# preon7/2019global

Measured on AMD Instinct MI355X. Metric: Mray/s + ms/frame at 1920x1080, depth 8; %HBM roofline, higher is better.
Workload: dtype f64

## Files before the change

### 2019global_amd/__init__.py

```python
from __future__ import annotations

import ctypes
import os
import threading
from typing import Optional, Sequence

import numpy as np

from . import scenes as _scenes

__all__ = [
    "GIError", "lib", "Camera", "Material", "Octree", "ImpSphere", "ImpTriangle", "ExpQuad",
    "ExpSphere", "ExpCube", "ExpCone", "ExpRectangle", "ExpBox",
    "RayTracer", "DeviceScene", "MODE_R", "MODE_X", "STAT_RAYS", "STAT_NODES", "STAT_PRIMS",
    "STAT_PIXELS", "TILE", "MultiScene", "devices_from_env", "obj_entities", "RAY_DOUBLES",
    "AOV_OUTPUTS", "camera_rays", "camera_rays_device",
]

HERE = os.path.dirname(os.path.abspath(__file__))
LIB_PATH = os.environ.get("GI_LIB") or os.path.join(HERE, "libgi.so")

MODE_R, MODE_X = 0, 1
FLAG_STATS = 1
FLAG_R_DFS = 2
FLAG_TIME = 4
FLAG_X_NO_SHADOW = 8
FLAG_X_WF = 16
FLAG_X_MEGA = 32
FLAG_X_SEG = 64
KAT_X_TREE, KAT_X_HBM = 1, 2
X_FORMS = ("k_mode_x", "k_wf_bounce", "k_seg")
R_KERNELS = ("k_mode_r", "k_rf_walk", "k_mode_r_batch")
STAT_RAYS, STAT_NODES, STAT_PRIMS, STAT_PIXELS, STAT_X_PATH_MAX = 0, 1, 2, 3, 4
STAT_X_ITERS, STAT_X_TRAV, STAT_X_HANDLE, STAT_X_HLANES, STAT_X_HCLOSE, STAT_X_HSHADOW = 5, 6, 7, 8, 9, 10
STAT_X_CYC_TRAV, STAT_X_CYC_HIT, STAT_X_CYC_NEXT, STAT_X_CYC_ALL = 11, 12, 13, 14
STAT_X_RESOLVED = 15
STAT_X_IT_NODE, STAT_X_LN_NODE, STAT_X_IT_LEAF, STAT_X_LN_LEAF = 16, 17, 18, 19
STAT_X_IT_RS, STAT_X_LN_RS, STAT_X_IT_ST, STAT_X_LN_ST = 20, 21, 22, 23
STAT_R_PAIRS, STAT_R_OVF_TILES = 24, 25
STATS_N = 26
TILE = 8
ABI_VERSION = 13
RAY_DOUBLES = 8
AOV_OUTPUTS = ("t", "normal", "albedo", "prim", "entity", "uv")
_AOV_KINDS = {"t": (np.float64, ()), "normal": (np.float64, (3,)), "albedo": (np.float64, (3,)),
              "prim": (np.int32, ()), "entity": (np.int32, ()), "uv": (np.int32, (2,))}


class GIError(RuntimeError):
    pass


class EntityDesc(ctypes.Structure):
    _fields_ = [("kind", ctypes.c_int32), ("has_material", ctypes.c_int32), ("args", ctypes.c_double * 11),
                ("mat_color", ctypes.c_double * 3), ("mat_shader", ctypes.c_double * 3),
                ("mat_specular_power", ctypes.c_double), ("mat_reflectivity", ctypes.c_double)]


class SceneDesc(ctypes.Structure):
    _fields_ = [("octree_min", ctypes.c_double * 3), ("octree_max", ctypes.c_double * 3),
                ("n_entities", ctypes.c_int32), ("entities", ctypes.POINTER(EntityDesc))]


class CameraDesc(ctypes.Structure):
    _fields_ = [("pos", ctypes.c_double * 3), ("up", ctypes.c_double * 3), ("forward", ctypes.c_double * 3),
                ("focal", ctypes.c_double)]


class Opts(ctypes.Structure):
    _fields_ = [("mode", ctypes.c_int32), ("spp", ctypes.c_int32), ("depth", ctypes.c_int32),
                ("shard_count", ctypes.c_int32), ("shard_index", ctypes.c_int32), ("band_rows", ctypes.c_int32),
                ("flags", ctypes.c_uint32), ("reserved", ctypes.c_int32), ("seed", ctypes.c_uint64),
                ("stats", ctypes.c_void_p), ("sample_begin", ctypes.c_int32), ("sample_end", ctypes.c_int32)]


class SceneInfo(ctypes.Structure):
    _fields_ = [("n_entities", ctypes.c_int32), ("n_nodes", ctypes.c_int32), ("n_leaves", ctypes.c_int32),
                ("max_depth", ctypes.c_int32), ("n_reachable", ctypes.c_int32), ("n_dropped", ctypes.c_int32),
                ("x_nodes", ctypes.c_int32), ("x_prims", ctypes.c_int32), ("device_bytes", ctypes.c_int64),
                ("x_node_bytes", ctypes.c_int32), ("x_lds_resident", ctypes.c_int32)]


class Hit(ctypes.Structure):
    _fields_ = [("entity", ctypes.c_int32), ("u", ctypes.c_int32), ("v", ctypes.c_int32),
                ("point", ctypes.c_double * 3), ("normal", ctypes.c_double * 3)]


class AovFrame(ctypes.Structure):
    _fields_ = [("w", ctypes.c_int32), ("h", ctypes.c_int32), ("x0", ctypes.c_int32), ("y0", ctypes.c_int32),
                ("x1", ctypes.c_int32), ("y1", ctypes.c_int32)]


class Aov(ctypes.Structure):
    _fields_ = [("t", ctypes.c_void_p), ("normal", ctypes.c_void_p), ("albedo", ctypes.c_void_p),
                ("prim", ctypes.c_void_p), ("entity", ctypes.c_void_p), ("uv", ctypes.c_void_p)]


TILE_CB = ctypes.CFUNCTYPE(None, ctypes.c_void_p, ctypes.c_int, ctypes.c_int, ctypes.POINTER(ctypes.c_uint8),
                           ctypes.POINTER(ctypes.c_double))

EXPORTS = ["gi_abi_version", "gi_last_error", "gi_camera_init", "gi_scene_create", "gi_scene_destroy",
           "gi_scene_get_info", "gi_render", "gi_render_device", "gi_shard_tiles", "gi_unshard_device",
           "gi_trace_ray", "gi_kat_expbox", "gi_kat_x_query", "gi_kat_x_variant", "gi_scene_kernel_ms", "gi_scene_x_form", "gi_scene_r_kernel", "gi_octree_create", "gi_octree_destroy",
           "gi_octree_intersect", "gi_multi_create", "gi_multi_destroy", "gi_multi_info", "gi_multi_render", "gi_device_count",
           "gi_device_list", "gi_build_id", "gi_obj_parse", "gi_intersect", "gi_occluded", "gi_intersect_device",
           "gi_occluded_device", "gi_render_aov", "gi_render_aov_device", "gi_camera_rays", "gi_camera_rays_device"]

_lib = None
_lock = threading.Lock()


def lib():
    global _lib
    with _lock:
        if _lib is not None:
            return _lib
        if not os.path.exists(LIB_PATH):
            raise GIError(f"{LIB_PATH} is missing: run `python 2019global_amd/build.py` (no CPU fallback)")
        try:
            import torch
        except ImportError:
            pass
        L = ctypes.CDLL(LIB_PATH)
        vp, i32, dp = ctypes.c_void_p, ctypes.c_int, ctypes.POINTER(ctypes.c_double)
        L.gi_abi_version.restype = i32
        L.gi_last_error.restype = ctypes.c_char_p
        L.gi_camera_init.argtypes = [dp, dp, ctypes.c_double, ctypes.POINTER(CameraDesc)]
        L.gi_scene_create.argtypes = [ctypes.POINTER(SceneDesc), ctypes.POINTER(vp)]
        L.gi_scene_destroy.argtypes = [vp]
        L.gi_scene_destroy.restype = None
        L.gi_scene_get_info.argtypes = [vp, ctypes.POINTER(SceneInfo)]
        L.gi_render.argtypes = [vp, ctypes.POINTER(CameraDesc), dp, i32, i32, ctypes.POINTER(Opts), dp,
                                ctypes.POINTER(ctypes.c_uint8), ctypes.POINTER(ctypes.c_int), TILE_CB, vp]
        L.gi_render_device.argtypes = [vp, ctypes.POINTER(CameraDesc), dp, i32, i32, ctypes.POINTER(Opts), vp, vp, vp]
        L.gi_shard_tiles.argtypes = [i32, i32, i32]
        L.gi_shard_tiles.restype = ctypes.c_int64
        L.gi_unshard_device.argtypes = [i32, i32, i32, vp, vp, vp, vp, vp]
        L.gi_trace_ray.argtypes = [vp, dp, dp, dp, ctypes.POINTER(Hit), dp]
        L.gi_kat_expbox.argtypes = [i32, dp, ctypes.POINTER(ctypes.c_int32)]
        ip = ctypes.POINTER(ctypes.c_int32)
        L.gi_kat_x_query.argtypes = [vp, i32, dp, dp, i32, ip, dp, ip, ip, ip, dp, ip, dp]
        L.gi_kat_x_variant.argtypes = [vp, i32, ip]
        i64 = ctypes.c_int64
        L.gi_intersect.argtypes = [vp, i64, dp, dp, ip, ip, dp]
        L.gi_occluded.argtypes = [vp, i64, dp, ip]
        L.gi_intersect_device.argtypes = [vp, i64, vp, vp, vp, vp, vp, vp]
        L.gi_occluded_device.argtypes = [vp, i64, vp, vp, vp]
        L.gi_render_aov.argtypes = [vp, ctypes.POINTER(CameraDesc), ctypes.POINTER(AovFrame), ctypes.POINTER(Aov)]
        L.gi_render_aov_device.argtypes = [vp, ctypes.POINTER(CameraDesc), ctypes.POINTER(AovFrame), ctypes.POINTER(Aov), vp]
        L.gi_camera_rays.argtypes = [ctypes.POINTER(CameraDesc), ctypes.POINTER(AovFrame), dp]
        L.gi_camera_rays_device.argtypes = [ctypes.POINTER(CameraDesc), ctypes.POINTER(AovFrame), vp, vp]
        L.gi_scene_kernel_ms.argtypes = [vp, ctypes.POINTER(ctypes.c_float), ctypes.POINTER(ctypes.c_int64)]
        L.gi_scene_x_form.argtypes = [vp, ctypes.POINTER(Opts), ctypes.POINTER(ctypes.c_int32)]
        L.gi_scene_r_kernel.argtypes = [vp, ctypes.POINTER(Opts), ctypes.POINTER(ctypes.c_int32)]
        L.gi_octree_create.argtypes = [ctypes.POINTER(SceneDesc), ctypes.POINTER(vp)]
        L.gi_octree_destroy.argtypes = [vp]
        L.gi_octree_destroy.restype = None
        L.gi_octree_intersect.argtypes = [vp, dp, dp, ctypes.POINTER(ctypes.c_int32), ctypes.c_int64,
                                          ctypes.POINTER(ctypes.c_int64)]
        L.gi_multi_create.argtypes = [ctypes.POINTER(SceneDesc), i32, ctypes.POINTER(ctypes.c_int), ctypes.POINTER(vp)]
        L.gi_multi_destroy.argtypes = [vp]
        L.gi_multi_destroy.restype = None
        L.gi_multi_info.argtypes = [vp, ctypes.POINTER(ctypes.c_int), ctypes.POINTER(ctypes.c_int),
                                    ctypes.POINTER(ctypes.c_int)]
        L.gi_multi_render.argtypes = [vp, ctypes.POINTER(CameraDesc), dp, i32, i32, ctypes.POINTER(Opts), dp,
                                      ctypes.POINTER(ctypes.c_uint8), ctypes.POINTER(ctypes.c_int), TILE_CB, vp]
        L.gi_device_list.argtypes = [ctypes.POINTER(ctypes.c_int32), i32]
        L.gi_build_id.restype = ctypes.c_char_p
        L.gi_obj_parse.argtypes = [ctypes.c_char_p, ctypes.c_int64, ctypes.POINTER(EntityDesc),
                                   ctypes.POINTER(EntityDesc), ctypes.c_int64, ctypes.POINTER(ctypes.c_int64)]
        if L.gi_abi_version() != ABI_VERSION:
            raise GIError(f"libgi ABI {L.gi_abi_version()} != {ABI_VERSION}")
        _lib = L
        return L


def build_id() -> str:
    return lib().gi_build_id().decode()


def _check(rc: int, what: str) -> None:
    if rc != 0:
        raise GIError(f"{what} failed ({rc}): {lib().gi_last_error().decode()}")


def _check_rays(rays) -> int:
    if not isinstance(rays, np.ndarray) or rays.dtype != np.float64 or rays.ndim != 2 or rays.shape[1] != RAY_DOUBLES or \
            not rays.flags.c_contiguous:
        raise ValueError(f"rays: a C-contiguous float64 array of shape (n, {RAY_DOUBLES}) -- o[3], d[3], tmax, reserved")
    return int(rays.shape[0])


def _aov_frame(w, h, window) -> AovFrame:
    def whole(v):
        return isinstance(v, (int, np.integer)) and not isinstance(v, bool)
    if not (whole(w) and whole(h)) or w <= 0 or h <= 0 or w >= 2 ** 31 or h >= 2 ** 31:
        raise ValueError("frame: w and h are positive integers")
    if window is None:
        window = (0, 0, w, h)
    window = tuple(window)
    if len(window) != 4 or not all(whole(v) for v in window):
        raise ValueError("window: four integers (x0, y0, x1, y1)")
    x0, y0, x1, y1 = (int(v) for v in window)
    if not (0 <= x0 <= x1 <= w and 0 <= y0 <= y1 <= h):
        raise ValueError(f"window {window}: reversed or not inside the {w} x {h} frame")
    return AovFrame(int(w), int(h), x0, y0, x1, y1)


def _d3(v) -> ctypes.Array:
    return (ctypes.c_double * 3)(*[float(x) for x in v])


class Material:

    def __init__(self, color, shader=(0.1, 0.7, 1.0), specular_power: float = 5.0, reflectivity: float = 0.0):
        self.color = tuple(float(c) for c in color)
        self.shader_parameters = tuple(float(c) for c in shader)
        self.specular_power = float(specular_power)
        self.reflectivity = float(reflectivity)


class _Entity:
    kind = 0

    def __init__(self, args: Sequence[float], material: Optional[Material]):
        self._args = tuple(float(a) for a in args)
        self._material = material

    @property
    def material(self) -> Optional[Material]:
        return self._material

    @material.setter
    def material(self, m: Material) -> None:
        self._material = m

    def _desc(self, d: EntityDesc) -> None:
        d.kind = self.kind
        for i, a in enumerate(self._args):
            d.args[i] = a
        m = self._material
        d.has_material = 1 if m is not None else 0
        if m is not None:
            for i in range(3):
                d.mat_color[i] = m.color[i]
                d.mat_shader[i] = m.shader_parameters[i]
            d.mat_specular_power = m.specular_power
            d.mat_reflectivity = m.reflectivity


class ImpSphere(_Entity):
    kind = _scenes.IMP_SPHERE

    def __init__(self, pos, radius, color):
        super().__init__((*pos, radius, *color), None)


class ImpTriangle(_Entity):
    kind = _scenes.IMP_TRIANGLE

    def __init__(self, p1, p2, p3):
        super().__init__((*p1, *p2, *p3), None)


class ExpQuad(_Entity):
    kind = _scenes.EXP_QUAD

    def __init__(self, pos, width, length, alpha, color):
        super().__init__((*pos, width, length, alpha, *color), None)


class ExpSphere(_Entity):
    kind = _scenes.EXP_SPHERE

    def __init__(self, pos, radius, color):
        super().__init__((*pos, radius, *color), None)


class ExpCube(_Entity):
    kind = _scenes.EXP_CUBE

    def __init__(self, pos, width, length, height, color):
        super().__init__((*pos, width, length, height, *color), None)


class ExpCone(_Entity):
    kind = _scenes.EXP_CONE

    def __init__(self, pos, dir, height, radius, color):
        super().__init__((*pos, *dir, height, radius, *color), None)


class ExpRectangle(_Entity):
    kind = _scenes.EXP_RECTANGLE

    def __init__(self, p1, p2, p3):
        super().__init__((*p1, *p2, *p3), None)


class ExpBox(_Entity):
    kind = _scenes.EXP_BOX

    def __init__(self, mn, mx):
        super().__init__((*mn, *mx), None)


def obj_entities(text, material: Optional[Material] = None) -> list:
    L = lib()
    data = text.encode() if isinstance(text, str) else bytes(text)
    tmpl = None
    if material is not None:
        tmpl = EntityDesc()
        t = _Entity((), material)
        t._desc(tmpl)
    n = ctypes.c_int64()
    _check(L.gi_obj_parse(data, len(data), tmpl, None, 0, ctypes.byref(n)), "gi_obj_parse")
    arr = (EntityDesc * max(1, n.value))()
    _check(L.gi_obj_parse(data, len(data), tmpl, arr, n.value, ctypes.byref(n)), "gi_obj_parse")
    out = []
    for i in range(n.value):
        d = arr[i]
        e = ImpTriangle(tuple(d.args[0:3]), tuple(d.args[3:6]), tuple(d.args[6:9]))
        if material is not None:
            e.material = Material(material.color, material.shader_parameters, material.specular_power,
                                  material.reflectivity)
        out.append(e)
    return out


class Octree:

    def __init__(self, min=(-20, -20, -20), max=(20, 20, 20)):
        self.min = tuple(float(v) for v in min)
        self.max = tuple(float(v) for v in max)
        self.entities = []
        self.generation = 0
        self._host = None
        self._host_gen = -1

    def push_back(self, e: _Entity) -> None:
        self.entities.append(e)
        self.generation += 1

    def intersect(self, origin, direction) -> list:
        L = lib()
        if self._host is None or self._host_gen != self.generation:
            self._close_host()
            d, keep = self._scene_desc()
            h = ctypes.c_void_p()
            _check(L.gi_octree_create(ctypes.byref(d), ctypes.byref(h)), "gi_octree_create")
            del keep
            self._host, self._host_gen = h, self.generation
        dv = np.asarray(direction, np.float64)
        dv = dv * (1.0 / np.sqrt((dv[0] * dv[0] + dv[1] * dv[1]) + dv[2] * dv[2]))
        n = ctypes.c_int64()
        _check(L.gi_octree_intersect(self._host, _d3(origin), _d3(dv), None, 0, ctypes.byref(n)), "gi_octree_intersect")
        out = (ctypes.c_int32 * max(1, n.value))()
        _check(L.gi_octree_intersect(self._host, _d3(origin), _d3(dv), out, n.value, ctypes.byref(n)),
               "gi_octree_intersect")
        return [self.entities[i] for i in out[:n.value]]

    def _close_host(self):
        if self._host is not None and self._host.value:
            lib().gi_octree_destroy(self._host)
        self._host = None

    def __del__(self):
        try:
            self._close_host()
        except Exception:
            pass

    @classmethod
    def from_scene(cls, s: "_scenes.Scene") -> "Octree":
        o = cls(s.octree_min, s.octree_max)
        for e in s.entities:
            ent = _Entity(e.args, None if e.material is None else
                          Material(e.material.color, e.material.shader, e.material.specular_power,
                                   e.material.reflectivity))
            ent.kind = e.kind
            o.push_back(ent)
        return o

    def _scene_desc(self):
        n = len(self.entities)
        arr = (EntityDesc * max(n, 1))()
        for i, e in enumerate(self.entities):
            e._desc(arr[i])
        d = SceneDesc()
        d.octree_min = _d3(self.min)
        d.octree_max = _d3(self.max)
        d.n_entities = n
        d.entities = ctypes.cast(arr, ctypes.POINTER(EntityDesc))
        return d, arr


class Camera:

    def __init__(self, pos, lookAt=(0.0, 0.0, 0.0), focal: float = 0.04):
        self._c = CameraDesc()
        _check(lib().gi_camera_init(_d3(pos), _d3(lookAt), float(focal), ctypes.byref(self._c)), "gi_camera_init")

    @property
    def pos(self):
        return tuple(self._c.pos)

    @property
    def up(self):
        return tuple(self._c.up)

    @property
    def forward(self):
        return tuple(self._c.forward)

    @property
    def focalDist(self):
        return self._c.focal


class DeviceScene:

    def __init__(self, octree: Octree):
        L = lib()
        d, keep = octree._scene_desc()
        h = ctypes.c_void_p()
        _check(L.gi_scene_create(ctypes.byref(d), ctypes.byref(h)), "gi_scene_create")
        self._h = h
        del keep

    @classmethod
    def from_scene(cls, s: "_scenes.Scene") -> "DeviceScene":
        return cls(Octree.from_scene(s))

    def close(self) -> None:
        if getattr(self, "_h", None) and self._h.value:
            lib().gi_scene_destroy(self._h)
            self._h = ctypes.c_void_p()

    def __del__(self):
        try:
            self.close()
        except Exception:
            pass

    def info(self) -> dict:
        i = SceneInfo()
        _check(lib().gi_scene_get_info(self._h, ctypes.byref(i)), "gi_scene_get_info")
        return {f: getattr(i, f) for f, _ in SceneInfo._fields_}

    @staticmethod
    def opts(mode=MODE_R, spp=1, depth=1, seed=0, shard_count=1, shard_index=0, band_rows=0, stats_ptr=0,
             flags=0, samples=None) -> Opts:
        o = Opts()
        o.mode, o.spp, o.depth, o.seed = mode, spp, depth, seed
        o.shard_count, o.shard_index, o.band_rows = shard_count, shard_index, band_rows
        o.flags = (FLAG_STATS if stats_ptr else 0) | flags
        o.stats = stats_ptr or None
        if samples is not None:
            o.sample_begin, o.sample_end = samples
        return o

    def render(self, cam: Camera, light, w: int, h: int, mode=MODE_R, spp=1, depth=1, seed=0, band_rows=0,
               cancel: Optional[ctypes.c_int] = None, callback=None, out=None, flags=0, samples=None):
        if out is None:
            rgb, rgb8 = np.zeros((h, w, 3), np.float64), np.zeros((h, w, 3), np.uint8)
        else:
            rgb, rgb8 = out
        for a, dt in ((rgb, np.float64), (rgb8, np.uint8)):
            if a is not None and (a.dtype != dt or a.size != w * h * 3 or not a.flags.c_contiguous):
                raise ValueError("render: out arrays must be C-contiguous [h, w, 3] float64 / uint8")
        cb = TILE_CB(callback) if callback is not None else TILE_CB()
        o = self.opts(mode, spp, depth, seed, band_rows=band_rows, flags=flags, samples=samples)
        _check(lib().gi_render(self._h, ctypes.byref(cam._c), _d3(light), w, h, ctypes.byref(o),
                               rgb.ctypes.data_as(ctypes.POINTER(ctypes.c_double)) if rgb is not None else None,
                               rgb8.ctypes.data_as(ctypes.POINTER(ctypes.c_uint8)) if rgb8 is not None else None,
                               ctypes.byref(cancel) if cancel is not None else None, cb, None), "gi_render")
        return rgb, rgb8

    def render_device(self, cam: Camera, light, w: int, h: int, d_rgb: int, d_rgb8: int = 0, stream: int = 0,
                      mode=MODE_R, spp=1, depth=1, seed=0, shard_count=1, shard_index=0, stats_ptr=0,
                      flags=0, samples=None) -> None:
        o = self.opts(mode, spp, depth, seed, shard_count, shard_index, stats_ptr=stats_ptr, flags=flags,
                      samples=samples)
        _check(lib().gi_render_device(self._h, ctypes.byref(cam._c), _d3(light), w, h, ctypes.byref(o),
                                      d_rgb or None, d_rgb8 or None, stream or None), "gi_render_device")

    def x_form(self, mode=MODE_X, spp=1, depth=1, flags=0) -> str:
        o = self.opts(mode, spp, depth, 0, flags=flags)
        f = ctypes.c_int32()
        _check(lib().gi_scene_x_form(self._h, ctypes.byref(o), ctypes.byref(f)), "gi_scene_x_form")
        return X_FORMS[f.value]

    def r_kernel(self, flags=0) -> str:
        o = self.opts(MODE_R, 1, 1, 0, flags=flags)
        k = ctypes.c_int32()
        _check(lib().gi_scene_r_kernel(self._h, ctypes.byref(o), ctypes.byref(k)), "gi_scene_r_kernel")
        return R_KERNELS[k.value]

    def kernel_ms(self):
        ms, n = ctypes.c_float(), ctypes.c_int64()
        _check(lib().gi_scene_kernel_ms(self._h, ctypes.byref(ms), ctypes.byref(n)), "gi_scene_kernel_ms")
        return float(ms.value), int(n.value)

    def trace_ray(self, origin, direction, light):
        hit = Hit()
        rgb = (ctypes.c_double * 3)()
        _check(lib().gi_trace_ray(self._h, _d3(origin), _d3(direction), _d3(light), ctypes.byref(hit), rgb),
               "gi_trace_ray")
        return hit, tuple(rgb)

    INTERSECT_OUTPUTS = ("t", "prim", "entity", "normal")

    def intersect(self, rays: np.ndarray, want=INTERSECT_OUTPUTS) -> dict:
        n = _check_rays(rays)
        want = tuple(want)
        if not want or any(k not in self.INTERSECT_OUTPUTS for k in want) or len(set(want)) != len(want):
            raise ValueError(f"intersect: want is a non-empty selection of {self.INTERSECT_OUTPUTS}")
        m = max(n, 1)
        bufs = {"t": np.empty(m, np.float64), "prim": np.empty(m, np.int32), "entity": np.empty(m, np.int32),
                "normal": np.empty((m, 3), np.float64)}
        ip, dp = ctypes.POINTER(ctypes.c_int32), ctypes.POINTER(ctypes.c_double)
        ptr = {k: (bufs[k].ctypes.data_as(dp if bufs[k].dtype == np.float64 else ip) if k in want else None)
               for k in self.INTERSECT_OUTPUTS}
        _check(lib().gi_intersect(self._h, n, rays.ctypes.data_as(dp), ptr["t"], ptr["prim"], ptr["entity"], ptr["normal"]),
               "gi_intersect")
        return {k: bufs[k][:n] for k in want}

    def occluded(self, rays: np.ndarray) -> np.ndarray:
        n = _check_rays(rays)
        out = np.empty(max(n, 1), np.int32)
        _check(lib().gi_occluded(self._h, n, rays.ctypes.data_as(ctypes.POINTER(ctypes.c_double)),
                                 out.ctypes.data_as(ctypes.POINTER(ctypes.c_int32))), "gi_occluded")
        return out[:n]

    def intersect_device(self, n: int, d_rays: int, d_t: int = 0, d_prim: int = 0, d_entity: int = 0, d_normal: int = 0,
                         stream: int = 0) -> None:
        _check(lib().gi_intersect_device(self._h, int(n), d_rays or None, d_t or None, d_prim or None, d_entity or None,
                                         d_normal or None, stream or None), "gi_intersect_device")

    def occluded_device(self, n: int, d_rays: int, d_occluded: int, stream: int = 0) -> None:
        _check(lib().gi_occluded_device(self._h, int(n), d_rays or None, d_occluded or None, stream or None),
               "gi_occluded_device")

    def render_aov(self, cam: "Camera", w: int, h: int, window=None, want=AOV_OUTPUTS) -> dict:
        want = tuple(want)
        if not want or any(k not in AOV_OUTPUTS for k in want) or len(set(want)) != len(want):
            raise ValueError(f"render_aov: want is a non-empty selection of {AOV_OUTPUTS}")
        f = _aov_frame(w, h, window)
        rows, cols = f.y1 - f.y0, f.x1 - f.x0
        bufs = {k: np.empty((rows, cols) + _AOV_KINDS[k][1], _AOV_KINDS[k][0]) for k in want}
        a = Aov(**{k: bufs[k].ctypes.data if bufs[k].size else _scratch_ptr() for k in want})
        _check(lib().gi_render_aov(self._h, ctypes.byref(cam._c), ctypes.byref(f), ctypes.byref(a)), "gi_render_aov")
        return bufs

    def render_aov_device(self, cam: "Camera", w: int, h: int, window=None, d_t: int = 0, d_normal: int = 0,
                          d_albedo: int = 0, d_prim: int = 0, d_entity: int = 0, d_uv: int = 0, stream: int = 0) -> None:
        f = _aov_frame(w, h, window)
        a = Aov(d_t or None, d_normal or None, d_albedo or None, d_prim or None, d_entity or None, d_uv or None)
        _check(lib().gi_render_aov_device(self._h, ctypes.byref(cam._c), ctypes.byref(f), ctypes.byref(a), stream or None),
               "gi_render_aov_device")

    def kat_x_variant(self, flags: int = 0) -> dict:
        out = (ctypes.c_int32 * 6)()
        _check(lib().gi_kat_x_variant(self._h, int(flags), out), "gi_kat_x_variant")
        return dict(zip(("LDS", "W4", "SH", "TRI", "CN", "FLAT"), (bool(v) for v in out)))

    def kat_x_query(self, recs: np.ndarray, cam_pos, flags: int = 0) -> dict:
        recs = np.ascontiguousarray(recs, np.float64).reshape(-1, 12)
        n = recs.shape[0]
        out = dict(prim1=np.zeros(n, np.int32), t1=np.zeros(n), occl=np.zeros(n, np.int32), skip_s=np.zeros(n, np.int32),
                   prim2=np.zeros(n, np.int32), t2=np.zeros(n), skip2=np.zeros(n, np.int32))
        sc = ctypes.c_double(float("nan"))
        ip, dp = ctypes.POINTER(ctypes.c_int32), ctypes.POINTER(ctypes.c_double)
        _check(lib().gi_kat_x_query(self._h, n, recs.ctypes.data_as(dp), _d3(cam_pos), int(flags),
                                    out["prim1"].ctypes.data_as(ip), out["t1"].ctypes.data_as(dp),
                                    out["occl"].ctypes.data_as(ip), out["skip_s"].ctypes.data_as(ip),
                                    out["prim2"].ctypes.data_as(ip), out["t2"].ctypes.data_as(dp),
                                    out["skip2"].ctypes.data_as(ip), ctypes.byref(sc)), "gi_kat_x_query")
        out["skip_cos"] = sc.value if n else None
        return out


_scratch = None


def _scratch_ptr() -> int:
    global _scratch
    if _scratch is None:
        _scratch = np.zeros(8)
    return _scratch.ctypes.data


def camera_rays(cam: "Camera", w: int, h: int, window=None) -> np.ndarray:
    f = _aov_frame(w, h, window)
    rays = np.empty(((f.y1 - f.y0) * (f.x1 - f.x0), RAY_DOUBLES), np.float64)
    p = rays.ctypes.data_as(ctypes.POINTER(ctypes.c_double)) if rays.size else \
        ctypes.cast(_scratch_ptr(), ctypes.POINTER(ctypes.c_double))
    _check(lib().gi_camera_rays(ctypes.byref(cam._c), ctypes.byref(f), p), "gi_camera_rays")
    return rays


def camera_rays_device(cam: "Camera", w: int, h: int, d_rays: int, window=None, stream: int = 0) -> None:
    f = _aov_frame(w, h, window)
    _check(lib().gi_camera_rays_device(ctypes.byref(cam._c), ctypes.byref(f), d_rays or None, stream or None),
           "gi_camera_rays_device")


def devices_from_env(default=None):
    v = os.environ.get("GI_DEVICES")
    if not v:
        return default
    if v.strip() == "all":
        import torch
        return list(range(torch.cuda.device_count()))
    return [int(t) for t in v.split(",") if t.strip()]


class MultiScene:

    def __init__(self, octree: Octree, devices: Sequence[int]):
        L = lib()
        d, keep = octree._scene_desc()
        devs = (ctypes.c_int * len(devices))(*[int(x) for x in devices])
        h = ctypes.c_void_p()
        _check(L.gi_multi_create(ctypes.byref(d), len(devices), devs, ctypes.byref(h)), "gi_multi_create")
        self._h = h
        del keep

    @classmethod
    def from_scene(cls, s: "_scenes.Scene", devices: Sequence[int]) -> "MultiScene":
        return cls(Octree.from_scene(s), devices)

    def info(self) -> dict:
        a, b, c = ctypes.c_int(), ctypes.c_int(), ctypes.c_int()
        _check(lib().gi_multi_info(self._h, ctypes.byref(a), ctypes.byref(b), ctypes.byref(c)), "gi_multi_info")
        return {"shards": a.value, "devices": b.value, "rccl": bool(c.value)}

    def render(self, cam: Camera, light, w: int, h: int, mode=MODE_R, spp=1, depth=1, seed=0, band_rows=0,
               cancel: Optional[ctypes.c_int] = None, callback=None, out=None):
        if out is None:
            rgb, rgb8 = np.zeros((h, w, 3), np.float64), np.zeros((h, w, 3), np.uint8)
        else:
            rgb, rgb8 = out
        for a, dt in ((rgb, np.float64), (rgb8, np.uint8)):
            if a is not None and (a.dtype != dt or a.size != w * h * 3 or not a.flags.c_contiguous):
                raise ValueError("render: out arrays must be C-contiguous [h, w, 3] float64 / uint8")
        cb = TILE_CB(callback) if callback is not None else TILE_CB()
        o = DeviceScene.opts(mode, spp, depth, seed, band_rows=band_rows)
        _check(lib().gi_multi_render(self._h, ctypes.byref(cam._c), _d3(light), w, h, ctypes.byref(o),
                                     rgb.ctypes.data_as(ctypes.POINTER(ctypes.c_double)) if rgb is not None else None,
                                     rgb8.ctypes.data_as(ctypes.POINTER(ctypes.c_uint8)) if rgb8 is not None else None,
                                     ctypes.byref(cancel) if cancel is not None else None, cb, None), "gi_multi_render")
        return rgb, rgb8

    def close(self) -> None:
        if getattr(self, "_h", None) and self._h.value:
            lib().gi_multi_destroy(self._h)
            self._h = ctypes.c_void_p()

    def __del__(self):
        try:
            self.close()
        except Exception:
            pass


def kat_expbox(recs: np.ndarray) -> np.ndarray:
    recs = np.ascontiguousarray(recs, np.float64)
    out = np.zeros(recs.shape[0], np.int32)
    _check(lib().gi_kat_expbox(recs.shape[0], recs.ctypes.data_as(ctypes.POINTER(ctypes.c_double)),
                               out.ctypes.data_as(ctypes.POINTER(ctypes.c_int32))), "gi_kat_expbox")
    return out


def shard_tiles(w: int, h: int, shard_count: int) -> int:
    return int(lib().gi_shard_tiles(w, h, shard_count))


def unshard_device(w, h, shard_count, d_packed, d_packed8, d_rgb, d_rgb8, stream=0) -> None:
    _check(lib().gi_unshard_device(w, h, shard_count, d_packed or None, d_packed8 or None, d_rgb or None,
                                   d_rgb8 or None, stream or None), "gi_unshard_device")


class Image:

    def __init__(self, rgb8: np.ndarray, rgb: Optional[np.ndarray] = None):
        self.rgb8 = rgb8
        self.radiance = rgb

    def width(self) -> int:
        return self.rgb8.shape[1]

    def height(self) -> int:
        return self.rgb8.shape[0]

    def getPixel(self, x: int, y: int):
        p = self.rgb8[y, x]
        return (p[0] / 255.0, p[1] / 255.0, p[2] / 255.0)


class RayTracer:

    def __init__(self, camera: Camera, light):
        self._camera = camera
        self._light = tuple(float(v) for v in light)
        self._image = Image(np.zeros((0, 0, 3), np.uint8))
        self._scene: Optional[Octree] = None
        self._dev: Optional[DeviceScene] = None
        self._cancel = ctypes.c_int(1)
        self.band_rows = 64

    def setScene(self, scene: Octree) -> None:
        self._scene = scene
        self._dev = None
        self._dev_gen = -1

    def running(self) -> bool:
        return self._cancel.value == 0

    def stop(self) -> None:
        self._cancel.value = 1

    def start(self) -> None:
        self._cancel.value = 0

    def getImage(self) -> Image:
        return self._image

    def run(self, w: int, h: int) -> None:
        self._image = Image(np.zeros((h, w, 3), np.uint8), np.zeros((h, w, 3)))
        if self._scene is None:
            raise GIError("setScene() was not called")
        if self._dev is None or getattr(self, "_dev_gen", -1) != self._scene.generation:
            devs = devices_from_env()
            self._dev = MultiScene(self._scene, devs) if devs and len(devs) > 1 else DeviceScene(self._scene)
            self._dev_gen = self._scene.generation
        img = self._image

        def on_band(_user, y0, rows, p8, pf):
            n = w * rows * 3
            img.rgb8[y0:y0 + rows] = np.ctypeslib.as_array(p8, shape=(n,)).reshape(rows, w, 3)
            img.radiance[y0:y0 + rows] = np.ctypeslib.as_array(pf, shape=(n,)).reshape(rows, w, 3)

        rgb = np.zeros((h, w, 3))
        rgb8 = np.zeros((h, w, 3), np.uint8)
        o = DeviceScene.opts(MODE_R, band_rows=self.band_rows)
        cb = TILE_CB(on_band)
        fn = lib().gi_multi_render if isinstance(self._dev, MultiScene) else lib().gi_render
        rc = fn(self._dev._h, ctypes.byref(self._camera._c), _d3(self._light), w, h, ctypes.byref(o),
                             rgb.ctypes.data_as(ctypes.POINTER(ctypes.c_double)),
                             rgb8.ctypes.data_as(ctypes.POINTER(ctypes.c_uint8)), ctypes.byref(self._cancel), cb, None)
        if rc not in (0, -4):
            _check(rc, "gi_render")
```

### 2019global_amd/build.py

```python
from __future__ import annotations

import glob
import hashlib
import os
import shutil
import subprocess
import sys

HERE = os.path.dirname(os.path.abspath(__file__))
ROOT = os.path.dirname(HERE)
CSRC = os.path.join(HERE, "csrc")
INCLUDE = os.path.join(ROOT, "include")
OUT = os.path.join(HERE, "libgi.so")
ROCM = os.environ.get("ROCM_PATH", "/opt/rocm")
ARCH = "gfx950"

HOST_SRCS = ["gi_build.cpp", "gi_bvh.cpp", "gi_capi.cpp", "gi_multi.cpp", "gi_obj.cpp"]
DEV_SRCS = ["gi_kernels.hip", "gi_wf.hip"]
HEADERS = ["gi_math.h", "gi_scene.h", "gi_internal.h", "gi_dev.h"]

COMMON = ["-std=c++17", "-fPIC", "-ffp-contract=off", "-fno-fast-math", f"-I{INCLUDE}", f"-I{CSRC}"]


def source_hash() -> str:
    h = hashlib.sha256()
    for name in sorted(HOST_SRCS + DEV_SRCS + HEADERS):
        h.update(name.encode() + b"\0" + open(os.path.join(CSRC, name), "rb").read() + b"\0")
    h.update(b"gi.h\0" + open(os.path.join(INCLUDE, "gi.h"), "rb").read())
    return h.hexdigest()[:16]


def _run(cmd, verbose):
    if verbose:
        print(" ".join(cmd), flush=True)
    subprocess.run(cmd, check=True)


def _stale(out, deps):
    if not os.path.exists(out):
        return True
    t = os.path.getmtime(out)
    return any(os.path.getmtime(d) > t for d in deps)


def build(verbose: bool = False, force: bool = False, variant: str = "", hip_defines=()) -> str:
    hipcc = shutil.which("hipcc") or os.path.join(ROCM, "bin", "hipcc")
    objdir = os.path.join(HERE, "_obj")
    out = OUT
    if variant:
        out = os.path.join(HERE, "_variants", f"libgi_{variant}.so")
        os.makedirs(os.path.dirname(out), exist_ok=True)
    os.makedirs(objdir, exist_ok=True)
    hdrs = [os.path.join(CSRC, h) for h in HEADERS] + [os.path.join(INCLUDE, "gi.h")]
    bid = source_hash()
    bid_file = os.path.join(objdir, "build_id")
    old_bid = open(bid_file).read().strip() if os.path.exists(bid_file) else ""
    objs = []
    for s in HOST_SRCS:
        src, obj = os.path.join(CSRC, s), os.path.join(objdir, s + ".o")
        defs = [f'-DGI_BUILD_ID="{bid}"'] if s == "gi_capi.cpp" else []
        if force or _stale(obj, [src] + hdrs) or (defs and old_bid != bid):
            _run(["g++", "-O2", *COMMON, *defs, "-D__HIP_PLATFORM_AMD__", f"-I{ROCM}/include", "-c", src, "-o", obj],
                 verbose)
        objs.append(obj)
    with open(bid_file, "w") as f:
        f.write(bid + "\n")
    jobs = []
    for s in DEV_SRCS:
        src = os.path.join(CSRC, s)
        obj = os.path.join(objdir, s + (f".{variant}" if variant else "") + ".o")
        if force or _stale(obj, [src] + hdrs):
            extra = os.environ.get("GI_VARIANT_FLAGS", "").split() if variant else []
            cmd = [hipcc, f"--offload-arch={ARCH}", "-O3", "-Wshadow", *COMMON, *[f"-D{d}" for d in hip_defines],
                   *extra, "-munsafe-fp-atomics", "-c", src, "-o", obj]
            if verbose:
                print(" ".join(cmd), flush=True)
            jobs.append((cmd, subprocess.Popen(cmd)))
        objs.append(obj)
    failed = [(cmd, p.returncode) for cmd, p in [(c, p) for c, p in jobs if p.wait() != 0]]
    for cmd, _ in failed:
        if os.path.exists(cmd[-1]):
            os.remove(cmd[-1])
    if failed:
        for cmd, rc in failed:
            print(f"build failed ({rc}): {' '.join(cmd)}", file=sys.stderr)
        raise subprocess.CalledProcessError(failed[0][1], failed[0][0])
    if force or _stale(out, objs):
        _run([hipcc, f"--offload-arch={ARCH}", "-shared", "-o", out, *objs, f"-L{ROCM}/lib", "-lamdhip64", "-ldl"], verbose)
    for leftover in glob.glob(out + ".[0-9]*.hipv4-*") + glob.glob(out + ".[0-9]*.host-*"):
        os.remove(leftover)
    return out


if __name__ == "__main__":
    args = sys.argv[1:]
    var, defs = "", []
    if "--variant" in args:
        i = args.index("--variant")
        var, defs = args[i + 1], [a for a in args[i + 2:] if not a.startswith("--")]
    build(verbose=True, force="--force" in args, variant=var, hip_defines=defs)
```

### 2019global_amd/csrc/gi_capi.cpp

```cpp
#include <hip/hip_runtime_api.h>

#include <algorithm>
#include <cmath>
#include <cstring>
#include <memory>
#include <mutex>
#include <new>
#include <string>
#include <vector>

#include "gi.h"
#include "gi_internal.h"
#include "gi_scene.h"

namespace gi {
bool build_host_scene(const gi_scene_desc& desc, HostScene& hs, std::string& err);
long long shard_tiles(int w, int h, int shard_count);
hipError_t x_launch_config(const DevScene& sc, int device, XLaunchCfg& cfg);
int x_form_choice(const DevScene& sc, const XLaunchCfg& xc, const gi_opts& o);
long long x_wf_chunk();
int x_env_rf_per_slot();
int r_kernel_choice(const DevScene& sc, const gi_opts& o);
unsigned rf_own_pairs();
unsigned rf_page_pairs();
// ... 399 lines not shown
        return fail(GI_ERR_ARG, "progressive pass out of order: a pass continues the previous pass's frame "
                                "(same camera, light, size, spp, depth, seed, shard) from its sample_end");
    }
    s->prog_key = key;
    s->prog_next = -1;
    return GI_OK;
}
void prog_done(gi_scene* s, const gi_opts& o) {
    s->prog_next = (o.sample_end > 0 && o.sample_end < o.spp) ? o.sample_end : -1;
}

int band_rows_of(const gi_opts* o, int h) {
    int band = o->band_rows > 0 ? o->band_rows : h;
    band = ((band + GI_TILE - 1) / GI_TILE) * GI_TILE;
    return std::min(band, ((h + GI_TILE - 1) / GI_TILE) * GI_TILE);
}

int scene_create_on(const gi_scene_desc* desc, int device, gi_scene** out) {
    *out = nullptr;
    int rc = bind_device(device);
    if (rc || (rc = check_device(device))) return rc;
    std::unique_ptr<gi_scene, void (*)(gi_scene*)> s(new gi_scene(), [](gi_scene* p) { destroy_scene(p); });
    s->device = device;
    std::string err;
    if (!build_host_scene(*desc, s->host, err)) return fail(GI_ERR_SCENE, err);
    DevScene& d = s->dev;
    memset(&d, 0, sizeof d);
    const HostScene& h = s->host;
    hipError_t e;
    gi_scene* sp = s.get();
    if ((e = upload(sp, h.rnodes, &d.rnodes)) != hipSuccess || (e = upload(sp, h.leaf_ents, &d.leaf_ents)) != hipSuccess ||
        (e = upload(sp, h.ents, &d.ents)) != hipSuccess || (e = upload(sp, h.tris, &d.tris)) != hipSuccess ||
        (e = upload(sp, h.xwnodes, &d.xwnodes)) != hipSuccess || (e = upload(sp, h.xhot, &d.xhot)) != hipSuccess ||
        (e = upload(sp, h.xbox, &d.xbox)) != hipSuccess ||
        (e = upload(sp, h.xprims, &d.xprims)) != hipSuccess || (e = upload(sp, h.xflat, &d.xflat)) != hipSuccess ||
        (e = upload(sp, std::vector<unsigned>(16, 0u), const_cast<const unsigned**>(&d.work))) != hipSuccess ||
        (e = upload(sp, h.app_off, &d.app_off)) != hipSuccess || (e = upload(sp, h.app_rec, &d.app_rec)) != hipSuccess ||
        (e = upload(sp, h.rpath_rec, &d.rpath_rec)) != hipSuccess || (e = upload(sp, h.rc_nodes, &d.rc_nodes)) != hipSuccess ||
        (e = upload(sp, h.rc_ent, &d.rc_ent)) != hipSuccess || (e = upload(sp, h.rc_maxkey, &d.rc_maxkey)) != hipSuccess ||
        (e = upload(sp, h.r_always, &d.r_always)) != hipSuccess ||
        (e = upload(sp, h.r_leaf_of_rank, &d.r_leaf_of_rank)) != hipSuccess)
        return hip_fail(e, "scene upload");
    d.n_rnodes = (int32_t)h.rnodes.size();
    d.n_ents = (int32_t)h.ents.size();
    d.n_xwnodes = (int32_t)h.xwnodes.size();
    d.n_xprims = (int32_t)h.xprims.size();
    d.x_max_depth = h.x_max_depth;
    d.x_handle8 = h.x_handle8;
    d.x_flags = h.x_flags;
    d.x_skip_a = h.x_skip_a;
    d.x_skip_b = h.x_skip_b;
    d.n_xhot = (int32_t)h.xhot.size();
    d.n_r_always = (int32_t)h.r_always.size();
    d.rc_ext = (float)h.rc_ext;
    {
        const size_t bytes = h.xwnodes.size() * sizeof(XWNode) + h.xhot.size() * sizeof(XHot) +
                             h.xprims.size() * sizeof(XPrim) + h.ents.size() * sizeof(REnt);
        d.x_lds_bytes = bytes <= 40 * 1024 ? (int32_t)bytes : 0;
        d.n_xflat = (int32_t)h.xflat.size();
        d.x_flat = (d.x_lds_bytes > 0 && h.x_flat_ok) ? 1 : 0;
        const size_t per_wg = bytes + 256 * 10 * sizeof(double) + 4 * 68 * sizeof(unsigned);
        d.x_waves4 = (d.x_lds_bytes > 0 && 4 * per_wg <= 160 * 1024) ? 1 : 0;
        d.x_tri_only = 1;
        for (const REnt& r : h.ents)
            if (r.kind == K_IMP_SPHERE || r.kind == K_EXP_SPHERE || r.kind == K_EXP_CONE || r.kind == K_EXP_RECTANGLE) {
                d.x_waves4 = 0;
                d.x_tri_only = 0;
            }
        for (const XPrim& xp : h.xprims)
            if (xp.kind != 0) d.x_tri_only = 0;
        d.r_tri_only = 1;
        for (const REnt& r : h.ents)
            if (r.kind != K_IMP_TRIANGLE) d.r_tri_only = 0;
    }
    const bool want_cn = h.xwnodes.size() * sizeof(XWNode) > (size_t)2 << 20;
    if (d.x_lds_bytes == 0 && want_cn && encode_xcnodes(h.xwnodes, s->host.xcnodes) &&
        (e = upload(sp, h.xcnodes, &d.xcnodes)) != hipSuccess)
        return hip_fail(e, "scene upload (quantised nodes)");
    for (int k = 0; k < 3; ++k) { d.root_lo[k] = INFINITY; d.root_hi[k] = -INFINITY; }
    if (!h.xwnodes.empty())
        for (int c = 0; c < 8; ++c)
            if (h.xwnodes[0].child[c] != XEMPTY)
                for (int k = 0; k < 3; ++k) {
                    d.root_lo[k] = std::min(d.root_lo[k], h.xwnodes[0].lo[k][c]);
                    d.root_hi[k] = std::max(d.root_hi[k], h.xwnodes[0].hi[k][c]);
                }
    d.x_far_r = INFINITY;
    for (int k = 0; k < 3; ++k)
        if (d.root_lo[k] <= d.root_hi[k]) {
            const float m = 16.0f * std::max(std::fabs(d.root_lo[k]), std::fabs(d.root_hi[k]));
            d.x_far_r = std::isinf(d.x_far_r) ? m : std::max(d.x_far_r, m);
        }
    if ((e = x_launch_config(d, device, s->xcfg)) != hipSuccess) return hip_fail(e, "occupancy query");
    *out = s.release();
    return GI_OK;
}

void scene_destroy(gi_scene* s) noexcept { destroy_scene(s); }
int scene_device(const gi_scene* s) { return s->device; }
std::mutex& scene_mutex(gi_scene* s) { return s->mu; }

int scene_render_band(gi_scene* s, const CamDev& cd, const double light[3], int w, int h, int y0, const gi_opts& o,
                      double* d_rgb, uint8_t* d_rgb8, hipStream_t stream, bool timer) {
    int rc = bind_device(s->device);
    if (rc || (rc = ensure_xscratch(s, w, h, &o)) || (timer && (rc = ensure_timer(s, &o)))) return rc;
    return issue_render(s, cd, v3(light[0], light[1], light[2]), w, h, y0, o, d_rgb, d_rgb8, stream, timer);
}

int unshard(int w, int h, int n, const double* packed, const uint8_t* packed8, double* rgb, uint8_t* rgb8,
            hipStream_t stream) {
    const hipError_t e = launch_unshard(w, h, n, packed, packed8, rgb, rgb8, stream);
    return e == hipSuccess ? GI_OK : hip_fail(e, "unshard launch");
}

}

extern "C" {

int gi_abi_version(void) { return GI_ABI_VERSION; }
const char* gi_last_error(void) { return g_err.c_str(); }

int gi_device_list(int32_t* out, int cap) {
    int ndev = 0, n = 0;
    if (hipGetDeviceCount(&ndev) != hipSuccess) return 0;
    for (int d = 0; d < ndev; ++d) {
        hipDeviceProp_t prop;
        if (hipGetDeviceProperties(&prop, d) == hipSuccess && std::strncmp(prop.gcnArchName, "gfx950", 6) == 0) {
            if (out && n < cap) out[n] = d;
            ++n;
        }
    }
    return n;
}

int gi_device_count(void) { return gi_device_list(nullptr, 0); }

#ifndef GI_BUILD_ID
#define GI_BUILD_ID "unknown"
#endif
const char* gi_build_id(void) { return GI_BUILD_ID; }

int gi_camera_init(const double pos[3], const double look_at[3], double focal, gi_camera* out) {
    if (!pos || !look_at || !out) return fail(GI_ERR_ARG, "null argument");
    const V3 p = v3(pos[0], pos[1], pos[2]);
    const V3 f = normalize(v3(look_at[0], look_at[1], look_at[2]) - p);
    st3(out->pos, p);
    out->up[0] = 0; out->up[1] = 0; out->up[2] = 1.0;
    st3(out->forward, f);
    out->focal = focal;
    return GI_OK;
}

int gi_scene_create(const gi_scene_desc* desc, gi_scene** out) {
    return guard([&]() -> int {
        if (!desc || !out || desc->n_entities < 0 || (desc->n_entities > 0 && !desc->entities))
            return fail(GI_ERR_ARG, "bad scene descriptor");
        *out = nullptr;
        int ndev = 0;
        hipError_t e = hipGetDeviceCount(&ndev);
        if (e != hipSuccess || ndev <= 0) return fail(GI_ERR_DEVICE, "no HIP device (libgi renders only on gfx950)");
        int dev = 0;
        if ((e = hipGetDevice(&dev)) != hipSuccess) return hip_fail(e, "hipGetDevice");
        return scene_create_on(desc, dev, out);
    });
}

void gi_scene_destroy(gi_scene* s) { destroy_scene(s); }

int gi_scene_get_info(const gi_scene* s, gi_scene_info* info) {
    if (!s || !info) return fail(GI_ERR_ARG, "null argument");
    info->n_entities = (int32_t)s->host.ents.size();
    info->n_nodes = (int32_t)s->host.rnodes.size();
    info->n_leaves = s->host.n_leaves;
    info->max_depth = s->host.max_depth;
    info->n_reachable = s->host.n_reachable;
    info->n_dropped = s->host.n_dropped;
    info->x_nodes = (int32_t)(s->host.xnodes.empty() ? s->host.xwnodes.size() : s->host.xnodes.size());
    info->x_prims = (int32_t)s->host.xprims.size();
    info->device_bytes = s->bytes;
    info->x_node_bytes = s->dev.xcnodes ? (int32_t)sizeof(XCNode) : (int32_t)sizeof(XWNode);
    info->x_lds_resident = s->dev.x_lds_bytes > 0 ? 1 : 0;
    return GI_OK;
}

int64_t gi_shard_tiles(int w, int h, int shard_count) {
    if (w <= 0 || h <= 0 || shard_count < 1) return -1;
    return shard_tiles(w, h, shard_count);
}

int gi_render_device(gi_scene* s, const gi_camera* cam, const double light[3], int w, int h, const gi_opts* o,
                     double* d_rgb, uint8_t* d_rgb8, void* stream) {
    return guard([&]() -> int {
        DeviceRestore keep;
        if (!s) return fail(GI_ERR_ARG, "null scene");
        int rc = check_opts(w, h, o);
        if (rc) return rc;
        if (!cam || !light) return fail(GI_ERR_ARG, "null camera or light");
        std::lock_guard<std::mutex> lk(s->mu);
        if ((rc = prog_check(s, *cam, light, w, h, *o))) return rc;
        rc = scene_render_band(s, make_cam(*cam, w), light, w, h, 0, *o, d_rgb, d_rgb8, static_cast<hipStream_t>(stream),
                               true);
        if (rc == GI_OK) prog_done(s, *o);
        return rc;
    });
}

int gi_render(gi_scene* s, const gi_camera* cam, const double light[3], int w, int h, const gi_opts* o, double* rgb,
              uint8_t* rgb8, const volatile int* cancel, gi_tile_cb cb, void* user) {
    return guard([&]() -> int {
        DeviceRestore keep;
        if (!s) return fail(GI_ERR_ARG, "null scene");
        int rc = check_opts(w, h, o);
        if (rc) return rc;
        if (!cam || !light) return fail(GI_ERR_ARG, "null camera or light");
        if (o->shard_count != 1) return fail(GI_ERR_ARG, "gi_render renders whole frames; use gi_render_device or gi_multi to shard");
        std::lock_guard<std::mutex> lk(s->mu);
        if ((rc = bind_device(s->device))) return rc;
        const int band = band_rows_of(o, h);
        const size_t band_px = (size_t)w * (size_t)band;
        const int n_bands = (h + band - 1) / band;
        if (o->sample_end > 0 && n_bands > 1)
            return fail(GI_ERR_ARG, "progressive passes render whole frames: band_rows 0 or >= h");
        if ((rc = prog_check(s, *cam, light, w, h, *o))) return rc;
        if ((rc = ensure_hostpath(s, band_px, std::min(n_bands, HostPath::kSlots)))) return rc;
        HostPath& hp = s->hp;
        const CamDev cd = make_cam(*cam, w);
        const bool want_rgb = rgb || cb, want_rgb8 = rgb8 || cb;
        const bool direct = n_bands == 1;
        double* const dst_rgb = direct && rgb ? rgb : hp.h_rgb[0];
        uint8_t* const dst_rgb8 = direct && rgb8 ? rgb8 : hp.h_rgb8[0];
        auto issue = [&](int i) -> int {
            const int k = i % HostPath::kSlots, y0 = i * band, rows = std::min(band, h - y0);
            const size_t n = (size_t)w * rows * 3;
            hipError_t e = hipSuccess;
            if (i >= HostPath::kSlots && (e = hipStreamWaitEvent(hp.render, hp.copied[k], 0)) != hipSuccess)
                return hip_fail(e, "render");
            const int r = scene_render_band(s, cd, light, w, rows, y0, *o, hp.d_rgb[k], hp.d_rgb8[k], hp.render, false);
            if (r) return r;
            e = hipEventRecord(hp.rendered[k], hp.render);
            if (e == hipSuccess) e = hipStreamWaitEvent(hp.copy, hp.rendered[k], 0);
            double* const to = i == 0 ? dst_rgb : hp.h_rgb[k];
            uint8_t* const to8 = i == 0 ? dst_rgb8 : hp.h_rgb8[k];
            if (e == hipSuccess && want_rgb) e = hipMemcpyAsync(to, hp.d_rgb[k], n * sizeof(double), hipMemcpyDeviceToHost, hp.copy);
            if (e == hipSuccess && want_rgb8) e = hipMemcpyAsync(to8, hp.d_rgb8[k], n, hipMemcpyDeviceToHost, hp.copy);
            if (e == hipSuccess) e = hipEventRecord(hp.copied[k], hp.copy);
            return e == hipSuccess ? GI_OK : hip_fail(e, "render");
        };
        hipError_t e = hipSuccess;
        if (cancel && *cancel) rc = fail(GI_ERR_CANCELLED, "cancelled");
        else rc = issue(0);
        for (int i = 0; rc == GI_OK && i < n_bands; i++) {
            if (i + 1 < n_bands) {
                if (cancel && *cancel) { rc = fail(GI_ERR_CANCELLED, "cancelled"); break; }
                if ((rc = issue(i + 1)) != GI_OK) break;
            }
            const int k = i % HostPath::kSlots, y0 = i * band, rows = std::min(band, h - y0);
            const size_t n = (size_t)w * rows * 3;
            if ((e = hipEventSynchronize(hp.copied[k])) != hipSuccess) { rc = hip_fail(e, "render"); break; }
            const double* hr = i == 0 ? dst_rgb : hp.h_rgb[k];
            const uint8_t* hr8 = i == 0 ? dst_rgb8 : hp.h_rgb8[k];
            if (rgb && hr != rgb) { std::memcpy(rgb + (size_t)y0 * w * 3, hr, n * sizeof(double)); hr = rgb + (size_t)y0 * w * 3; }
            if (rgb8 && hr8 != rgb8) { std::memcpy(rgb8 + (size_t)y0 * w * 3, hr8, n); hr8 = rgb8 + (size_t)y0 * w * 3; }
            if (cb) cb(user, y0, rows, hr8, hr);
        }
        const hipError_t e1 = hipStreamSynchronize(hp.render), e2 = hipStreamSynchronize(hp.copy);
        if (rc == GI_OK && (e1 != hipSuccess || e2 != hipSuccess)) rc = hip_fail(e1 != hipSuccess ? e1 : e2, "render");
        if (rc == GI_OK) prog_done(s, *o);
        return rc;
    });
}

int gi_scene_kernel_ms(gi_scene* s, float* avg_ms, int64_t* n) {
    return guard([&]() -> int {
        DeviceRestore keep;
        if (!s || !avg_ms) return fail(GI_ERR_ARG, "null argument");
        std::lock_guard<std::mutex> lk(s->mu);
        KTimer& kt = s->kt;
        if (kt.recorded == 0) return fail(GI_ERR_ARG, "no render issued with GI_FLAG_TIME since the last read");
        int rc = bind_device(s->device);
        if (rc) return rc;
        const long long first = kt.recorded > KTimer::kRing ? kt.recorded - KTimer::kRing : 0;
        for (long long r = std::max(first, kt.folded); r < kt.recorded; r++) {
            const hipError_t e = fold_timer(kt, (int)(r % KTimer::kRing));
            if (e != hipSuccess) return hip_fail(e, "gi_scene_kernel_ms");
        }
        *avg_ms = (float)(kt.sum_ms / (double)kt.folded);
        if (n) *n = kt.folded;
        kt.recorded = 0;
        kt.folded = 0;
        kt.sum_ms = 0.0;
        return GI_OK;
    });
}

int gi_scene_x_form(gi_scene* s, const gi_opts* o, int32_t* form) {
    return guard([&]() -> int {
        if (!s || !o || !form) return fail(GI_ERR_ARG, "null argument");
        std::lock_guard<std::mutex> lk(s->mu);
        *form = x_form_choice(s->dev, s->xcfg, *o);
        return GI_OK;
    });
}

int gi_scene_r_kernel(gi_scene* s, const gi_opts* o, int32_t* kernel) {
    return guard([&]() -> int {
        if (!s || !o || !kernel) return fail(GI_ERR_ARG, "null argument");
        std::lock_guard<std::mutex> lk(s->mu);
        *kernel = r_kernel_choice(s->dev, *o);
        if (*kernel == 1 && s->xs.rf_failed > 0 && s->xs.rf_slots == 0) *kernel = 2;
        return GI_OK;
    });
}

int gi_unshard_device(int w, int h, int shard_count, const double* d_packed, const uint8_t* d_packed8, double* d_rgb,
                      uint8_t* d_rgb8, void* stream) {
    return guard([&]() -> int {
        if (w <= 0 || h <= 0 || shard_count < 1) return fail(GI_ERR_ARG, "bad unshard arguments");
        if ((d_rgb && !d_packed) || (d_rgb8 && !d_packed8)) return fail(GI_ERR_ARG, "missing packed input");
        return unshard(w, h, shard_count, d_packed, d_packed8, d_rgb, d_rgb8, static_cast<hipStream_t>(stream));
    });
}

int gi_trace_ray(gi_scene* s, const double origin[3], const double dir[3], const double light[3], gi_hit* hit,
                 double rgb[3]) {
    return guard([&]() -> int {
        DeviceRestore keep;
        if (!s || !origin || !dir || !light || !hit || !rgb) return fail(GI_ERR_ARG, "null argument");
        std::lock_guard<std::mutex> lk(s->mu);
        int rc = bind_device(s->device);
        if (rc) return rc;
        int32_t* d_i = nullptr;
        double* d_d = nullptr;
        hipError_t e;
        if ((e = hipMalloc((void**)&d_i, 4 * sizeof(int32_t))) != hipSuccess) return hip_fail(e, "hipMalloc");
        if ((e = hipMalloc((void**)&d_d, 9 * sizeof(double))) != hipSuccess) { (void)hipFree(d_i); return hip_fail(e, "hipMalloc"); }
        const V3 o = v3(origin[0], origin[1], origin[2]);
        const V3 d = normalize(v3(dir[0], dir[1], dir[2]));
        e = launch_trace_ray(s->dev, o, d, v3(light[0], light[1], light[2]), d_i, d_d, nullptr);
        int32_t hi[3] = {-1, 0, 0};
        double hd[9] = {0};
        if (e == hipSuccess) e = hipMemcpy(hi, d_i, 3 * sizeof(int32_t), hipMemcpyDeviceToHost);
        if (e == hipSuccess) e = hipMemcpy(hd, d_d, 9 * sizeof(double), hipMemcpyDeviceToHost);
        (void)hipFree(d_i);
        (void)hipFree(d_d);
        if (e != hipSuccess) return hip_fail(e, "trace_ray");
        hit->entity = hi[0];
        hit->u = hi[1];
        hit->v = hi[2];
        for (int k = 0; k < 3; ++k) { hit->point[k] = hd[k]; hit->normal[k] = hd[3 + k]; rgb[k] = hd[6 + k]; }
        return GI_OK;
    });
}

namespace {
int check_ray_args(const gi_scene* s, int64_t n, const double* rays) {
    if (!s) return fail(GI_ERR_ARG, "null scene");
    if (n < 0) return fail(GI_ERR_ARG, "negative ray count");
    if (n > 0 && !rays) return fail(GI_ERR_ARG, "null rays");
    return GI_OK;
}
int ray_query_device(gi_scene* s, bool any, const CastIO& io, hipStream_t stream) {
    if (reinterpret_cast<uintptr_t>(io.rays) & 15) return fail(GI_ERR_ARG, "device ray records must be 16-byte aligned");
    int rc = bind_device(s->device);
    if (rc) return rc;
    const hipError_t e = launch_ray_query(s->dev, s->xcfg, any, io, stream);
    return e == hipSuccess ? GI_OK : hip_fail(e, any ? "gi_occluded launch" : "gi_intersect launch");
}
struct DevBuf {
    void* p = nullptr;
    ~DevBuf() { (void)hipFree(p); }
    hipError_t alloc(size_t bytes) { return hipMalloc(&p, bytes); }
};
}

int gi_intersect_device(gi_scene* s, int64_t n, const double* d_rays, double* d_t, int32_t* d_prim, int32_t* d_entity,
                        double* d_normal, void* stream) {
    return guard([&]() -> int {
        DeviceRestore keep;
        int rc = check_ray_args(s, n, d_rays);
        if (rc) return rc;
        if (!d_t && !d_prim && !d_entity && !d_normal) return fail(GI_ERR_ARG, "gi_intersect: every output is null");
        if (n == 0) return GI_OK;
        return ray_query_device(s, false, CastIO{d_rays, (long long)n, d_t, d_prim, d_entity, d_normal, nullptr},
                                static_cast<hipStream_t>(stream));
    });
}

int gi_occluded_device(gi_scene* s, int64_t n, const double* d_rays, int32_t* d_occluded, void* stream) {
    return guard([&]() -> int {
        DeviceRestore keep;
        int rc = check_ray_args(s, n, d_rays);
        if (rc) return rc;
        if (!d_occluded) return fail(GI_ERR_ARG, "gi_occluded: null output");
        if (n == 0) return GI_OK;
        return ray_query_device(s, true, CastIO{d_rays, (long long)n, nullptr, nullptr, nullptr, nullptr, d_occluded},
                                static_cast<hipStream_t>(stream));
    });
}

int gi_intersect(gi_scene* s, int64_t n, const double* rays, double* t, int32_t* prim, int32_t* entity, double* normal) {
    return guard([&]() -> int {
        DeviceRestore keep;
        int rc = check_ray_args(s, n, rays);
        if (rc) return rc;
        if (!t && !prim && !entity && !normal) return fail(GI_ERR_ARG, "gi_intersect: every output is null");
        if (n == 0) return GI_OK;
        if ((rc = bind_device(s->device))) return rc;
        const size_t m = (size_t)n;
        DevBuf dr, dt, dp, de, dn;
        hipError_t e = dr.alloc(m * GI_RAY_DOUBLES * sizeof(double));
        if (e == hipSuccess && t) e = dt.alloc(m * sizeof(double));
        if (e == hipSuccess && prim) e = dp.alloc(m * sizeof(int32_t));
        if (e == hipSuccess && entity) e = de.alloc(m * sizeof(int32_t));
        if (e == hipSuccess && normal) e = dn.alloc(m * 3 * sizeof(double));
        if (e != hipSuccess) return hip_fail(e, "hipMalloc (ray query staging)");
        if ((e = hipMemcpy(dr.p, rays, m * GI_RAY_DOUBLES * sizeof(double), hipMemcpyHostToDevice)) != hipSuccess)
            return hip_fail(e, "gi_intersect");
        rc = ray_query_device(s, false, CastIO{static_cast<const double*>(dr.p), (long long)n, static_cast<double*>(dt.p),
                                               static_cast<int32_t*>(dp.p), static_cast<int32_t*>(de.p),
                                               static_cast<double*>(dn.p), nullptr}, nullptr);
        if (rc) return rc;
        if (t) e = hipMemcpy(t, dt.p, m * sizeof(double), hipMemcpyDeviceToHost);
        if (e == hipSuccess && prim) e = hipMemcpy(prim, dp.p, m * sizeof(int32_t), hipMemcpyDeviceToHost);
        if (e == hipSuccess && entity) e = hipMemcpy(entity, de.p, m * sizeof(int32_t), hipMemcpyDeviceToHost);
        if (e == hipSuccess && normal) e = hipMemcpy(normal, dn.p, m * 3 * sizeof(double), hipMemcpyDeviceToHost);
        return e == hipSuccess ? GI_OK : hip_fail(e, "gi_intersect");
    });
}

int gi_occluded(gi_scene* s, int64_t n, const double* rays, int32_t* occluded) {
    return guard([&]() -> int {
        DeviceRestore keep;
        int rc = check_ray_args(s, n, rays);
        if (rc) return rc;
        if (!occluded) return fail(GI_ERR_ARG, "gi_occluded: null output");
        if (n == 0) return GI_OK;
        if ((rc = bind_device(s->device))) return rc;
        const size_t m = (size_t)n;
        DevBuf dr, dc;
        hipError_t e = dr.alloc(m * GI_RAY_DOUBLES * sizeof(double));
        if (e == hipSuccess) e = dc.alloc(m * sizeof(int32_t));
        if (e != hipSuccess) return hip_fail(e, "hipMalloc (ray query staging)");
        if ((e = hipMemcpy(dr.p, rays, m * GI_RAY_DOUBLES * sizeof(double), hipMemcpyHostToDevice)) != hipSuccess)
            return hip_fail(e, "gi_occluded");
        rc = ray_query_device(s, true, CastIO{static_cast<const double*>(dr.p), (long long)n, nullptr, nullptr, nullptr, nullptr,
                                              static_cast<int32_t*>(dc.p)}, nullptr);
        if (rc) return rc;
        e = hipMemcpy(occluded, dc.p, m * sizeof(int32_t), hipMemcpyDeviceToHost);
        return e == hipSuccess ? GI_OK : hip_fail(e, "gi_occluded");
    });
}

namespace {
int check_aov_frame(const gi_camera* cam, const gi_aov_frame* f, bool* empty) {
    if (!cam || !f) return fail(GI_ERR_ARG, "null camera or frame");
    if (f->w <= 0 || f->h <= 0 || (int64_t)f->w * f->h > (int64_t)1 << 34) return fail(GI_ERR_ARG, "bad frame size");
    if (f->x0 < 0 || f->y0 < 0 || f->x1 > f->w || f->y1 > f->h || f->x0 > f->x1 || f->y0 > f->y1)
        return fail(GI_ERR_ARG, "the window [x0, x1) x [y0, y1) is reversed or not inside the frame");
    bool fin = std::isfinite(cam->focal);
    for (int k = 0; k < 3; ++k) fin = fin && std::isfinite(cam->pos[k]) && std::isfinite(cam->up[k]) && std::isfinite(cam->forward[k]);
    if (!fin) return fail(GI_ERR_ARG, "non-finite camera field");
    *empty = f->x0 == f->x1 || f->y0 == f->y1;
    return GI_OK;
}
bool aov_all_null(const gi_aov& a) { return !a.t && !a.normal && !a.albedo && !a.prim && !a.entity && !a.uv; }
AovIO aov_io(const gi_aov_frame& f, const gi_aov& a) {
    return AovIO{f.x0, f.y0, f.x1 - f.x0, f.y1 - f.y0, a.t, a.normal, a.albedo, a.prim, a.entity, a.uv};
}
}

int gi_render_aov_device(gi_scene* s, const gi_camera* cam, const gi_aov_frame* frame, const gi_aov* d_out, void* stream) {
    return guard([&]() -> int {
        DeviceRestore keep;
        if (!s) return fail(GI_ERR_ARG, "null scene");
        if (!d_out) return fail(GI_ERR_ARG, "null output struct");
        bool empty = false;
        int rc = check_aov_frame(cam, frame, &empty);
        if (rc) return rc;
        if (aov_all_null(*d_out)) return fail(GI_ERR_ARG, "gi_render_aov: every output is null");
        if (empty) return GI_OK;
        if ((rc = bind_device(s->device))) return rc;
        const hipError_t e = launch_aov(s->dev, s->xcfg, make_cam(*cam, frame->w), aov_io(*frame, *d_out), static_cast<hipStream_t>(stream));
        return e == hipSuccess ? GI_OK : hip_fail(e, "gi_render_aov launch");
    });
}

int gi_render_aov(gi_scene* s, const gi_camera* cam, const gi_aov_frame* frame, const gi_aov* out) {
    return guard([&]() -> int {
        DeviceRestore keep;
        if (!s) return fail(GI_ERR_ARG, "null scene");
        if (!out) return fail(GI_ERR_ARG, "null output struct");
        bool empty = false;
        int rc = check_aov_frame(cam, frame, &empty);
        if (rc) return rc;
        if (aov_all_null(*out)) return fail(GI_ERR_ARG, "gi_render_aov: every output is null");
        if (empty) return GI_OK;
        if ((rc = bind_device(s->device))) return rc;
        const size_t m = (size_t)(frame->x1 - frame->x0) * (size_t)(frame->y1 - frame->y0);
        DevBuf dt, dn, da, dp, de, du;
        hipError_t e = hipSuccess;
        if (out->t) e = dt.alloc(m * sizeof(double));
        if (e == hipSuccess && out->normal) e = dn.alloc(m * 3 * sizeof(double));
        if (e == hipSuccess && out->albedo) e = da.alloc(m * 3 * sizeof(double));
        if (e == hipSuccess && out->prim) e = dp.alloc(m * sizeof(int32_t));
        if (e == hipSuccess && out->entity) e = de.alloc(m * sizeof(int32_t));
        if (e == hipSuccess && out->uv) e = du.alloc(m * 2 * sizeof(int32_t));
        if (e != hipSuccess) return hip_fail(e, "hipMalloc (feature buffer staging)");
        const gi_aov d{static_cast<double*>(dt.p), static_cast<double*>(dn.p), static_cast<double*>(da.p),
                       static_cast<int32_t*>(dp.p), static_cast<int32_t*>(de.p), static_cast<int32_t*>(du.p)};
        e = launch_aov(s->dev, s->xcfg, make_cam(*cam, frame->w), aov_io(*frame, d), nullptr);
        if (e != hipSuccess) return hip_fail(e, "gi_render_aov launch");
        if (out->t) e = hipMemcpy(out->t, dt.p, m * sizeof(double), hipMemcpyDeviceToHost);
        if (e == hipSuccess && out->normal) e = hipMemcpy(out->normal, dn.p, m * 3 * sizeof(double), hipMemcpyDeviceToHost);
        if (e == hipSuccess && out->albedo) e = hipMemcpy(out->albedo, da.p, m * 3 * sizeof(double), hipMemcpyDeviceToHost);
        if (e == hipSuccess && out->prim) e = hipMemcpy(out->prim, dp.p, m * sizeof(int32_t), hipMemcpyDeviceToHost);
        if (e == hipSuccess && out->entity) e = hipMemcpy(out->entity, de.p, m * sizeof(int32_t), hipMemcpyDeviceToHost);
        if (e == hipSuccess && out->uv) e = hipMemcpy(out->uv, du.p, m * 2 * sizeof(int32_t), hipMemcpyDeviceToHost);
        return e == hipSuccess ? GI_OK : hip_fail(e, "gi_render_aov");
    });
}

int gi_camera_rays_device(const gi_camera* cam, const gi_aov_frame* frame, double* d_rays, void* stream) {
    return guard([&]() -> int {
        bool empty = false;
        int rc = check_aov_frame(cam, frame, &empty);
        if (rc) return rc;
        if (!d_rays) return fail(GI_ERR_ARG, "null rays");
        if (reinterpret_cast<uintptr_t>(d_rays) & 15) return fail(GI_ERR_ARG, "device ray records must be 16-byte aligned");
        if (empty) return GI_OK;
        const hipError_t e = launch_cam_rays(make_cam(*cam, frame->w), frame->x0, frame->y0, frame->x1 - frame->x0,
                                             frame->y1 - frame->y0, d_rays, static_cast<hipStream_t>(stream));
        return e == hipSuccess ? GI_OK : hip_fail(e, "gi_camera_rays launch");
    });
}

int gi_camera_rays(const gi_camera* cam, const gi_aov_frame* frame, double* rays) {
    return guard([&]() -> int {
        bool empty = false;
        int rc = check_aov_frame(cam, frame, &empty);
        if (rc) return rc;
        if (!rays) return fail(GI_ERR_ARG, "null rays");
        if (empty) return GI_OK;
        const size_t bytes = (size_t)(frame->x1 - frame->x0) * (size_t)(frame->y1 - frame->y0) * GI_RAY_DOUBLES * sizeof(double);
        DevBuf dr;
        hipError_t e = dr.alloc(bytes);
        if (e != hipSuccess) return hip_fail(e, "hipMalloc (camera ray staging)");
        e = launch_cam_rays(make_cam(*cam, frame->w), frame->x0, frame->y0, frame->x1 - frame->x0, frame->y1 - frame->y0,
                            static_cast<double*>(dr.p), nullptr);
        if (e == hipSuccess) e = hipMemcpy(rays, dr.p, bytes, hipMemcpyDeviceToHost);
        return e == hipSuccess ? GI_OK : hip_fail(e, "gi_camera_rays");
    });
}

int gi_kat_expbox(int n, const double* recs, int32_t* out) {
    return guard([&]() -> int {
        if (n < 0 || (n > 0 && (!recs || !out))) return fail(GI_ERR_ARG, "bad arguments");
        if (n == 0) return GI_OK;
        int ndev = 0;
        if (hipGetDeviceCount(&ndev) != hipSuccess || ndev <= 0) return fail(GI_ERR_DEVICE, "no HIP device");
        double* d_r = nullptr;
        int32_t* d_o = nullptr;
        hipError_t e;
        if ((e = hipMalloc((void**)&d_r, (size_t)n * 12 * sizeof(double))) != hipSuccess) return hip_fail(e, "hipMalloc");
        if ((e = hipMalloc((void**)&d_o, (size_t)n * sizeof(int32_t))) != hipSuccess) { (void)hipFree(d_r); return hip_fail(e, "hipMalloc"); }
        e = hipMemcpy(d_r, recs, (size_t)n * 12 * sizeof(double), hipMemcpyHostToDevice);
        if (e == hipSuccess) e = launch_box_kat(n, d_r, d_o, nullptr);
        if (e == hipSuccess) e = hipMemcpy(out, d_o, (size_t)n * sizeof(int32_t), hipMemcpyDeviceToHost);
        (void)hipFree(d_r);
        (void)hipFree(d_o);
        return e == hipSuccess ? GI_OK : hip_fail(e, "gi_kat_expbox");
    });
}

int gi_kat_x_query(gi_scene* s, int n, const double* recs, const double cam_pos[3], int flags, int32_t* prim1, double* t1,
                   int32_t* occl, int32_t* skip_s, int32_t* prim2, double* t2, int32_t* skip2, double* skip_cos) {
    return guard([&]() -> int {
        DeviceRestore keep;
        if (!s || !cam_pos || n < 0 || (flags & ~3) != 0) return fail(GI_ERR_ARG, "bad arguments");
        if (n > 0 && (!recs || !prim1 || !t1 || !occl || !skip_s || !prim2 || !t2 || !skip2)) return fail(GI_ERR_ARG, "null argument");
        if (n == 0) return GI_OK;
        std::lock_guard<std::mutex> lk(s->mu);
        int rc = bind_device(s->device);
        if (rc) return rc;
        double *d_r = nullptr, *d_d = nullptr;
        int32_t* d_i = nullptr;
        std::vector<int32_t> hi((size_t)n * 5);
        std::vector<double> hd((size_t)n * 2 + 1);
        hipError_t e;
        if ((e = hipMalloc((void**)&d_r, (size_t)n * 12 * sizeof(double))) == hipSuccess &&
            (e = hipMalloc((void**)&d_i, hi.size() * sizeof(int32_t))) == hipSuccess)
            e = hipMalloc((void**)&d_d, hd.size() * sizeof(double));
        if (e == hipSuccess) e = hipMemcpy(d_r, recs, (size_t)n * 12 * sizeof(double), hipMemcpyHostToDevice);
        if (e == hipSuccess)
            e = launch_x_query(s->dev, s->xcfg, v3(cam_pos[0], cam_pos[1], cam_pos[2]), flags, n, d_r, d_i, d_d, nullptr);
        if (e == hipSuccess) e = hipMemcpy(hi.data(), d_i, hi.size() * sizeof(int32_t), hipMemcpyDeviceToHost);
        if (e == hipSuccess) e = hipMemcpy(hd.data(), d_d, hd.size() * sizeof(double), hipMemcpyDeviceToHost);
        (void)hipFree(d_r);
        (void)hipFree(d_i);
        (void)hipFree(d_d);
        if (e != hipSuccess) return hip_fail(e, "gi_kat_x_query");
        for (size_t i = 0; i < (size_t)n; ++i) {
            prim1[i] = hi[5 * i];
            occl[i] = hi[5 * i + 1];
            skip_s[i] = hi[5 * i + 2];
            prim2[i] = hi[5 * i + 3];
            skip2[i] = hi[5 * i + 4];
// ... 48 lines not shown
```

### 2019global_amd/csrc/gi_kernels.hip

```cpp
#include <hip/hip_runtime.h>

#include <algorithm>
#include <cfloat>
#include <cmath>
#include <cstdlib>
#include <mutex>

#include "gi.h"
#include "gi_dev.h"
#include "gi_scene.h"

namespace gi {

namespace {

template <bool TRI = false>
__device__ bool ent_hit(const DevScene& sc, const REnt& e, V3 o, V3 d, V3& P, V3& N, uint32_t& nprim) {
    if (TRI) {
        ++nprim;
        return tri_hit(sc.tris[e.tri_first], o, d, P, N);
    }
    if (e.kind == K_IMP_SPHERE) {
        ++nprim;
        return sphere_hit(ld3(e.pos), e.radius, o, d, P, N);
// ... 1486 lines not shown
                                    const unsigned li = spread ? e * n_groups + ng : ng * 64u + e;
                                    blk_list[e] = li < n_list ? wk.list[li] : 0xFFFFFFFFu;
                                }
                            }
                            __builtin_amdgcn_wave_barrier();
                            used_new = n_need - avail;
                            if (lane == leader) { blk_meta[1] = ng; blk_meta[2] = nc; }
                            if (!have) {
                                j = rank - avail;
                                ps = blk_list[j];
                                c = nc;
                                g = ng;
                                have = true;
                            }
                        } else if (!have && phase == PH_NEED) {
                            phase = PH_DEAD;
                        }
                        if (nb >= n_blocks && lane == leader) blk_meta[3] = 1u;
                    }
                    if (lane == leader) blk_meta[0] = used_new;
                    __builtin_amdgcn_wave_barrier();
                    if (phase == PH_NEED && have) {
                        const unsigned i = pm ? g : spread ? j * n_groups + g : g * 64u + j;
                        const unsigned cu = pm ? c + j : c;
                        if (ps != 0xFFFFFFFFu) {
                            slot_pixel(m, (long long)(ps >> 6), (int)(ps & 63), idx, x, y);
                            y += m.y0;
                            if (spp > 1) idx = (long long)i;
                            key = mx_key(seed, (uint64_t)y * (uint64_t)m.w + (uint64_t)x);
                            smp = wk.s0 + (int)cu * k;
                            phase = PH_START;
                            if (cu == 0) ++npx;
                        }
                    }
                }
                if (phase == PH_NEED) continue;
                if (phase == PH_DEAD) break;
                if (phase == PH_START) {
                    double jx = 0.0, jy = 0.0;
                    if (spp > 1) {
                        jx = mx_u01k(key, smp, 0xFFFF, 0);
                        jy = mx_u01k(key, smp, 0xFFFF, 1);
                    }
                    const V3 d0 = primary_dir(cam, (double)x + jx, (double)y + jy);
                    if (burst < GI_X_START_BURST) {
                        const F3 iv0 = f3(__builtin_amdgcn_rcpf((float)d0.x), __builtin_amdgcn_rcpf((float)d0.y),
                                          __builtin_amdgcn_rcpf((float)d0.z));
                        if (!root_hit(sc, f3((float)cam.pos.x, (float)cam.pos.y, (float)cam.pos.z), iv0)) {
                            ++nrays;
                            ++nres;
                            if (spp > 1) {
                                double* q = wk.part + 3 * ((size_t)idx * (size_t)spp + (size_t)smp);
                                q[0] = 0.0; q[1] = 0.0; q[2] = 0.0;
                            } else {
                                if (rgb) { rgb[3 * idx] = 0.0; rgb[3 * idx + 1] = 0.0; rgb[3 * idx + 2] = 0.0; }
                                if (rgb8) { rgb8[3 * idx] = 0; rgb8[3 * idx + 1] = 0; rgb8[3 * idx + 2] = 0; }
                            }
                            ++burst;
                            ++smp;
                            phase = (smp < wk.s1 && ((smp - wk.s0) & (k - 1)) != 0) ? PH_START : PH_DONEPX;
                            continue;
                        }
                    }
                    if (STATS) {
                        cnt.path_t0 = (uint64_t)wall_clock64();
                        cnt.path_it = 0;
                        cnt.path_st = 0;
                    }
                    o = cam.pos;
                    d = normalize(d0);
                    Lv = v3(0, 0, 0);
                    T = v3(1, 1, 1);
                    b = 0;
                    tmax = INFINITY;
                    tbest = INFINITY;
                    tbest_f = INFINITY;
                }
                if (no_shadow && phase == PH_SHADOW) {
                    best = -1;
                    raying = false;
                    break;
                }
                of = f3((float)o.x, (float)o.y, (float)o.z);
                ivf = inv_dir(d);
                dmask = (d.x < 0 ? 1 : 0) | (d.y < 0 ? 2 : 0) | (d.z < 0 ? 4 : 0);
                const uint32_t rm = children_mask<false>(W, of, ivf, tbest_f, dmask);
                if (phase == PH_START) phase = PH_CLOSEST;
                best = -1;
                node = 0;
                level = 0;
                mlo = mhi = 0;
                lvl_set<SH>(mlo, mhi, 0, rm);
                raying = rm != 0;
                if (raying) prefetch();
                break;
            }
        }
        if (HELP) any_gave = __ballot(gave) != 0;
        if (STATS) {
            const uint64_t t3 = clock64();
            cnt.cyc_trav += t1 - t0;
            cnt.cyc_hit += t2 - t1;
            cnt.cyc_next += t3 - t2;
        }
    }
    if (STATS) cnt.cyc_all += clock64() - t_begin;
    if (STATS) {
        uint64_t ns = nsteps;
        for (int off = 32; off > 0; off >>= 1) ns += __shfl_xor(ns, off);
        cnt.trav += ns;
    }
    cnt.rays += nrays;
    cnt.nodes += nnode;
    cnt.prims += nprim;
    cnt.px += npx;
    cnt.res += nres;
}

template <bool STATS, bool HELP, bool CN, bool SH, bool TR>
__global__ __launch_bounds__(256, GI_X_MIN_WAVES) void k_mode_x(DevScene sc, CamDev cam, V3 light, TileMap m, int spp, int depth,
                                                 uint64_t seed, double* rgb, uint8_t* rgb8,
                                                 unsigned long long* stats, XWork wk, int handle8, int xflags) {
    XCounters c;
    __shared__ unsigned s_blk[kWavesPerBlock][68];
    unsigned* blk = s_blk[threadIdx.x >> 6];
    extern __shared__ int lds_nst[];
    XHelp hp;
    hp.ray = reinterpret_cast<double*>(lds_nst + 16 * 256);
    hp.own = reinterpret_cast<int*>(hp.ray + 7 * 256);
    hp.res = hp.own + 256;
    if constexpr (CN)
        mode_x_wave<STATS, HELP, SH, TR>(sc, sc.xcnodes, sc.xhot, sc.xprims, sc.ents, lds_nst + threadIdx.x, hp, cam, light, m,
                                         spp, depth, seed, rgb, rgb8, blk, wk, handle8, xflags, c);
    else
        mode_x_wave<STATS, HELP, SH, TR>(sc, sc.xwnodes, sc.xhot, sc.xprims, sc.ents, lds_nst + threadIdx.x, hp, cam, light, m,
                                         spp, depth, seed, rgb, rgb8, blk, wk, handle8, xflags, c);
    if (STATS) {
        if ((threadIdx.x & 63) == 0) {
            atomicAdd(stats + GI_STAT_X_ITERS, (unsigned long long)c.iters);
            atomicAdd(stats + GI_STAT_X_TRAV, (unsigned long long)c.trav);
            atomicAdd(stats + GI_STAT_X_HANDLE, (unsigned long long)c.handle);
            atomicAdd(stats + GI_STAT_X_HLANES, (unsigned long long)c.hlanes);
            atomicAdd(stats + GI_STAT_X_HCLOSE, (unsigned long long)c.hclose);
            atomicAdd(stats + GI_STAT_X_HSHADOW, (unsigned long long)c.hshadow);
            atomicAdd(stats + GI_STAT_X_CYC_TRAV, (unsigned long long)c.cyc_trav);
            atomicAdd(stats + GI_STAT_X_CYC_HIT, (unsigned long long)c.cyc_hit);
            atomicAdd(stats + GI_STAT_X_CYC_NEXT, (unsigned long long)c.cyc_next);
            atomicAdd(stats + GI_STAT_X_CYC_ALL, (unsigned long long)c.cyc_all);
            atomicAdd(stats + GI_STAT_X_IT_NODE, (unsigned long long)c.it_node);
            atomicAdd(stats + GI_STAT_X_LN_NODE, (unsigned long long)c.ln_node);
            atomicAdd(stats + GI_STAT_X_IT_LEAF, (unsigned long long)c.it_leaf);
            atomicAdd(stats + GI_STAT_X_LN_LEAF, (unsigned long long)c.ln_leaf);
            atomicAdd(stats + GI_STAT_X_IT_RS, (unsigned long long)c.it_rs);
            atomicAdd(stats + GI_STAT_X_LN_RS, (unsigned long long)c.ln_rs);
            atomicAdd(stats + GI_STAT_X_IT_ST, (unsigned long long)c.it_st);
            atomicAdd(stats + GI_STAT_X_LN_ST, (unsigned long long)c.ln_st);
        }
        wave_add_stats(stats, c.rays, c.nodes, c.prims, c.px);
        uint64_t cr = c.res, pm = c.path_max;
        for (int off = 32; off > 0; off >>= 1) {
            cr += __shfl_xor(cr, off);
            pm = max(pm, (uint64_t)__shfl_xor(pm, off));
        }
        if ((threadIdx.x & 63) == 0) {
            atomicAdd(stats + GI_STAT_X_RESOLVED, (unsigned long long)cr);
            atomicMax(stats + GI_STAT_X_PATH_MAX, (unsigned long long)pm);
        }
    }
}

constexpr int kClassifyBlock = 1024;
template <bool STATS>
__global__ __launch_bounds__(kClassifyBlock) void k_x_classify(DevScene sc, CamDev cam, TileMap m, int spp, double* rgb,
                                                     uint8_t* rgb8, unsigned* list, unsigned* n_list,
                                                     unsigned long long* stats, unsigned* zero2) {
    if (zero2 && blockIdx.x == 0 && threadIdx.x < 2) zero2[threadIdx.x] = 0u;
    const long long s = (long long)blockIdx.x * blockDim.x + threadIdx.x;
    const long long lt = s >> 6;
    const int lane = threadIdx.x & 63;
    long long idx = -1;
    int x = 0, y = 0;
    bool scene = false, zero = false, bg = false;
    if (lt < m.n_local) {
        if (slot_pixel(m, lt, lane, idx, x, y)) {
            bg = pixel_misses_box(cam, x, y + m.y0, sc.root_lo, sc.root_hi);
            scene = !bg;
            zero = bg;
        } else {
            zero = idx >= 0 && m.shard_count > 1;
        }
    }
    if (zero) {
        if (rgb) { rgb[3 * idx] = 0; rgb[3 * idx + 1] = 0; rgb[3 * idx + 2] = 0; }
        if (rgb8) { rgb8[3 * idx] = 0; rgb8[3 * idx + 1] = 0; rgb8[3 * idx + 2] = 0; }
    }
    const unsigned long long ms = __ballot(scene && list != nullptr);
    __shared__ unsigned s_cnt[kClassifyBlock / 64 + 1];
    const int wv = threadIdx.x >> 6;
    if (lane == 0) s_cnt[wv] = (unsigned)__popcll(ms);
    __syncthreads();
    if (threadIdx.x == 0) {
        unsigned acc = 0;
        for (int k = 0; k < kClassifyBlock / 64; ++k) {
            const unsigned c = s_cnt[k];
            s_cnt[k] = acc;
            acc += c;
        }
        s_cnt[kClassifyBlock / 64] = acc ? atomicAdd(n_list, acc) : 0u;
    }
    __syncthreads();
    if (scene && list) list[s_cnt[kClassifyBlock / 64] + s_cnt[wv] + (unsigned)__popcll(ms & ((1ull << lane) - 1))] = (unsigned)s;
    if (STATS && (s & ~63ll) < m.n_local * 64) {
        wave_add_stats(stats, bg ? (uint64_t)spp : 0, 0, 0, bg ? 1 : 0);
        uint64_t r = bg ? (uint64_t)spp : 0;
        for (int off = 32; off > 0; off >>= 1) r += __shfl_xor(r, off);
        if (lane == 0 && r) atomicAdd(stats + GI_STAT_X_RESOLVED, (unsigned long long)r);
    }
}

__global__ __launch_bounds__(256) void k_x_reduce(TileMap m, XWork wk, int spp, double* rgb, uint8_t* rgb8) {
    const unsigned i = blockIdx.x * blockDim.x + threadIdx.x;
    if (i >= *wk.n_list) return;
    const unsigned ps = wk.list[i];
    long long idx = -1;
    int x = 0, y = 0;
    slot_pixel(m, (long long)(ps >> 6), (int)(ps & 63), idx, x, y);
    double a = 0, b = 0, c = 0;
    const double* p = wk.part + 3 * (size_t)i * (size_t)spp;
    int s = 0;
    if ((spp & 1) == 0) {
        const double2* q = reinterpret_cast<const double2*>(p);
        for (; s + 1 < wk.s1; s += 2) {
            const double2 v0 = q[3 * (s >> 1)], v1 = q[3 * (s >> 1) + 1], v2 = q[3 * (s >> 1) + 2];
            a = a + v0.x;
            b = b + v0.y;
            c = c + v1.x;
            a = a + v1.y;
            b = b + v2.x;
            c = c + v2.y;
        }
    }
    for (; s < wk.s1; ++s) {
        a = a + p[3 * s];
        b = b + p[3 * s + 1];
        c = c + p[3 * s + 2];
    }
    const double n = (double)wk.s1;
    const double c0 = smin(a / n, 1.0), c1 = smin(b / n, 1.0), c2 = smin(c / n, 1.0);
    if (rgb) { rgb[3 * idx] = c0; rgb[3 * idx + 1] = c1; rgb[3 * idx + 2] = c2; }
    if (rgb8) quantize(c0, c1, c2, rgb8 + 3 * idx);
}

__global__ __launch_bounds__(256) void k_unshard(TileMap m, const double* packed, const uint8_t* packed8, double* rgb,
                                                  uint8_t* rgb8) {
    const long long i = (long long)blockIdx.x * blockDim.x + threadIdx.x;
    const long long t = i / (kTile * kTile);
    if (t >= m.n_tiles) return;
    const int lane = (int)(i % (kTile * kTile));
    const int ty = (int)(t / m.tiles_x), tx = (int)(t % m.tiles_x);
    const int x = tx * kTile + (lane & 7), y = ty * kTile + (lane >> 3);
    if (x >= m.w || y >= m.h) return;
    const long long r = t % m.shard_count, lt = t / m.shard_count;
    const long long src = (r * m.n_local + lt) * (kTile * kTile) + lane;
    const long long dst = (long long)y * m.w + x;
    if (rgb) { rgb[3 * dst] = packed[3 * src]; rgb[3 * dst + 1] = packed[3 * src + 1]; rgb[3 * dst + 2] = packed[3 * src + 2]; }
    if (rgb8) { rgb8[3 * dst] = packed8[3 * src]; rgb8[3 * dst + 1] = packed8[3 * src + 1]; rgb8[3 * dst + 2] = packed8[3 * src + 2]; }
}

__global__ __launch_bounds__(256) void k_box_kat(int n, const double* recs, int32_t* out) {
    const int i = blockIdx.x * blockDim.x + threadIdx.x;
    if (i >= n) return;
    const double* q = recs + 12 * (size_t)i;
    out[i] = box_hit(v3(q[0], q[1], q[2]), v3(q[3], q[4], q[5]), v3(q[6], q[7], q[8]),
                     normalize(v3(q[9], q[10], q[11]))) ? 1 : 0;
}

__global__ __launch_bounds__(64) void k_trace_ray(DevScene sc, V3 o, V3 d, V3 light, int32_t* out_i, double* out_d) {
    if (threadIdx.x != 0 || blockIdx.x != 0) return;
    RResult r;
    uint32_t nn = 0, np = 0;
    const double reach = fmax(fabs(o.x), fmax(fabs(o.y), fabs(o.z))) + (double)sc.rc_ext;
    trace_mode_r_cand(sc, o, d, (float)(1e-5 * reach + 1e-30), r, nn, np);
    out_i[0] = r.ent;
    out_i[1] = out_i[2] = 0;
    for (int k = 0; k < 9; ++k) out_d[k] = 0;
    if (r.ent >= 0) {
        const REnt e = sc.ents[r.ent];
        int32_t u, v;
        tex_coord(sc, e, r.P, u, v);
        const V3 col = shade_ref(e, d, light, r.P, r.N, u, v);
        out_i[1] = u; out_i[2] = v;
        out_d[0] = r.P.x; out_d[1] = r.P.y; out_d[2] = r.P.z;
        out_d[3] = r.N.x; out_d[4] = r.N.y; out_d[5] = r.N.z;
        out_d[6] = col.x; out_d[7] = col.y; out_d[8] = col.z;
    }
}


}

long long shard_tiles(int w, int h, int shard_count) { return make_map(w, h, shard_count, 0).n_local; }

struct XEnv {
    int run_log2 = 0, help = 1, wf = -1, flat = 1;
    int r_flat = -1;
    int rf_per_slot = 16;
    int rf_group = 0;
};
const XEnv& x_env() {
    static XEnv env;
    static std::once_flag once;
    std::call_once(once, [] {
        if (const char* v = std::getenv("GI_X_HELP")) env.help = std::atoi(v) != 0;
        if (const char* v = std::getenv("GI_X_FLAT")) env.flat = std::atoi(v) != 0;
        if (const char* v = std::getenv("GI_R_FLAT")) env.r_flat = std::atoi(v);
        if (const char* v = std::getenv("GI_RF_PER_SLOT")) env.rf_per_slot = std::max(0, std::min(1024, std::atoi(v)));
        if (const char* v = std::getenv("GI_X_WF")) env.wf = std::atoi(v);
        if (const char* v = std::getenv("GI_RF_GROUP")) env.rf_group = (std::atoi(v) == 1 || std::atoi(v) == 4) ? std::atoi(v) : 0;
        const char* v = std::getenv("GI_X_MAX_RUN");
        const int r = v ? std::max(1, std::min(128, std::atoi(v))) : GI_X_MAX_RUN;
        int lg = 0;
        while ((2 << lg) <= r) ++lg;
        env.run_log2 = lg;
    });
    return env;
}

hipError_t launch_wf(const DevScene& sc, XVariant var, size_t lds_bytes, int resident, int form, const CamDev& cam, V3 light,
                     int w, int h, int y0, const gi_opts& o, double* rgb, uint8_t* rgb8, const XScratch& xs,
                     const unsigned* n_list_dev, unsigned long long* stats, int xflags, hipStream_t stream,
                     hipEvent_t ev_begin, hipEvent_t ev_end);
hipError_t wf_occupancy(const DevScene& sc, XVariant var, bool flat, size_t lds_bytes, int form, int* per_cu);
size_t wf_slot_bytes();
size_t wf_scene_lds_bytes(const DevScene& sc);

#ifndef GI_WF_MAX_DEPTH
#define GI_WF_MAX_DEPTH 64
#endif
int x_form_choice(const DevScene& sc, const XLaunchCfg& xc, const gi_opts& o) {
    if (o.mode != GI_MODE_X || (o.flags & GI_FLAG_X_MEGA)) return 0;
    if (o.flags & GI_FLAG_X_SEG) return 2;
    if (o.flags & GI_FLAG_X_WF) return o.depth <= GI_WF_MAX_DEPTH ? 1 : 0;
    const XEnv& env = x_env();
    if (env.wf >= 0) return env.wf == 1 ? (o.depth <= GI_WF_MAX_DEPTH ? 1 : 0) : env.wf == 2 ? 2 : 0;
    return (xc.var.lds || (size_t)sc.n_xwnodes * sizeof(XWNode) <= ((size_t)1 << 20)) ? 2 : 0;
}
long long x_wf_chunk() { return 8ll << 20; }
int x_env_rf_per_slot() { return x_env().rf_per_slot; }
unsigned rf_own_pairs() { return GI_RF_S0; }
unsigned rf_page_pairs() { return GI_RF_PAGE; }
unsigned rf_max_pages() { return GI_RF_KMAX; }
unsigned rf_seg_pairs() { return GI_RF_SEG; }
int r_kernel_choice(const DevScene& sc, const gi_opts& o) {
    if (o.mode != GI_MODE_R || (o.flags & GI_FLAG_R_DFS) || sc.n_rnodes <= 1) return 0;
    const XEnv& env = x_env();
    const bool large = env.r_flat >= 0 ? env.r_flat != 0 : sc.n_ents > 4096;
    if (!large) return 0;
    return (env.r_flat == 2 || (unsigned)sc.n_ents > kRfEntMask) ? 2 : 1;
}

template <typename F>
void x_dispatch(const DevScene& sc, bool help, bool stats, F&& f) {
    with_bools([&](auto S, auto HP, auto C, auto H, auto T) { f(&k_mode_x<S.value, HP.value, C.value, H.value, T.value>); },
               stats, help, sc.xcnodes != nullptr, sc.x_max_depth <= 7, sc.x_tri_only != 0);
}

hipError_t x_launch_config(const DevScene& sc, int device, XLaunchCfg& cfg) {
    const bool lds = sc.x_lds_bytes > 0;
    cfg.lds_bytes = 16 * 256 * sizeof(int) + 256 * (7 * sizeof(double) + 2 * sizeof(int));
    cfg.var.lds = lds;
    cfg.var.w4 = lds && sc.x_waves4;
    int cus = 0, per_cu = 0;
    hipError_t e = hipDeviceGetAttribute(&cus, hipDeviceAttributeMultiprocessorCount, device);
    if (e != hipSuccess) return e;
    x_dispatch(sc, false, false, [&](auto kernel) {
        e = hipOccupancyMaxActiveBlocksPerMultiprocessor(&per_cu, reinterpret_cast<const void*>(kernel), 64 * kWavesPerBlock,
                                                         cfg.lds_bytes);
    });
    if (e != hipSuccess) return e;
    cfg.resident = std::max(1, cus) * std::max(1, per_cu);
    cfg.wf_lds_bytes = (lds ? wf_scene_lds_bytes(sc) : 16 * 256 * sizeof(int)) + wf_slot_bytes();
    const bool flat = sc.x_flat && x_env().flat;
    e = wf_occupancy(sc, cfg.var, flat, cfg.wf_lds_bytes, 1, &per_cu);
    if (e != hipSuccess) return e;
    cfg.wf_resident = std::max(1, cus) * std::max(1, per_cu);
    e = wf_occupancy(sc, cfg.var, flat, cfg.wf_lds_bytes, 2, &per_cu);
    if (e != hipSuccess) return e;
    cfg.seg_resident = std::max(1, cus) * std::max(1, per_cu);
    e = wf_occupancy(sc, cfg.var, flat, cfg.wf_lds_bytes, 3, &per_cu);
    if (e != hipSuccess) return e;
    cfg.cast_resident = std::max(1, cus) * std::max(1, per_cu);
    e = wf_occupancy(sc, cfg.var, flat, cfg.wf_lds_bytes, 4, &per_cu);
    if (e != hipSuccess) return e;
    cfg.occl_resident = std::max(1, cus) * std::max(1, per_cu);
    e = wf_occupancy(sc, cfg.var, flat, cfg.wf_lds_bytes, 5, &per_cu);
    if (e != hipSuccess) return e;
    cfg.aov_resident = std::max(1, cus) * std::max(1, per_cu);
    return hipSuccess;
}

hipError_t launch_render(const DevScene& sc, const XLaunchCfg& xc, const CamDev& cam, V3 light, int w, int h, int y0,
                         const gi_opts& o, double* rgb, uint8_t* rgb8, const XScratch& xs, KTimer* kt,
                         hipStream_t stream) {
    const bool timed = (o.flags & GI_FLAG_TIME) && kt && kt->ev0[0];
    const int slot = timed ? (int)(kt->recorded % KTimer::kRing) : 0;
    hipEvent_t ev_begin = timed ? static_cast<hipEvent_t>(kt->ev0[slot]) : nullptr;
    hipEvent_t ev_end = timed ? static_cast<hipEvent_t>(kt->ev1[slot]) : nullptr;
    auto mark = [&](hipEvent_t ev) { if (timed) (void)hipEventRecord(ev, stream); };
    const TileMap m = make_map(w, h, o.shard_count, o.shard_index, y0);
    if (m.n_local == 0) return hipSuccess;
    const dim3 grid((unsigned)((m.n_local + kWavesPerBlock - 1) / kWavesPerBlock)), block(64 * kWavesPerBlock);
    unsigned long long* st = reinterpret_cast<unsigned long long*>(o.stats);
    const bool stats = (o.flags & GI_FLAG_STATS) && st;
    if (o.mode == GI_MODE_R) {
        const double reach = std::max(std::fabs(cam.pos.x), std::max(std::fabs(cam.pos.y), std::fabs(cam.pos.z))) + (double)sc.rc_ext;
        const float tau = (float)(1e-5 * reach + 1e-30);
        const int dfs = ((o.flags & GI_FLAG_R_DFS) || sc.n_rnodes <= 1) ? 1 : 0;
        const int rk = r_kernel_choice(sc, o);
        const bool tri = sc.r_tri_only != 0;
        mark(ev_begin);
        if (rk == 1 && xs.rf_pairs && xs.rf_slots >= m.n_local * (kTile * kTile)) {
            const RFlat f{xs.rf_pairs, xs.rf_pairs + (size_t)(xs.rf_slots / 64) * GI_RF_S0, xs.rf_pt, xs.rf_best, xs.rf_cnt,
                          xs.rf_ovf, xs.rf_rcnt, xs.rf_soff, xs.rf_shc, xs.rf_sreg, xs.rf_hoff, xs.rf_dir, xs.rf_pages};
            const dim3 pgrid((unsigned)((m.n_local * (kTile * kTile) + 255) / 256)), fgrid(4096);
            hipError_t e1 = hipMemsetAsync(xs.rf_cnt, 0, 2 * sizeof(unsigned), stream);
            if (e1 != hipSuccess) return e1;
            const dim3 bgrid((unsigned)std::min<long long>(2 * m.n_local, 2048));
            const dim3 hgrid(16384);
            const int rgroup = x_env().rf_group;
            with_bools([&](auto S, auto T) {
                hipLaunchKernelGGL(k_rf_walk<S.value>, pgrid, block, 0, stream, sc, cam, m, tau, f, st);
                hipLaunchKernelGGL(k_rf_scan, dim3(1), dim3(1024), 0, stream, f.rcnt, f.soff, nullptr, m.n_local, GI_RF_SEG);
                hipLaunchKernelGGL((k_rf_hit<S.value, T.value>), hgrid, dim3(64), 0, stream, sc, cam, m, f, st);
                hipLaunchKernelGGL(k_rf_scan, dim3(1), dim3(1024), 0, stream, f.shc, f.hoff, f.soff + m.n_local, 0ll, 1u);
                hipLaunchKernelGGL(k_rf_reach<S.value>, dim3(4 * fgrid.x), dim3(64), 0, stream, sc, cam, m, f, st, rgroup);
                hipLaunchKernelGGL((k_rf_shade<S.value, T.value>), pgrid, block, 0, stream, sc, cam, light, m, rgb, rgb8, f, st);
                hipLaunchKernelGGL((k_mode_r_batch<S.value, T.value>), bgrid, block, 0, stream, sc, cam, light, m, rgb, rgb8, st, tau,
                                   (const unsigned*)xs.rf_ovf, (const unsigned*)(xs.rf_cnt + 1));
            }, stats, tri);
        } else if (rk) {
            const dim3 sgrid((unsigned)((m.n_local * (kTile * kTile) + 31) / 32));
            with_bools([&](auto S, auto T) {
                hipLaunchKernelGGL((k_mode_r_batch<S.value, T.value>), sgrid, block, 0, stream, sc, cam, light, m, rgb, rgb8, st, tau, nullptr, nullptr);
            }, stats, tri);
        } else {
            with_bools([&](auto S) { hipLaunchKernelGGL(k_mode_r<S.value>, grid, block, 0, stream, sc, cam, light, m, rgb, rgb8, st, tau, dfs); },
                       stats);
        }
        mark(ev_end);
    } else {
        const XEnv& env = x_env();
        const long long n_slots = m.n_local * (kTile * kTile);
        const bool help = env.help && n_slots * (long long)o.spp <= 32ll * 256ll * (long long)xc.resident;
        const long long want = (n_slots * (long long)o.spp / 64 + kWavesPerBlock - 1) / kWavesPerBlock;
        const dim3 pgrid((unsigned)std::max<long long>(1, std::min<long long>(want, xc.resident)));
        if (!xs.list || (unsigned long long)xs.cap < (unsigned long long)n_slots || (o.spp > 1 && (!xs.part || xs.spp < o.spp)))
            return hipErrorInvalidValue;
        const int s0 = o.sample_end > 0 ? o.sample_begin : 0, s1 = o.sample_end > 0 ? o.sample_end : o.spp;
        const bool cont = s0 > 0;
        hipError_t e = hipMemsetAsync(sc.work, 0, (cont ? 1 : 16) * sizeof(unsigned), stream);
        if (e == hipSuccess && cont) e = hipMemsetAsync(sc.work + 2, 0, 14 * sizeof(unsigned), stream);
        if (e != hipSuccess) return e;
        XWork wk;
        wk.list = xs.list;
        wk.n_list = sc.work + 1;
        wk.part = xs.part;
        wk.blocks = sc.work;
        wk.s0 = s0;
        wk.s1 = s1;
        const dim3 sgrid((unsigned)((n_slots + 255) / 256));
        const dim3 cgrid((unsigned)((n_slots + kClassifyBlock - 1) / kClassifyBlock));
        const int form = x_form_choice(sc, xc, o);
        unsigned* zero2 = form == 2 ? xs.wcnt : nullptr;
        unsigned* cl = cont ? nullptr : xs.list;
        with_bools([&](auto S) {
            hipLaunchKernelGGL(k_x_classify<S.value>, cgrid, dim3(kClassifyBlock), 0, stream, sc, cam, m, s1 - s0, rgb, rgb8, cl, sc.work + 1, st, zero2);
        }, stats);
        const int h8 = sc.x_handle8;
        const int xf = sc.x_flags | (env.run_log2 << XF_RUN_SHIFT) | ((o.flags & GI_FLAG_X_NO_SHADOW) ? XF_NO_SHADOW : 0) |
                       (env.help ? XF_HANDOFF : 0) | (help ? XF_SPREAD : 0) | XF_PIXEL_MAJOR | (env.flat ? 0 : XF_NO_FLAT);
        if (form) {
            if (!xs.wcnt || (form == 1 && (!xs.wq[0] || !xs.wq[1] || xs.wcap <= 0))) return hipErrorInvalidValue;
            e = launch_wf(sc, xc.var, xc.wf_lds_bytes, form == 2 ? xc.seg_resident : xc.wf_resident, form, cam, light, w, h, y0,
                          o, rgb, rgb8, xs, sc.work + 1, stats ? st : nullptr, xf, stream, ev_begin, ev_end);
            if (e != hipSuccess) return e;
            if (o.spp > 1) hipLaunchKernelGGL(k_x_reduce, sgrid, dim3(256), 0, stream, m, wk, o.spp, rgb, rgb8);
            if (timed) kt->recorded++;
            return hipGetLastError();
        }
        mark(ev_begin);
        x_dispatch(sc, help, stats, [&](auto kernel) {
            hipLaunchKernelGGL(kernel, pgrid, block, xc.lds_bytes, stream, sc, cam, light, m, o.spp, o.depth, o.seed, rgb, rgb8, st, wk,
                               h8, xf);
        });
        mark(ev_end);
        if (o.spp > 1) hipLaunchKernelGGL(k_x_reduce, sgrid, dim3(256), 0, stream, m, wk, o.spp, rgb, rgb8);
    }
    if (timed) kt->recorded++;
    return hipGetLastError();
}

hipError_t launch_unshard(int w, int h, int shard_count, const double* packed, const uint8_t* packed8, double* rgb,
                          uint8_t* rgb8, hipStream_t stream) {
    const TileMap m = make_map(w, h, shard_count, 0);
    const long long n = m.n_tiles * kTile * kTile;
    hipLaunchKernelGGL(k_unshard, dim3((unsigned)((n + 255) / 256)), dim3(256), 0, stream, m, packed, packed8, rgb, rgb8);
    return hipGetLastError();
}

hipError_t launch_box_kat(int n, const double* recs, int32_t* out, hipStream_t stream) {
    if (n > 0) hipLaunchKernelGGL(k_box_kat, dim3((unsigned)((n + 255) / 256)), dim3(256), 0, stream, n, recs, out);
    return hipGetLastError();
}

hipError_t launch_x_query_kat(const DevScene& sc, XVariant var, bool flat, size_t lds_bytes, V3 cam_pos, int n,
                              const double* recs, int32_t* oi, double* od, hipStream_t stream);
void wf_variant(const DevScene& sc, XVariant var, bool flat, int32_t out[6]);
namespace {
struct XQueryCfg {
    XVariant var;
    size_t lds_bytes;
    bool flat;
};
XQueryCfg x_query_cfg(const XLaunchCfg& xc, int flags) {
    const bool hbm = (flags & 2) != 0 && xc.var.lds;
    return XQueryCfg{hbm ? XVariant{} : xc.var, hbm ? 16 * 256 * sizeof(int) + wf_slot_bytes() : xc.wf_lds_bytes,
                     x_env().flat && (flags & 1) == 0};
}
}
hipError_t launch_x_query(const DevScene& sc, const XLaunchCfg& xc, V3 cam_pos, int flags, int n, const double* recs,
                          int32_t* oi, double* od, hipStream_t stream) {
    const XQueryCfg c = x_query_cfg(xc, flags);
    return launch_x_query_kat(sc, c.var, c.flat, c.lds_bytes, cam_pos, n, recs, oi, od, stream);
}
void x_query_variant(const DevScene& sc, const XLaunchCfg& xc, int flags, int32_t out[6]) {
    const XQueryCfg c = x_query_cfg(xc, flags);
    wf_variant(sc, c.var, c.flat, out);
}

hipError_t launch_cast(const DevScene& sc, XVariant var, bool flat, size_t lds_bytes, int resident, bool any, const CastIO& io,
                       hipStream_t stream);
hipError_t launch_ray_query(const DevScene& sc, const XLaunchCfg& xc, bool any, const CastIO& io, hipStream_t stream) {
    const XQueryCfg c = x_query_cfg(xc, 0);
    return launch_cast(sc, c.var, c.flat, c.lds_bytes, any ? xc.occl_resident : xc.cast_resident, any, io, stream);
}

hipError_t launch_aov_kernel(const DevScene& sc, XVariant var, bool flat, size_t lds_bytes, int resident, const CamDev& cam,
                             const AovIO& io, hipStream_t stream);
hipError_t launch_aov(const DevScene& sc, const XLaunchCfg& xc, const CamDev& cam, const AovIO& io, hipStream_t stream) {
    const XQueryCfg c = x_query_cfg(xc, 0);
    return launch_aov_kernel(sc, c.var, c.flat, c.lds_bytes, xc.aov_resident, cam, io, stream);
}

hipError_t launch_trace_ray(const DevScene& sc, V3 o, V3 d, V3 light, int32_t* out_i, double* out_d, hipStream_t stream) {
    hipLaunchKernelGGL(k_trace_ray, dim3(1), dim3(64), 0, stream, sc, o, d, light, out_i, out_d);
    return hipGetLastError();
}

}
```

### 2019global_amd/csrc/gi_scene.h

```cpp
#pragma once
#include <stdint.h>
#include <type_traits>
#include <vector>

#include "gi_math.h"

namespace gi {

enum EntKind : int32_t { K_IMP_SPHERE = 1, K_IMP_TRIANGLE = 2, K_EXP_QUAD = 3, K_EXP_SPHERE = 4, K_EXP_CUBE = 5,
                         K_EXP_CONE = 6, K_EXP_RECTANGLE = 7, K_EXP_BOX = 8 };

struct RNode {
    double mn[3], mx[3];
    int32_t child0;
    int32_t parent;
    int32_t ent_off;
    int32_t ent_cnt;
};
static_assert(sizeof(RNode) == 64, "RNode layout");

struct RPathRec {
    double mn[3], mx[3];
    int32_t node;
    int32_t ent_cnt;
    int32_t pad[2];
};
static_assert(sizeof(RPathRec) == 64, "RPathRec layout");
struct RApp {
    int64_t rank;
    int32_t p0, p1;
};
static_assert(sizeof(RApp) == 16, "RApp layout");

struct REnt {
    int32_t kind, tri_first, tri_count, pad0;
    double pos[3];
    float radius, width, length, alpha;
    double qv0[3], qv1[3], qv2[3];
    double color[3], shader[3];
    double spec_pow;
    float height, pad1;
    double sin_theta;
    double refl;
};
static_assert(sizeof(REnt) == 208, "REnt layout");

struct XPrim {
    double a[3];
    double b[3];
    double c[3];
    double n[3];
    int32_t kind;
    int32_t ent;
    int32_t pad[2];
};
static_assert(sizeof(XPrim) == 112, "XPrim layout");

struct XNode {
    double mn[3], mx[3];
    int32_t child_base;
    int32_t child_mask;
    int32_t prim_off;
    int32_t prim_cnt;
};
static_assert(sizeof(XNode) == 64, "XNode layout");

constexpr int32_t XEMPTY = (int32_t)0x80000000;
struct XWNode {
    float lo[3][8];
    float hi[3][8];
    int32_t child[8];
    int32_t parent;
    uint16_t cnt[8];
    int32_t exists;
    int32_t pad[2];
};
static_assert(sizeof(XWNode) == 256, "XWNode layout");
struct XCNode {
    float org[3];
    int8_t ex[3];
    uint8_t exists;
    uint8_t qlo[3][8];
    uint8_t qhi[3][8];
    int32_t child[8];
    uint8_t cnt[8];
    int32_t parent;
    int32_t pad[5];
};
static_assert(sizeof(XCNode) == 128, "XCNode layout");
bool encode_xcnodes(const std::vector<XWNode>& w, std::vector<XCNode>& out);

struct XHot {
    double a[3], b[3], c[3];
    int32_t prim;
    int32_t kind;
};
static_assert(sizeof(XHot) == 80, "XHot layout");
struct XBox {
    float lo[3], hi[3];
    int32_t pad[2];
};
static_assert(sizeof(XBox) == 32, "XBox layout");
struct XLeaf {
    int32_t off, cnt;
};
#ifndef GI_XFLAT_MAX
#define GI_XFLAT_MAX 32
#endif
static_assert(GI_XFLAT_MAX >= 1 && GI_XFLAT_MAX <= 32, "the candidate mask is one 32-bit word");
struct XFlatLeaf {
    float lo[3], hi[3];
    int32_t off;
    uint16_t cnt;
    uint8_t group;
    uint8_t pad;
};
static_assert(sizeof(XFlatLeaf) == 32, "XFlatLeaf layout");

struct HostScene {
    std::vector<RNode> rnodes;
    std::vector<int32_t> leaf_ents;
    std::vector<REnt> ents;
    std::vector<TriRec> tris;
    int32_t max_depth = 0, n_leaves = 0, n_reachable = 0, n_dropped = 0;
    std::vector<XNode> xnodes;
    std::vector<XWNode> xwnodes;
    std::vector<XCNode> xcnodes;
    std::vector<XLeaf> xleaves;
    std::vector<int32_t> xprim_idx;
    std::vector<XHot> xhot;
    std::vector<XBox> xbox;
    std::vector<XPrim> xprims;
    int32_t x_max_depth = 0;
    std::vector<int32_t> app_off;
    std::vector<int32_t> app_leaf;
    std::vector<int64_t> app_rank;
    std::vector<int32_t> rpath_off;
    std::vector<int32_t> rpath;
    std::vector<RPathRec> rpath_rec;
    std::vector<RApp> app_rec;
    std::vector<XWNode> rc_nodes;
    std::vector<int32_t> rc_ent;
    std::vector<int64_t> rc_maxkey;
    std::vector<int32_t> r_always;
    std::vector<int32_t> r_leaf_of_rank;
    double rc_ext = 0;
    int32_t x_handle8 = 6;
    int32_t x_flags = 0;
    double x_est_nodes = 0, x_est_prims = 0;
    bool x_spatial = false;
    double x_skip_a = 0.0, x_skip_b = 2.0;
    std::vector<XFlatLeaf> xflat;
    bool x_flat_ok = false;
};
void build_xflat(HostScene& hs);

inline void finalize_xwnodes(std::vector<XWNode>& w) {
    for (XWNode& n : w) {
        n.exists = 0;
        for (int c = 0; c < 8; ++c)
            if (n.child[c] != XEMPTY) n.exists |= 1 << c;
    }
}

void build_xbvh(const std::vector<XPrim>& prims, const std::vector<double>& bounds, int leaf_max, HostScene& hs,
                bool geometric = false);
void build_rcand(HostScene& hs);

struct DevScene {
    const RNode* rnodes;
    const int32_t* leaf_ents;
    const REnt* ents;
    const TriRec* tris;
    const XWNode* xwnodes;
    const XCNode* xcnodes;
    const XHot* xhot;
    const XBox* xbox;
    const XPrim* xprims;
    unsigned* work;
    int32_t n_rnodes, n_ents, n_xwnodes, n_xprims;
    int32_t x_max_depth;
    int32_t x_handle8;
    int32_t x_flags;
    int32_t n_xhot;
    int32_t x_lds_bytes;
    int32_t x_waves4;
    int32_t x_tri_only;
    int32_t r_tri_only;
    float root_lo[3], root_hi[3];
    double x_skip_a, x_skip_b;
    const int32_t* app_off;
    const RApp* app_rec;
    const RPathRec* rpath_rec;
    const XWNode* rc_nodes;
    const int32_t* rc_ent;
    const int64_t* rc_maxkey;
    const int32_t* r_always;
    const int32_t* r_leaf_of_rank;
    int32_t n_r_always;
    float rc_ext;
    const XFlatLeaf* xflat;
    int32_t n_xflat;
    int32_t x_flat;
    float x_far_r;
};

struct KTimer {
    static constexpr int kRing = 64;
    void* ev0[kRing] = {};
    void* ev1[kRing] = {};
    long long recorded = 0;
    double sum_ms = 0.0;
    long long folded = 0;
};

struct XScratch {
    unsigned* list = nullptr;
    double* part = nullptr;
    long long cap = 0;
    int spp = 0;
    double* wq[2] = {nullptr, nullptr};
    unsigned* wid[2] = {nullptr, nullptr};
    unsigned* wcnt = nullptr;
    long long wcap = 0;
    unsigned* rf_pairs = nullptr;
    unsigned* rf_pt = nullptr;
    unsigned long long* rf_best = nullptr;
    double* rf_dir = nullptr;
    unsigned* rf_cnt = nullptr;
    unsigned* rf_ovf = nullptr;
    unsigned* rf_rcnt = nullptr;
    unsigned* rf_soff = nullptr;
    unsigned* rf_shc = nullptr;
    unsigned* rf_sreg = nullptr;
    unsigned* rf_hoff = nullptr;
    unsigned rf_pages = 0;
    long long rf_slots = 0;
    size_t rf_bytes = 0;
    long long rf_failed = 0;
};

enum XFlag : int {
    XF_INLINE_SHADOW = 1 << 0,
    XF_NO_SHADOW = 1 << 2,
    XF_HANDOFF = 1 << 3,
    XF_SPREAD = 1 << 4,
    XF_PIXEL_MAJOR = 1 << 5,
    XF_NO_FLAT = 1 << 6,
    XF_RUN_SHIFT = 8, XF_RUN_MASK = 7,
};

struct XVariant {
    bool lds = false;
    bool w4 = false;
};
template <bool STATS, bool LDS, bool W4, bool SH, bool TRI, bool CN, bool FLAT>
struct XTag {
    static constexpr bool stats = STATS, lds = LDS, w4 = W4, sh = SH, tri = TRI, cn = CN, flat = FLAT;
};
template <bool... Bs, typename F>
void with_bools(F&& f) {
    f(std::integral_constant<bool, Bs>{}...);
}
template <bool... Bs, typename F, typename... R>
void with_bools(F&& f, bool b, R... r) {
    if (b) with_bools<Bs..., true>(f, r...);
    else with_bools<Bs..., false>(f, r...);
}

struct XLaunchCfg {
    XVariant var;
    size_t lds_bytes = 0;
    int resident = 1;
    size_t wf_lds_bytes = 0;
    int wf_resident = 1;
    int seg_resident = 1;
    int cast_resident = 1;
    int occl_resident = 1;
    int aov_resident = 1;
};

struct CastIO {
    const double* rays;
    long long n;
    double* t;
    int32_t* prim;
    int32_t* ent;
    double* nrm;
    int32_t* occl;
};

struct AovIO {
    int x0, y0, cols, rows;
    double* t;
    double* nrm;
    double* alb;
    int32_t* prim;
    int32_t* ent;
    int32_t* uv;
};

}
```

### 2019global_amd/csrc/gi_wf.hip

```cpp
#include <hip/hip_runtime.h>

#include <algorithm>
#include <cstdlib>
#include <mutex>
#include <type_traits>

#include "gi.h"
#include "gi_dev.h"
#include "gi_scene.h"

namespace gi {
namespace {

constexpr long long kWfTile = 8;

#ifndef GI_WF_MIN_WAVES_LDS
#define GI_WF_MIN_WAVES_LDS 4
#endif
#ifndef GI_WF_MIN_WAVES
#define GI_WF_MIN_WAVES 3
#endif
#ifndef GI_WF_TAKE
#define GI_WF_TAKE 16
#endif
constexpr size_t kWfSlotBytes = 9 * 256 * sizeof(double);

struct PathId {
    uint64_t key;
    unsigned smp;
    int b;
};
__device__ __forceinline__ void slot_put_u64(double* pl, int f, uint64_t v) { reinterpret_cast<uint64_t*>(pl)[f * 256] = v; }
__device__ __forceinline__ uint64_t slot_get_u64(const double* pl, int f) { return reinterpret_cast<const uint64_t*>(pl)[f * 256]; }

struct WFQ {
    double* r;
    uint2* id;
    long long cap;
};

template <bool ANY, bool PAIR, bool AXIS, bool SH, bool TRI, bool NST, typename NodeP, typename HotP>
__device__ __forceinline__ int wf_trace(float far_r, NodeP W, HotP H, V3 o, V3 d, double tmax, bool act, int* nst, double& t_out,
                                        uint32_t& nnode, uint32_t& nprim, uint32_t& nsteps, int skip = 254) {
    constexpr bool kSkip = std::is_same<NodeP, const XWNode*>::value;
    const F3 of = ray_org32(o, d, far_r);
    const F3 ivf = inv_dir(d);
    const int dmask = (d.x < 0 ? 1 : 0) | (d.y < 0 ? 2 : 0) | (d.z < 0 ? 4 : 0);
    double tb = tmax;
    float tbf = up32(tmax);
    int best = -1;
    uint64_t mlo = 0, mhi = 0;
    int node = 0, level = 0;
    bool raying = false;
    if (act) {
        uint32_t rm;
        if constexpr (kSkip) rm = children_mask<AXIS, true>(W, of, ivf, tbf, dmask, skip);
        else rm = children_mask<AXIS>(W, of, ivf, tbf, dmask);
        lvl_set<SH>(mlo, mhi, 0, rm);
        raying = rm != 0;
    }
    while (raying) {
        ++nsteps;
        const auto* nd = W + node;
        const uint32_t msk = lvl_get<SH>(mlo, mhi, level);
        const int kc = __builtin_ctz(msk);
        lvl_set<SH>(mlo, mhi, level, msk & (msk - 1));
        const int c = kc ^ dmask;
        bool keep = true;
        if (!ANY && !NST && best >= 0) {
            keep = child_hit(nd, c, of, ivf, tbf);
        }
        const int ch = nd->child[c];
        if (keep) {
            if (ch < 0) {
                const int cnt = nd->cnt[c];
                const auto* hp = H + ~ch;
                if constexpr (PAIR) {
                    for (int j = 0; j < cnt; j += 2) {
                        const bool two = j + 1 < cnt;
                        const XHotR r0 = load_hot(hp + j), r1 = load_hot(hp + (two ? j + 1 : j));
                        const double ta = x_prim_t<TRI>(r0.h, o, d, MX_TMIN);
                        const double tq = two ? x_prim_t<TRI>(r1.h, o, d, MX_TMIN) : INFINITY;
                        nprim += two ? 2 : 1;
                        if (ANY) {
                            if ((ta < tmax) | (tq < tmax)) {
                                best = ta < tmax ? r0.h.prim : r1.h.prim;
                                break;
                            }
                        } else {
                            const bool ua = (ta < tb) | ((ta == tb) & (r0.h.prim < best));
                            tb = ua ? ta : tb;
                            best = ua ? r0.h.prim : best;
                            const bool uq = (tq < tb) | ((tq == tb) & (r1.h.prim < best));
                            tb = uq ? tq : tb;
                            best = uq ? r1.h.prim : best;
                            tbf = up32(tb);
                        }
                    }
                } else {
                    XHotR cur = load_hot(hp);
                    for (int j = 0; j < cnt; ++j) {
                        const XHotR rec = cur;
                        if (j + 1 < cnt) cur = load_hot(hp + j + 1);
                        ++nprim;
                        const double t = x_prim_t<TRI>(rec.h, o, d, MX_TMIN);
                        if (ANY) {
                            if (t < tmax) { best = rec.h.prim; break; }
                        } else {
                            const bool u = (t < tb) | ((t == tb) & (rec.h.prim < best));
                            tb = u ? t : tb;
                            best = u ? rec.h.prim : best;
                            tbf = u ? up32(t) : tbf;
                        }
                    }
                }
            } else {
                ++nnode;
                uint32_t cm;
                if constexpr (kSkip) cm = children_mask<AXIS, true>(W + ch, of, ivf, tbf, dmask, skip);
                else cm = children_mask<AXIS>(W + ch, of, ivf, tbf, dmask);
                if (cm) {
                    node = ch;
                    ++level;
                    lvl_set<SH>(mlo, mhi, level, cm);
                    if (NST) nst[level * 256] = ch;
                }
            }
        }
        if (ANY && best >= 0) break;
        uint32_t rest = lvl_get<SH>(mlo, mhi, level);
        if (rest == 0 && level > 0) {
            if constexpr (NST) {
                const uint64_t lm = level >= 8 ? mlo : mlo & ((1ull << (8 * level)) - 1);
                const uint64_t hm = level <= 8 ? 0ull : mhi & ((1ull << (8 * (level - 8))) - 1);
                level = hm ? 8 + (63 - __clzll((long long)hm)) / 8 : lm ? (63 - __clzll((long long)lm)) / 8 : 0;
                rest = lvl_get<SH>(mlo, mhi, level);
                node = level == 0 ? 0 : nst[level * 256];
            } else {
                do {
                    --level;
                    node = level == 0 ? 0 : W[node].parent;
                    rest = lvl_get<SH>(mlo, mhi, level);
                } while (rest == 0 && level > 0);
            }
        }
        raying = rest != 0;
    }
    t_out = tb;
    return best;
}

constexpr size_t kFlatPkBytes = GI_XFLAT_MAX * sizeof(uint32_t);
typedef uint32_t u32x8 __attribute__((ext_vector_type(8)));
__device__ __forceinline__ u32x8 flat_rec_uniform(const XFlatLeaf* tab, int k) {
    return *(const __attribute__((address_space(4))) u32x8*)(uintptr_t)(tab + k);
}
__device__ __forceinline__ uint32_t flat_pack(uint32_t off, int k, uint32_t w7) { return off | ((uint32_t)k << 16) | ((w7 & 0xFFu) << 24); }
__device__ __forceinline__ uint32_t flat_shift_in(uint32_t m, unsigned long long hm) {
    uint32_t r;
    asm("v_addc_co_u32 %0, vcc, %1, %1, %2" : "=v"(r) : "v"(m), "s"(hm) : "vcc");
    return r;
}
__device__ __forceinline__ int flat_key(float tn, int k) {
    int r;
    asm("v_bfi_b32 %0, 31, %1, %2" : "=v"(r) : "s"(k), "v"(tn));
    return r;
}
__device__ __forceinline__ int flat_med3(int a, int b, int c) { return max(min(a, b), min(max(a, b), c)); }
__device__ __forceinline__ float flat_key_floor(int e) { return __int_as_float(e & ~31); }
__device__ __forceinline__ uint32_t flat_pk_of(const uint32_t* pkw, int k) { return pkw[k]; }
__device__ __forceinline__ bool flat_hit(const XFlatLeaf* r, F3 no, F3 ivf, int sm, float tmax, uint32_t& pk, int k) {
    const int4* q = reinterpret_cast<const int4*>(r);
    const int4 a = q[0], b = q[1];
    const float lx = __int_as_float(a.x), ly = __int_as_float(a.y), lz = __int_as_float(a.z);
    const float hx = __int_as_float(a.w), hy = __int_as_float(b.x), hz = __int_as_float(b.y);
    const float nx = (sm & 1) ? hx : lx, fx = (sm & 1) ? lx : hx;
    const float ny = (sm & 2) ? hy : ly, fy = (sm & 2) ? ly : hy;
    const float nz = (sm & 4) ? hz : lz, fz = (sm & 4) ? lz : hz;
    const float tn = fmaxf(fmaxf(__builtin_fmaf(nx, ivf.x, no.x), __builtin_fmaf(ny, ivf.y, no.y)),
                           fmaxf(__builtin_fmaf(nz, ivf.z, no.z), 0.0f));
    const float tf = fminf(fminf(__builtin_fmaf(fx, ivf.x, no.x), __builtin_fmaf(fy, ivf.y, no.y)),
                           fminf(__builtin_fmaf(fz, ivf.z, no.z), tmax));
    pk = flat_pack((uint32_t)b.z, k, (uint32_t)b.w);
    return tn <= tf;
}
template <bool ANY, bool TRI>
__device__ __forceinline__ int wf_flat(float far_r, const XFlatLeaf* tab, const uint32_t* pkw, int n, const XHot* H, V3 o, V3 d, double tmax, bool act,
                                       double& t_out, uint32_t& nnode, uint32_t& nprim, uint32_t& nsteps, int skip) {
    const F3 of = ray_org32(o, d, far_r);
    const F3 ivf = inv_dir(d);
    const F3 no = neg_oiv(of, ivf);
    const int sm = iv_signs(ivf);
    const bool sx = (sm & 1) != 0, sy = (sm & 2) != 0, sz = (sm & 4) != 0;
    double tb = tmax;
    float tbf = up32(tmax);
    int best = -1;
    const float tfa = __builtin_canonicalizef(act ? tbf : -1.0f);
    constexpr int kNone = 0x7F800000;
    uint32_t m = 0, pk = 0;
    int e1 = kNone, e2 = kNone;
    auto step = [&](const u32x8 w, int k) {
        const float lx = __uint_as_float(w[0]), ly = __uint_as_float(w[1]), lz = __uint_as_float(w[2]);
        const float hx = __uint_as_float(w[3]), hy = __uint_as_float(w[4]), hz = __uint_as_float(w[5]);
        const float ax = __builtin_fmaf(lx, ivf.x, no.x), bx = __builtin_fmaf(hx, ivf.x, no.x);
        const float ay = __builtin_fmaf(ly, ivf.y, no.y), by = __builtin_fmaf(hy, ivf.y, no.y);
        const float az = __builtin_fmaf(lz, ivf.z, no.z), bz = __builtin_fmaf(hz, ivf.z, no.z);
        const float tn = fmaxf(fmaxf(sx ? bx : ax, sy ? by : ay), fmaxf(sz ? bz : az, 0.0f));
        const float tf = fminf(fminf(sx ? ax : bx, sy ? ay : by), fminf(sz ? az : bz, tfa));
        const bool in = tn <= tf, other = (int)((w[7] >> 16) & 0xFFu) != skip;
        m = flat_shift_in(m, __builtin_amdgcn_ballot_w64(in) & __builtin_amdgcn_ballot_w64(other));
        if (!ANY) {
            const int key = flat_key(tn, k);
            const int eh = (in & other) ? key : kNone;
            e2 = flat_med3(e1, e2, eh);
            e1 = min(e1, eh);
        }
    };
    int k0 = 0;
    for (; k0 + 4 <= n; k0 += 4) {
        const u32x8 w0 = flat_rec_uniform(tab, k0), w1 = flat_rec_uniform(tab, k0 + 1);
        const u32x8 w2 = flat_rec_uniform(tab, k0 + 2), w3 = flat_rec_uniform(tab, k0 + 3);
        step(w0, k0);
        step(w1, k0 + 1);
        step(w2, k0 + 2);
        step(w3, k0 + 3);
    }
#pragma unroll 1
    for (int k = k0; k < n; ++k) step(flat_rec_uniform(tab, k), k);
    if (act) nnode += (uint32_t)((n * (int)sizeof(XFlatLeaf) + 255) / 256);
    bool go = m != 0;
    if (go) {
        const int bit = (ANY || e1 == kNone) ? __builtin_ctz(m) : n - 1 - (e1 & 31);
        m &= ~(1u << bit);
        pk = flat_pk_of(pkw, n - 1 - bit);
    }
    while (go) {
        ++nsteps;
        const int cnt = (int)(pk >> 24);
        const XHot* hp = H + (pk & 0xFFFFu);
        for (int j = 0; j < cnt; j += 2) {
            const bool two = j + 1 < cnt;
            const XHotR r0 = load_hot(hp + j), r1 = load_hot(hp + (two ? j + 1 : j));
            const double ta = x_prim_t<TRI>(r0.h, o, d, MX_TMIN);
            const double tq = two ? x_prim_t<TRI>(r1.h, o, d, MX_TMIN) : INFINITY;
            nprim += two ? 2 : 1;
            if (ANY) {
                if ((ta < tmax) | (tq < tmax)) {
                    best = ta < tmax ? r0.h.prim : r1.h.prim;
                    break;
                }
            } else {
                const bool ua = (ta < tb) | ((ta == tb) & (r0.h.prim < best));
                tb = ua ? ta : tb;
                best = ua ? r0.h.prim : best;
                const bool uq = (tq < tb) | ((tq == tb) & (r1.h.prim < best));
                tb = uq ? tq : tb;
                best = uq ? r1.h.prim : best;
                tbf = up32(tb);
            }
        }
        go = false;
        if (ANY) {
            if (best < 0 && m != 0) {
                const int bit = __builtin_ctz(m);
                m &= m - 1;
                pk = flat_pk_of(pkw, n - 1 - bit);
                go = true;
            }
        } else {
            if (flat_key_floor(e2) > tbf) m = 0;
            while (m != 0) {
                const int bit = 31 - __builtin_clz(m);
                m &= ~(1u << bit);
                const int k = n - 1 - bit;
                if (flat_hit(tab + k, no, ivf, sm, tbf, pk, k)) {
                    go = true;
                    break;
                }
            }
        }
    }
    t_out = tb;
    return best;
}

struct WFArgs {
    const unsigned* list;
    const unsigned* n_list;
    double* part;
    unsigned* take;
    const unsigned* n_in;
    unsigned* n_out;
    unsigned long long u0, u1;
    unsigned s0, ns;
};

struct WFView {
    const XWNode* LW = nullptr;
    const XHot* LH = nullptr;
    const XPrim* XP = nullptr;
    const REnt* EN = nullptr;
    const XFlatLeaf* FT = nullptr;
    const uint32_t* FP = nullptr;
    int* nst = nullptr;
    double* pl = nullptr;
};
template <bool LDS, bool FLAT = false>
__device__ __forceinline__ WFView wf_stage(const DevScene& sc, int4* lds) {
    WFView v;
    v.XP = sc.xprims;
    v.EN = sc.ents;
    v.FT = sc.xflat;
    if constexpr (LDS) {
        const int nw = sc.n_xwnodes * (int)(sizeof(XWNode) / sizeof(int4));
        const int nh = sc.n_xhot * (int)(sizeof(XHot) / sizeof(int4));
        const int np = sc.n_xprims * (int)(sizeof(XPrim) / sizeof(int4));
        const int ne = sc.n_ents * (int)(sizeof(REnt) / sizeof(int4));
        const int4* gw = reinterpret_cast<const int4*>(sc.xwnodes);
        const int4* gh = reinterpret_cast<const int4*>(sc.xhot);
        const int4* gp = reinterpret_cast<const int4*>(sc.xprims);
        const int4* ge = reinterpret_cast<const int4*>(sc.ents);
        for (int i = threadIdx.x; i < nw; i += blockDim.x) lds[i] = gw[i];
        for (int i = threadIdx.x; i < nh; i += blockDim.x) lds[nw + i] = gh[i];
        for (int i = threadIdx.x; i < np; i += blockDim.x) lds[nw + nh + i] = gp[i];
        for (int i = threadIdx.x; i < ne; i += blockDim.x) lds[nw + nh + np + i] = ge[i];
        constexpr int nk = FLAT ? (int)(kFlatPkBytes / sizeof(int4)) : 0;
        if constexpr (FLAT) {
            uint32_t* pkw = reinterpret_cast<uint32_t*>(lds + nw + nh + np + ne);
            for (int i = threadIdx.x; i < sc.n_xflat; i += blockDim.x) pkw[i] = flat_pack((uint32_t)sc.xflat[i].off, i, (uint32_t)sc.xflat[i].cnt);
            v.FP = pkw;
        }
        __syncthreads();
        v.LW = reinterpret_cast<const XWNode*>(lds);
        v.LH = reinterpret_cast<const XHot*>(lds + nw);
        v.XP = reinterpret_cast<const XPrim*>(lds + nw + nh);
        v.EN = reinterpret_cast<const REnt*>(lds + nw + nh + np);
        v.pl = reinterpret_cast<double*>(lds + nw + nh + np + ne + nk) + threadIdx.x;
    } else {
        v.nst = reinterpret_cast<int*>(lds) + threadIdx.x;
        v.pl = reinterpret_cast<double*>(reinterpret_cast<int*>(lds) + 16 * 256) + threadIdx.x;
    }
    return v;
}

__device__ __forceinline__ V3 wf_primary(const CamDev& cam, const TileMap& m, unsigned ps, int spp, uint64_t seed,
                                         unsigned li, unsigned smp, long long& idx, uint64_t& key) {
    int x = 0, y = 0;
    slot_pixel(m, (long long)(ps >> 6), (int)(ps & 63), idx, x, y);
    y += m.y0;
    if (spp > 1) idx = (long long)li;
    key = mx_key(seed, (uint64_t)y * (uint64_t)m.w + (uint64_t)x);
    double jx = 0.0, jy = 0.0;
    if (spp > 1) {
        jx = mx_u01k(key, smp, 0xFFFF, 0);
        jy = mx_u01k(key, smp, 0xFFFF, 1);
    }
    return primary_dir(cam, (double)x + jx, (double)y + jy);
}
__device__ __forceinline__ bool wf_primary_misses(const DevScene& sc, const CamDev& cam, V3 d0) {
    const F3 iv0 = f3(__builtin_amdgcn_rcpf((float)d0.x), __builtin_amdgcn_rcpf((float)d0.y), __builtin_amdgcn_rcpf((float)d0.z));
    return !root_hit(sc, ray_org32(cam.pos, d0, ray_far_r(sc, cam.pos)), iv0);
}
__device__ __forceinline__ void wf_store(double* part, double* rgb, uint8_t* rgb8, int spp, long long idx, unsigned smp, V3 L) {
    if (spp > 1) {
        double* q = part + 3 * ((size_t)idx * (size_t)spp + (size_t)smp);
        q[0] = L.x; q[1] = L.y; q[2] = L.z;
    } else {
        const double c0 = smin((0.0 + L.x) / 1.0, 1.0), c1 = smin((0.0 + L.y) / 1.0, 1.0), c2 = smin((0.0 + L.z) / 1.0, 1.0);
        if (rgb) { rgb[3 * idx] = c0; rgb[3 * idx + 1] = c1; rgb[3 * idx + 2] = c2; }
        if (rgb8) quantize(c0, c1, c2, rgb8 + 3 * idx);
    }
}

struct WFSegStats {
    uint64_t it_c = 0, ln_c = 0, it_s = 0, ln_s = 0, segs = 0, live = 0, iters = 0;
    uint64_t cyc_c = 0, cyc_s = 0, cyc_sh = 0, cyc_ref = 0, cyc_all = 0;
};
__device__ __forceinline__ void wf_wave_steps(uint32_t n, uint64_t& it, uint64_t& ln) {
    uint32_t mx = n, sm = n;
    for (int off = 32; off > 0; off >>= 1) {
        mx = max(mx, (uint32_t)__shfl_xor(mx, off));
        sm += __shfl_xor(sm, off);
    }
    if ((threadIdx.x & 63) == 0) { it += mx; ln += sm; }
}
template <bool ANY, bool LDS, bool SH, bool TRI, bool CN, bool FLAT>
__device__ __forceinline__ int x_query(const DevScene& sc, const WFView& v, float far_r, const V3& o, const V3& d, double tmax,
                                       bool act, double& t_out, uint32_t& nnode, uint32_t& nprim, uint32_t& st_steps, int skip) {
    if constexpr (FLAT) return wf_flat<ANY, TRI>(far_r, v.FT, v.FP, sc.n_xflat, v.LH, o, d, tmax, act, t_out, nnode, nprim, st_steps, skip);
    else if constexpr (LDS) return wf_trace<ANY, true, false, SH, TRI, false>(far_r, v.LW, v.LH, o, d, tmax, act, v.nst, t_out, nnode, nprim, st_steps, skip);
    else if constexpr (CN) return wf_trace<ANY, false, false, SH, TRI, true>(far_r, sc.xcnodes, sc.xhot, o, d, tmax, act, v.nst, t_out, nnode, nprim, st_steps);
    else return wf_trace<ANY, false, false, SH, TRI, true>(far_r, sc.xwnodes, sc.xhot, o, d, tmax, act, v.nst, t_out, nnode, nprim, st_steps, skip);
}
__device__ __forceinline__ int x_own_plane(int pg, const V3& pn, const V3& dir, double skip_cos) {
    return (pg < 254 && fabs(dot(dir, pn)) >= skip_cos) ? pg : 254;
}
struct XHitFrame { V3 P, Ld, pn; double ldist; int pg; };
__device__ __forceinline__ XHitFrame x_hit_frame(const WFView& v, const V3& light, const V3& o, const V3& d, bool hit, int best, double t) {
    XHitFrame h{o, v3(0, 0, 1), v3(0, 0, 1), 0.0, 254};
    if (hit) {
        h.P = o + t * d;
        const V3 lv = light - h.P;
        h.ldist = gsqrt(dot(lv, lv));
        h.Ld = normalize(lv);
        const XPrim& px = v.XP[best];
        h.pg = px.pad[0] < 254 ? px.pad[0] : 254;
        h.pn = ld3(px.n);
    }
    return h;
}

template <bool STATS, bool LDS, bool SH, bool TRI, bool CN, bool FLAT, typename KeyF>
__device__ __forceinline__ bool x_segment(const DevScene& sc, const WFView& v, const V3& light, int depth, bool no_shadow, bool act,
                                          const KeyF& id_of, V3& o, V3& d, V3& L, V3& T,
                                          uint32_t& nnode, uint32_t& nprim, uint32_t& nrays, WFSegStats& ws,
                                          double skip_cos = 2.0, int* splane = nullptr, float far_r = INFINITY) {
    uint32_t st_steps = 0;
    uint64_t c0 = STATS ? clock64() : 0;
    bool occl = false;
    double tbest = INFINITY;
    const int skip_c = splane ? *splane : 254;
    const int best = x_query<false, LDS, SH, TRI, CN, FLAT>(sc, v, far_r, o, d, INFINITY, act, tbest, nnode, nprim, st_steps, skip_c);
    if (act) ++nrays;
    if (STATS) {
        wf_wave_steps(st_steps, ws.it_c, ws.ln_c);
        st_steps = 0;
        const uint64_t c1 = clock64();
        ws.cyc_c += c1 - c0;
        c0 = c1;
    }
    const bool hit = act && best >= 0;
    const XHitFrame h = x_hit_frame(v, light, o, d, hit, best, tbest);
    const V3 &P = h.P, &Ld = h.Ld;
    if (!no_shadow) {
        double tdummy;
        const int skip_s = x_own_plane(h.pg, h.pn, Ld, skip_cos);
        occl = x_query<true, LDS, SH, TRI, CN, FLAT>(sc, v, INFINITY, P, Ld, h.ldist, hit, tdummy, nnode, nprim, st_steps, skip_s) >= 0;
        if (STATS) wf_wave_steps(st_steps, ws.it_s, ws.ln_s);
    }
    if (STATS) {
        const uint64_t c1 = clock64();
        ws.cyc_s += c1 - c0;
        c0 = c1;
    }
    {
        L = v3(v.pl[0], v.pl[256], v.pl[512]);
        T = v3(v.pl[768], v.pl[1024], v.pl[1280]);
    }
    bool cont = false;
    if (hit) {
        ++nrays;
        const XPrim& p = v.XP[best];
        V3 N = (TRI || p.kind == 0) ? ld3(p.n) : normalize(P - ld3(p.a));
        N = dot(d, N) < 0 ? N : -N;
        const REnt& e = v.EN[p.ent];
        int32_t tu, tv;
        x_texcoord<TRI>(sc, e, P, tu, tv);
        const V3 tc = texel(ld3(e.color), tu, tv);
        const V3 la = tc * e.shader[0];
        V3 loc = la;
        if (!occl) {
            const V3 ldf = (smax(0.0, dot(N, Ld)) * (tc * 0.5)) * e.shader[1];
            const V3 bis = normalize(normalize(-d) + Ld);
            const double spw = mx_pow(smax(0.0, dot(N, bis)), e.spec_pow);
            const V3 ls = v3(spw, spw, spw) * e.shader[2];
            loc = (la + ldf) + ls;
        }
        L = L + vmul(T, v3(smin(loc.x, 1.0), smin(loc.y, 1.0), smin(loc.z, 1.0)));
        const PathId id = id_of();
        const uint64_t key = id.key;
        const unsigned smp = id.smp;
        const int b = id.b;
        if (b != depth - 1) {
            if (e.refl > 0.0 && mx_u01k(key, smp, b, 4) < e.refl) {
                d = normalize(d - N * (2.0 * dot(d, N)));
                cont = true;
            } else {
                T = vmul(T, tc * 0.5);
                if (!((T.x == 0.0) & (T.y == 0.0) & (T.z == 0.0))) {
                    double sx, sy, r2;
                    mx_disk(mx_u01k(key, smp, b, 2), mx_u01k(key, smp, b, 3), sx, sy, r2);
                    const double sz = gsqrt(1.0 - r2);
                    const double sg = N.z >= 0.0 ? 1.0 : -1.0;
                    const double aa = -1.0 / (sg + N.z);
                    const double bb = N.x * N.y * aa;
                    const V3 bt1 = v3(1.0 + sg * N.x * N.x * aa, sg * bb, -sg * N.x);
                    const V3 bt2 = v3(bb, sg + N.y * N.y * aa, -N.y);
                    d = normalize((bt1 * sx + bt2 * sy) + N * sz);
                    cont = true;
                }
            }
            o = P;
        }
        if (cont) {
            v.pl[0] = L.x; v.pl[256] = L.y; v.pl[512] = L.z;
            v.pl[768] = T.x; v.pl[1024] = T.y; v.pl[1280] = T.z;
            if (splane) *splane = x_own_plane(h.pg, h.pn, d, skip_cos);
        }
    }
    if (STATS) ws.cyc_sh += clock64() - c0;
    return cont;
}

template <bool STATS, bool LDS, bool W4, bool SH, bool TRI, bool CN, bool FLAT>
__global__ __launch_bounds__(256, (LDS && W4) ? GI_WF_MIN_WAVES_LDS : GI_WF_MIN_WAVES) void k_wf_bounce(
    DevScene sc, CamDev cam, V3 light, TileMap m, int spp, int depth, uint64_t seed, int b, double* rgb, uint8_t* rgb8,
    unsigned long long* stats, WFArgs a, WFQ qin, WFQ qout, int xflags) {
    unsigned n_in;
    if (b == 0) {
        const unsigned long long tot = (unsigned long long)*a.n_list * (unsigned long long)a.ns;
        n_in = (unsigned)(min(tot, a.u1) > a.u0 ? min(tot, a.u1) - a.u0 : 0ull);
    } else {
        n_in = *a.n_in;
    }
    if (*(volatile unsigned*)a.take >= n_in) return;
    extern __shared__ int4 lds_dyn[];
    const WFView v = wf_stage<LDS, FLAT>(sc, lds_dyn);
    const bool no_shadow = (xflags & XF_NO_SHADOW) != 0;
    const int lane = threadIdx.x & 63;
    uint32_t nnode = 0, nprim = 0, nrays = 0, nres = 0, npx = 0;
    const long long qc = qin.cap, oc = qout.cap;
    const unsigned take = (unsigned)max(1u, min((unsigned)GI_WF_TAKE, n_in / (64u * 8u * (gridDim.x * (blockDim.x >> 6)))));
    unsigned base = 0, left = 0;
    for (;;) {
        if (left == 0) {
            if (lane == 0) base = atomicAdd(a.take, 64u * take);
            base = __shfl(base, 0);
            left = take;
        }
        if (base >= n_in) break;
        const unsigned j = base + (unsigned)lane;
        base += 64u;
        --left;
        bool act = j < n_in;
        unsigned li = 0, smp = 0;
        V3 o = cam.pos, d = v3(1, 0, 0), L = v3(0, 0, 0), T = v3(1, 1, 1);
        long long idx = -1;
        uint64_t key = 0;
        if (act) {
            if (b == 0) {
                const unsigned long long u = a.u0 + j;
                if (u < (1ull << 32)) {
                    li = (unsigned)u / a.ns;
                    smp = a.s0 + ((unsigned)u - li * a.ns);
                } else {
                    li = (unsigned)(u / (unsigned long long)a.ns);
                    smp = a.s0 + (unsigned)(u - (unsigned long long)li * (unsigned long long)a.ns);
                }
            } else {
                const uint2 id = qin.id[j];
                li = id.x;
                smp = id.y;
                const double* r = qin.r + j;
                o = v3(r[0], r[qc], r[2 * qc]);
                d = v3(r[3 * qc], r[4 * qc], r[5 * qc]);
                L = v3(r[6 * qc], r[7 * qc], r[8 * qc]);
                T = v3(r[9 * qc], r[10 * qc], r[11 * qc]);
            }
            const V3 d0 = wf_primary(cam, m, a.list[li], spp, seed, li, smp, idx, key);
            if (b == 0) {
                if (smp == 0) ++npx;
                if (wf_primary_misses(sc, cam, d0)) {
                    ++nrays;
                    ++nres;
                    act = false;
                    wf_store(a.part, rgb, rgb8, spp, idx, smp, v3(0, 0, 0));
                } else {
                    d = normalize(d0);
                }
            }
            v.pl[0] = L.x; v.pl[256] = L.y; v.pl[512] = L.z;
            v.pl[768] = T.x; v.pl[1024] = T.y; v.pl[1280] = T.z;
        }
        WFSegStats ws;
        const double skip_cos = x_skip_cos(sc, cam.pos);
        const float far_r = ray_far_r(sc, cam.pos);
        int splane = 254;
        const bool cont = x_segment<false, LDS, SH, TRI, CN, FLAT>(sc, v, light, depth, no_shadow, act, [&] { return PathId{key, smp, b}; }, o, d, L, T,
                                                             nnode, nprim, nrays, ws, skip_cos, &splane, far_r);
        const unsigned long long mc = __ballot(cont);
        if (mc) {
            const int leader = __ffsll((long long)mc) - 1;
            unsigned ob = 0;
            if (lane == leader) ob = atomicAdd(a.n_out, (unsigned)__popcll(mc));
            ob = __shfl(ob, leader);
            if (cont) {
                const unsigned k = ob + (unsigned)__popcll(mc & ((1ull << lane) - 1));
                qout.id[k] = make_uint2(li, smp);
                double* r = qout.r + k;
                r[0] = o.x; r[oc] = o.y; r[2 * oc] = o.z;
                r[3 * oc] = d.x; r[4 * oc] = d.y; r[5 * oc] = d.z;
                r[6 * oc] = L.x; r[7 * oc] = L.y; r[8 * oc] = L.z;
                r[9 * oc] = T.x; r[10 * oc] = T.y; r[11 * oc] = T.z;
            }
        }
        if (act && !cont) wf_store(a.part, rgb, rgb8, spp, idx, smp, L);
    }
    if (STATS) {
        wave_add_stats(stats, nrays, nnode, nprim, npx);
        uint64_t r = nres;
        for (int off = 32; off > 0; off >>= 1) r += __shfl_xor(r, off);
        if (lane == 0 && r) atomicAdd(stats + GI_STAT_X_RESOLVED, (unsigned long long)r);
    }
}

#ifndef GI_SEG_BURST
#define GI_SEG_BURST 16
#endif
#ifndef GI_SEG_TAKE
#define GI_SEG_TAKE 2
#endif
#ifndef GI_SEG_TAKE_TRI
#define GI_SEG_TAKE_TRI 1
#endif
template <bool STATS, bool LDS, bool W4, bool SH, bool TRI, bool CN, bool FLAT>
__global__ __launch_bounds__(256, (LDS && W4) ? GI_WF_MIN_WAVES_LDS : GI_WF_MIN_WAVES) void k_seg(
    DevScene sc, CamDev cam, V3 light, TileMap m, int spp, int depth, uint64_t seed, double* rgb, uint8_t* rgb8,
    unsigned long long* stats, WFArgs a, int xflags) {
    extern __shared__ int4 lds_dyn[];
    const WFView v = wf_stage<LDS, FLAT>(sc, lds_dyn);
    const bool no_shadow = (xflags & XF_NO_SHADOW) != 0;
    const int lane = threadIdx.x & 63;
    const unsigned long long total = (unsigned long long)*a.n_list * (unsigned long long)a.ns;
    constexpr long long kTake = (LDS && TRI) ? GI_SEG_TAKE_TRI : GI_SEG_TAKE;
    const unsigned long long n_waves = (unsigned long long)gridDim.x * (blockDim.x >> 6);
    const unsigned long long run = 64ull * (unsigned long long)max(1ll, min(kTake, (long long)(total / (64ull * 8ull * n_waves))));
    uint32_t nnode = 0, nprim = 0, nrays = 0, nres = 0, npx = 0;
    unsigned long long cur = 0, cur_end = 0;
    bool exhausted = false;
    bool live = false;
    unsigned li = 0, smp = 0;
    long long idx = -1;
    uint64_t key = 0;
    V3 o = cam.pos, d = v3(1, 0, 0), L = v3(0, 0, 0), T = v3(1, 1, 1);
    int splane = 254;
    const double skip_cos = x_skip_cos(sc, cam.pos);
    const float far_r = ray_far_r(sc, cam.pos);
    WFSegStats ws;
    const uint64_t t_begin = STATS ? clock64() : 0;
    for (;;) {
        if (STATS && lane == 0) ++ws.iters;
        const uint64_t t_ref = STATS ? clock64() : 0;
        for (int burst = 0; burst < GI_SEG_BURST; ++burst) {
            const unsigned long long m_need = __ballot(!live);
            if (m_need == 0 || (exhausted && cur >= cur_end)) break;
            const unsigned rank = (unsigned)__popcll(m_need & ((1ull << lane) - 1));
            const unsigned n_need = (unsigned)__popcll(m_need);
            unsigned long long u = ~0ull;
            const unsigned long long avail = cur_end - cur;
            if (n_need > avail && !exhausted) {
                unsigned long long nb = 0;
                if (lane == 0) nb = atomicAdd(reinterpret_cast<unsigned long long*>(a.take), run);
                nb = __shfl(nb, 0);
                if (nb >= total) {
                    exhausted = true;
                    if (!live && rank < avail) u = cur + rank;
                    cur = cur_end;
                } else {
                    const unsigned long long ne = min(total, nb + run);
                    if (!live) {
                        if (rank < avail) u = cur + rank;
                        else if (nb + (rank - avail) < ne) u = nb + (rank - avail);
                    }
                    cur = min(ne, nb + (n_need - avail));
                    cur_end = ne;
                    if (ne == total) exhausted = true;
                }
            } else {
                if (!live && rank < avail) u = cur + rank;
                cur += min((unsigned long long)n_need, avail);
            }
            unsigned li_u = 0, smp_u = 0;
            if (u != ~0ull) {
                if (u < (1ull << 32)) {
                    li_u = (unsigned)u / a.ns;
                    smp_u = a.s0 + ((unsigned)u - li_u * a.ns);
                } else {
                    li_u = (unsigned)(u / (unsigned long long)a.ns);
                    smp_u = a.s0 + (unsigned)(u - (unsigned long long)li_u * (unsigned long long)a.ns);
                }
            }
            if (!live && u != ~0ull) {
                li = li_u;
                smp = smp_u;
                const unsigned ps = a.list[li];
                const V3 d0 = wf_primary(cam, m, ps, spp, seed, li, smp, idx, key);
                if (smp == 0) ++npx;
                if (wf_primary_misses(sc, cam, d0)) {
                    ++nrays;
                    ++nres;
                    wf_store(a.part, rgb, rgb8, spp, idx, smp, v3(0, 0, 0));
                } else {
                    live = true;
                    o = cam.pos;
                    d = normalize(d0);
                    splane = 254;
                    L = v3(0, 0, 0);
                    T = v3(1, 1, 1);
                    v.pl[0] = 0.0; v.pl[256] = 0.0; v.pl[512] = 0.0;
                    v.pl[768] = 1.0; v.pl[1024] = 1.0; v.pl[1280] = 1.0;
                    slot_put_u64(v.pl, 6, key);
                    slot_put_u64(v.pl, 7, (uint64_t)(uint32_t)idx | ((uint64_t)smp << 32));
                    slot_put_u64(v.pl, 8, 0ull);
                }
            }
        }
        if (STATS) ws.cyc_ref += clock64() - t_ref;
        if (__ballot(live) == 0) {
            if (exhausted && cur >= cur_end) break;
            continue;
        }
        if (STATS) {
            const unsigned long long ml = __ballot(live);
            if (lane == 0) { ++ws.segs; ws.live += __popcll(ml); }
        }
        const bool cont = x_segment<STATS, LDS, SH, TRI, CN, FLAT>(
            sc, v, light, depth, no_shadow, live,
            [&] { return PathId{slot_get_u64(v.pl, 6), (unsigned)(slot_get_u64(v.pl, 7) >> 32), (int)slot_get_u64(v.pl, 8)}; },
            o, d, L, T, nnode, nprim, nrays, ws, skip_cos, &splane, far_r);
        if (live) {
            if (cont) {
                slot_put_u64(v.pl, 8, slot_get_u64(v.pl, 8) + 1);
            } else {
                const uint64_t is = slot_get_u64(v.pl, 7);
                wf_store(a.part, rgb, rgb8, spp, (long long)(uint32_t)is, (unsigned)(is >> 32), L);
                live = false;
            }
        }
    }
    if (STATS && lane == 0) {
        atomicAdd(stats + GI_STAT_X_ITERS, (unsigned long long)ws.iters);
        atomicAdd(stats + GI_STAT_X_HANDLE, (unsigned long long)ws.segs);
        atomicAdd(stats + GI_STAT_X_HLANES, (unsigned long long)ws.live);
        atomicAdd(stats + GI_STAT_X_IT_LEAF, (unsigned long long)ws.it_c);
        atomicAdd(stats + GI_STAT_X_LN_LEAF, (unsigned long long)ws.ln_c);
        atomicAdd(stats + GI_STAT_X_IT_NODE, (unsigned long long)ws.it_s);
        atomicAdd(stats + GI_STAT_X_LN_NODE, (unsigned long long)ws.ln_s);
        atomicAdd(stats + GI_STAT_X_CYC_TRAV, (unsigned long long)(ws.cyc_c + ws.cyc_s));
        atomicAdd(stats + GI_STAT_X_IT_RS, (unsigned long long)ws.cyc_c);
        atomicAdd(stats + GI_STAT_X_CYC_HIT, (unsigned long long)ws.cyc_sh);
        atomicAdd(stats + GI_STAT_X_CYC_NEXT, (unsigned long long)ws.cyc_ref);
        atomicAdd(stats + GI_STAT_X_CYC_ALL, (unsigned long long)(clock64() - t_begin));
    }
    if (STATS) {
        wave_add_stats(stats, nrays, nnode, nprim, npx);
        uint64_t r = nres;
        for (int off = 32; off > 0; off >>= 1) r += __shfl_xor(r, off);
        if (lane == 0 && r) atomicAdd(stats + GI_STAT_X_RESOLVED, (unsigned long long)r);
    }
}

template <bool LDS, bool W4, bool SH, bool TRI, bool CN, bool FLAT>
__global__ __launch_bounds__(256, (LDS && W4) ? GI_WF_MIN_WAVES_LDS : GI_WF_MIN_WAVES) void k_x_query_kat(
    DevScene sc, V3 cam_pos, int n, const double* recs, int32_t* oi, double* od) {
    extern __shared__ int4 lds_dyn[];
    const WFView v = wf_stage<LDS, FLAT>(sc, lds_dyn);
    const long long i = (long long)blockIdx.x * 256 + threadIdx.x;
    const bool act = i < (long long)n;
    const double skip_cos = x_skip_cos(sc, cam_pos);
    const float far_r = ray_far_r(sc, cam_pos);
    V3 o = v3(0, 0, 0), d = v3(1, 0, 0), light = v3(0, 0, 0), d2 = v3(1, 0, 0);
    if (act) {
        const double* q = recs + 12 * i;
        o = v3(q[0], q[1], q[2]);
        d = v3(q[3], q[4], q[5]);
        light = v3(q[6], q[7], q[8]);
        d2 = v3(q[9], q[10], q[11]);
    }
    uint32_t nnode = 0, nprim = 0, st_steps = 0;
    double t1 = INFINITY;
    const int p1 = x_query<false, LDS, SH, TRI, CN, FLAT>(sc, v, far_r, o, d, INFINITY, act, t1, nnode, nprim, st_steps, 254);
    const bool hit = act && p1 >= 0;
    const XHitFrame h = x_hit_frame(v, light, o, d, hit, p1, t1);
    double tdummy;
    const int skip_s = x_own_plane(h.pg, h.pn, h.Ld, skip_cos);
    const int sb = x_query<true, LDS, SH, TRI, CN, FLAT>(sc, v, INFINITY, h.P, h.Ld, h.ldist, hit, tdummy, nnode, nprim, st_steps, skip_s);
    const int skip2 = x_own_plane(h.pg, h.pn, d2, skip_cos);
    double t2 = INFINITY;
    const int p2 = x_query<false, LDS, SH, TRI, CN, FLAT>(sc, v, far_r, h.P, d2, INFINITY, hit, t2, nnode, nprim, st_steps, skip2);
    if (act) {
        oi[5 * i] = p1 >= 0 ? p1 : -1;
        oi[5 * i + 1] = hit ? (sb >= 0 ? 1 : 0) : -1;
        oi[5 * i + 2] = skip_s;
        oi[5 * i + 3] = (hit && p2 >= 0) ? p2 : -1;
        oi[5 * i + 4] = skip2;
        od[2 * i] = p1 >= 0 ? t1 : INFINITY;
        od[2 * i + 1] = (hit && p2 >= 0) ? t2 : INFINITY;
    }
    if (i == 0) od[2 * (long long)n] = skip_cos;
}

template <bool ANY, bool LDS, bool W4, bool SH, bool TRI, bool CN, bool FLAT>
__global__ __launch_bounds__(256, (LDS && W4) ? GI_WF_MIN_WAVES_LDS : GI_WF_MIN_WAVES) void k_cast(DevScene sc, CastIO io) {
    extern __shared__ int4 lds_dyn[];
    const WFView v = wf_stage<LDS, FLAT>(sc, lds_dyn);
    const int lane = threadIdx.x & 63;
    const long long stride = 64ll * (long long)gridDim.x * (long long)(blockDim.x >> 6);
    for (long long base = 64ll * ((long long)blockIdx.x * (blockDim.x >> 6) + (threadIdx.x >> 6)); base < io.n; base += stride) {
        const long long i = base + lane;
        const bool in = i < io.n;
        V3 o = v3(0, 0, 0), d = v3(1, 0, 0);
        double tmax = INFINITY;
        bool act = false;
        if (in) {
            const double2* q = reinterpret_cast<const double2*>(io.rays) + 4 * i;
            const double2 q0 = q[0], q1 = q[1], q2 = q[2], q3 = q[3];
            const V3 ro = v3(q0.x, q0.y, q1.x), rd = v3(q1.y, q2.x, q2.y);
            const bool fin = __builtin_isfinite(ro.x) & __builtin_isfinite(ro.y) & __builtin_isfinite(ro.z) &
                             __builtin_isfinite(rd.x) & __builtin_isfinite(rd.y) & __builtin_isfinite(rd.z);
            const bool nz = (rd.x != 0.0) | (rd.y != 0.0) | (rd.z != 0.0);
            act = fin & nz & (q3.x > MX_TMIN);
            if (act) {
                o = ro;
                d = rd;
                tmax = q3.x;
            }
        }
        uint32_t nnode = 0, nprim = 0, nsteps = 0;
        double tb = INFINITY;
        const int best = x_query<ANY, LDS, SH, TRI, CN, FLAT>(sc, v, sc.x_far_r, o, d, tmax, act, tb, nnode, nprim, nsteps, 254);
        const bool hit = act && best >= 0;
        if constexpr (ANY) {
            if (in) io.occl[i] = hit ? 1 : 0;
        } else {
            if (in) {
                if (io.t) io.t[i] = hit ? tb : INFINITY;
                if (io.prim) io.prim[i] = hit ? best : -1;
                if (io.ent || io.nrm) {
                    int ent = -1;
                    V3 N = v3(0, 0, 0);
                    if (hit) {
                        const XPrim& p = v.XP[best];
                        ent = p.ent;
                        const V3 P = o + tb * d;
                        N = (TRI || p.kind == 0) ? ld3(p.n) : normalize(P - ld3(p.a));
                        N = dot(d, N) < 0 ? N : -N;
                    }
                    if (io.ent) io.ent[i] = ent;
                    if (io.nrm) {
                        double* q = io.nrm + 3 * i;
                        q[0] = N.x; q[1] = N.y; q[2] = N.z;
                    }
                }
            }
        }
    }
}

__host__ __device__ inline long long aov_batches(int cols, int rows) { return ((long long)cols * (long long)rows + 63) / 64; }
__device__ __forceinline__ bool aov_pixel(int cols, int rows, long long b, int lane, int& px, int& py) {
    const long long i = 64 * b + lane;
    if (i < (1ll << 32)) {
        const unsigned q = (unsigned)i / (unsigned)cols;
        py = (int)q;
        px = (int)((unsigned)i - q * (unsigned)cols);
    } else {
        const long long q = i / (long long)cols;
        py = (int)q;
        px = (int)(i - q * (long long)cols);
    }
    return i < (long long)cols * (long long)rows;
}

template <bool LDS, bool W4, bool SH, bool TRI, bool CN, bool FLAT>
__global__ __launch_bounds__(256, (LDS && W4) ? GI_WF_MIN_WAVES_LDS : GI_WF_MIN_WAVES) void k_aov(DevScene sc, CamDev cam, AovIO io) {
    extern __shared__ int4 lds_dyn[];
    const WFView v = wf_stage<LDS, FLAT>(sc, lds_dyn);
    const int lane = threadIdx.x & 63;
    const float far_r = ray_far_r(sc, cam.pos);
    const long long n_batches = aov_batches(io.cols, io.rows);
    const long long stride = (long long)gridDim.x * (long long)(blockDim.x >> 6);
    const bool want_tex = io.alb || io.uv;
    for (long long b = (long long)blockIdx.x * (blockDim.x >> 6) + (threadIdx.x >> 6); b < n_batches; b += stride) {
        int px = 0, py = 0;
        const bool in = aov_pixel(io.cols, io.rows, b, lane, px, py);
        const V3 o = cam.pos;
        V3 d = v3(1, 0, 0);
        bool act = false;
        if (in) {
            const V3 d0 = primary_dir(cam, (double)(io.x0 + px), (double)(io.y0 + py));
            if (!wf_primary_misses(sc, cam, d0)) {
                act = true;
                d = normalize(d0);
            }
        }
        uint32_t nnode = 0, nprim = 0, nsteps = 0;
        double tb = INFINITY;
        const int best = x_query<false, LDS, SH, TRI, CN, FLAT>(sc, v, far_r, o, d, INFINITY, act, tb, nnode, nprim, nsteps, 254);
        const bool hit = act && best >= 0;
        if (in) {
            const long long i = (long long)py * (long long)io.cols + (long long)px;
            int ent = -1, tu = 0, tv = 0;
            V3 N = v3(0, 0, 0), tc = v3(0, 0, 0);
            if (hit) {
                const XPrim& p = v.XP[best];
                ent = p.ent;
                const V3 P = o + tb * d;
                N = (TRI || p.kind == 0) ? ld3(p.n) : normalize(P - ld3(p.a));
                N = dot(d, N) < 0 ? N : -N;
                if (want_tex) {
                    const REnt& e = v.EN[p.ent];
                    x_texcoord<TRI>(sc, e, P, tu, tv);
                    tc = texel(ld3(e.color), tu, tv);
                }
            }
            if (io.t) io.t[i] = hit ? tb : INFINITY;
            if (io.prim) io.prim[i] = hit ? best : -1;
            if (io.ent) io.ent[i] = ent;
            if (io.nrm) {
                double* q = io.nrm + 3 * i;
                q[0] = N.x; q[1] = N.y; q[2] = N.z;
            }
            if (io.alb) {
                double* q = io.alb + 3 * i;
                q[0] = tc.x; q[1] = tc.y; q[2] = tc.z;
            }
            if (io.uv) {
                int32_t* q = io.uv + 2 * i;
                q[0] = tu; q[1] = tv;
            }
        }
    }
}

__global__ __launch_bounds__(256) void k_cam_rays(CamDev cam, int x0, int y0, int cols, int rows, double* rays) {
    const long long n_batches = aov_batches(cols, rows);
    const long long stride = (long long)gridDim.x * (long long)(blockDim.x >> 6);
    const int lane = threadIdx.x & 63;
    for (long long b = (long long)blockIdx.x * (blockDim.x >> 6) + (threadIdx.x >> 6); b < n_batches; b += stride) {
        int px = 0, py = 0;
        if (!aov_pixel(cols, rows, b, lane, px, py)) continue;
        const V3 d = normalize(primary_dir(cam, (double)(x0 + px), (double)(y0 + py)));
        double2* q = reinterpret_cast<double2*>(rays) + 4 * (64 * b + lane);
        q[0] = make_double2(cam.pos.x, cam.pos.y);
        q[1] = make_double2(cam.pos.z, d.x);
        q[2] = make_double2(d.y, d.z);
        q[3] = make_double2(INFINITY, 0.0);
    }
}

}

size_t wf_slot_bytes() { return kWfSlotBytes; }
size_t wf_scene_lds_bytes(const DevScene& sc) { return (size_t)sc.x_lds_bytes + (sc.x_flat ? kFlatPkBytes : 0); }

template <typename F>
void wf_dispatch(const DevScene& sc, XVariant var, bool flat, bool stats, F&& f) {
    if (var.lds && flat && sc.x_flat)
        with_bools([&](auto S, auto W) { f(XTag<S.value, true, W.value, true, W.value, false, true>{}); }, stats, var.w4);
    else if (var.lds)
        with_bools([&](auto S, auto W, auto H) { f(XTag<S.value, true, W.value, H.value, W.value, false, false>{}); },
                   stats, var.w4, sc.x_max_depth <= 7);
    else
        with_bools([&](auto S, auto T, auto C) { f(XTag<S.value, false, false, false, T.value, C.value, false>{}); },
                   stats, sc.x_tri_only != 0, sc.xcnodes != nullptr);
}
template <typename V>
constexpr auto seg_kernel(V) { return &k_seg<V::stats, V::lds, V::w4, V::sh, V::tri, V::cn, V::flat>; }
template <typename V>
constexpr auto bounce_kernel(V) { return &k_wf_bounce<V::stats, V::lds, V::w4, V::sh, V::tri, V::cn, V::flat>; }

template <bool ANY, typename V>
constexpr auto cast_kernel(V) { return &k_cast<ANY, V::lds, V::w4, V::sh, V::tri, V::cn, V::flat>; }

template <typename V>
constexpr auto aov_kernel(V) { return &k_aov<V::lds, V::w4, V::sh, V::tri, V::cn, V::flat>; }

hipError_t wf_occupancy(const DevScene& sc, XVariant var, bool flat, size_t lds_bytes, int form, int* per_cu) {
    hipError_t e = hipSuccess;
    wf_dispatch(sc, var, flat, false, [&](auto V) {
        const void* f = form == 5   ? reinterpret_cast<const void*>(aov_kernel(V))
                        : form == 4 ? reinterpret_cast<const void*>(cast_kernel<true>(V))
                        : form == 3 ? reinterpret_cast<const void*>(cast_kernel<false>(V))
                        : form == 2 ? reinterpret_cast<const void*>(seg_kernel(V))
                                    : reinterpret_cast<const void*>(bounce_kernel(V));
        e = hipOccupancyMaxActiveBlocksPerMultiprocessor(per_cu, f, 256, lds_bytes);
    });
    return e;
}

hipError_t launch_wf(const DevScene& sc, XVariant var, size_t lds_bytes, int resident, int form, const CamDev& cam, V3 light,
                     int w, int h, int y0, const gi_opts& o, double* rgb, uint8_t* rgb8, const XScratch& xs,
                     const unsigned* n_list_dev, unsigned long long* stats, int xflags, hipStream_t stream,
                     hipEvent_t ev_begin, hipEvent_t ev_end) {
    const TileMap m = make_map(w, h, o.shard_count, o.shard_index, y0);
    const int depth = o.depth;
    const int s0 = o.sample_end > 0 ? o.sample_begin : 0, s1 = o.sample_end > 0 ? o.sample_end : o.spp;
    const dim3 grid((unsigned)std::max(1, resident)), block(256);
    hipError_t e = hipSuccess;
    const bool flat = (xflags & XF_NO_FLAT) == 0;
    if (form == 2) {
        WFArgs a{};
        a.list = xs.list;
        a.n_list = n_list_dev;
        a.part = xs.part;
        a.take = xs.wcnt;
        a.s0 = (unsigned)s0;
        a.ns = (unsigned)(s1 - s0);
        if (ev_begin) (void)hipEventRecord(ev_begin, stream);
        wf_dispatch(sc, var, flat, stats != nullptr, [&](auto V) {
            hipLaunchKernelGGL(seg_kernel(V), grid, block, lds_bytes, stream, sc, cam, light, m, o.spp, depth, o.seed, rgb, rgb8, stats, a, xflags);
        });
        if (ev_end) (void)hipEventRecord(ev_end, stream);
        return hipGetLastError();
    }
    const unsigned long long units = (unsigned long long)m.n_local * (unsigned long long)(kWfTile * kWfTile) *
                                     (unsigned long long)(s1 - s0);
    if (ev_begin) (void)hipEventRecord(ev_begin, stream);
    for (unsigned long long u0 = 0; u0 < units; u0 += (unsigned long long)xs.wcap) {
        e = hipMemsetAsync(xs.wcnt, 0, 2 * (size_t)depth * sizeof(unsigned), stream);
        if (e != hipSuccess) return e;
        for (int b = 0; b < depth; ++b) {
            WFArgs a;
            a.list = xs.list;
            a.n_list = n_list_dev;
            a.part = xs.part;
            a.take = xs.wcnt + 2 * b;
            a.n_in = b > 0 ? xs.wcnt + 2 * (b - 1) + 1 : nullptr;
            a.n_out = xs.wcnt + 2 * b + 1;
            a.u0 = u0;
            a.u1 = std::min(units, u0 + (unsigned long long)xs.wcap);
            a.s0 = (unsigned)s0;
            a.ns = (unsigned)(s1 - s0);
            WFQ qin, qout;
            qin.cap = qout.cap = xs.wcap;
            qin.r = xs.wq[(b + 1) & 1];
            qin.id = reinterpret_cast<uint2*>(xs.wid[(b + 1) & 1]);
            qout.r = xs.wq[b & 1];
            qout.id = reinterpret_cast<uint2*>(xs.wid[b & 1]);
            wf_dispatch(sc, var, flat, stats != nullptr, [&](auto V) {
                hipLaunchKernelGGL(bounce_kernel(V), grid, block, lds_bytes, stream, sc, cam, light, m, o.spp, depth, o.seed, b, rgb, rgb8, stats, a, qin, qout, xflags);
            });
        }
    }
    if (ev_end) (void)hipEventRecord(ev_end, stream);
    return hipGetLastError();
}

hipError_t launch_x_query_kat(const DevScene& sc, XVariant var, bool flat, size_t lds_bytes, V3 cam_pos, int n,
                              const double* recs, int32_t* oi, double* od, hipStream_t stream) {
    if (n <= 0) return hipSuccess;
    const dim3 grid((unsigned)(((long long)n + 255) / 256)), block(256);
    wf_dispatch(sc, var, flat, false, [&](auto V) {
        using T = decltype(V);
        hipLaunchKernelGGL((k_x_query_kat<T::lds, T::w4, T::sh, T::tri, T::cn, T::flat>), grid, block, lds_bytes, stream, sc, cam_pos, n, recs, oi, od);
    });
    return hipGetLastError();
}

hipError_t launch_cast(const DevScene& sc, XVariant var, bool flat, size_t lds_bytes, int resident, bool any, const CastIO& io,
                       hipStream_t stream) {
    if (io.n <= 0) return hipSuccess;
    const long long want = (io.n + 255) / 256;
    const dim3 grid((unsigned)std::max<long long>(1, std::min<long long>(want, resident))), block(256);
    wf_dispatch(sc, var, flat, false, [&](auto V) {
        if (any) hipLaunchKernelGGL(cast_kernel<true>(V), grid, block, lds_bytes, stream, sc, io);
        else hipLaunchKernelGGL(cast_kernel<false>(V), grid, block, lds_bytes, stream, sc, io);
    });
    return hipGetLastError();
}

hipError_t launch_aov_kernel(const DevScene& sc, XVariant var, bool flat, size_t lds_bytes, int resident, const CamDev& cam,
                             const AovIO& io, hipStream_t stream) {
    if (io.cols <= 0 || io.rows <= 0) return hipSuccess;
    const long long want = (aov_batches(io.cols, io.rows) + 3) / 4;
    const dim3 grid((unsigned)std::max<long long>(1, std::min<long long>(want, resident))), block(256);
    wf_dispatch(sc, var, flat, false, [&](auto V) {
        hipLaunchKernelGGL(aov_kernel(V), grid, block, lds_bytes, stream, sc, cam, io);
    });
    return hipGetLastError();
}

hipError_t launch_cam_rays(const CamDev& cam, int x0, int y0, int cols, int rows, double* rays, hipStream_t stream) {
    if (cols <= 0 || rows <= 0) return hipSuccess;
    const long long want = ((long long)cols * (long long)rows + 255) / 256;
    const dim3 grid((unsigned)std::min<long long>(want, 2048)), block(256);
    hipLaunchKernelGGL(k_cam_rays, grid, block, 0, stream, cam, x0, y0, cols, rows, rays);
    return hipGetLastError();
}

void wf_variant(const DevScene& sc, XVariant var, bool flat, int32_t out[6]) {
    wf_dispatch(sc, var, flat, false, [&](auto V) {
        out[0] = V.lds; out[1] = V.w4; out[2] = V.sh; out[3] = V.tri; out[4] = V.cn; out[5] = V.flat;
    });
}

}
```

### include/gi.h

```cpp
#ifndef GI_H_
#define GI_H_

#include <stddef.h>
#include <stdint.h>

#ifdef __cplusplus
extern "C" {
#endif

#define GI_ABI_VERSION 13

typedef enum gi_status {
    GI_OK = 0,
    GI_ERR_ARG = -1,
    GI_ERR_DEVICE = -2,
    GI_ERR_SCENE = -3,
    GI_ERR_CANCELLED = -4,
    GI_ERR_NOMEM = -5,
    GI_ERR_INTERNAL = -6
} gi_status;

typedef enum gi_entity_kind {
    GI_IMP_SPHERE = 1,
    GI_IMP_TRIANGLE = 2,
    GI_EXP_QUAD = 3,
    GI_EXP_SPHERE = 4,
    GI_EXP_CUBE = 5,
    GI_EXP_CONE = 6,
    GI_EXP_RECTANGLE = 7,
    GI_EXP_BOX = 8
} gi_entity_kind;

typedef struct gi_entity_desc {
    int32_t kind;
    int32_t has_material;
    double args[11];
    double mat_color[3];
    double mat_shader[3];
    double mat_specular_power;
    double mat_reflectivity;
} gi_entity_desc;

typedef struct gi_scene_desc {
    double octree_min[3];
    double octree_max[3];
    int32_t n_entities;
    const gi_entity_desc* entities;
} gi_scene_desc;

typedef struct gi_camera {
    double pos[3];
    double up[3];
    double forward[3];
    double focal;
} gi_camera;

typedef enum gi_mode {
    GI_MODE_R = 0,
    GI_MODE_X = 1
} gi_mode;

#define GI_FLAG_STATS 1u
#define GI_FLAG_R_DFS 2u
#define GI_FLAG_TIME 4u
#define GI_FLAG_X_NO_SHADOW 8u
#define GI_FLAG_X_WF 16u
#define GI_FLAG_X_MEGA 32u
#define GI_FLAG_X_SEG 64u

typedef struct gi_opts {
    int32_t mode;
    int32_t spp;
    int32_t depth;
    int32_t shard_count;
    int32_t shard_index;
    int32_t band_rows;
    uint32_t flags;
    int32_t reserved;
    uint64_t seed;
    uint64_t* stats;
    int32_t sample_begin;
    int32_t sample_end;
} gi_opts;

#define GI_STAT_RAYS 0
#define GI_STAT_NODES 1
#define GI_STAT_PRIMS 2
#define GI_STAT_PIXELS 3
#define GI_STAT_X_PATH_MAX 4
#define GI_STAT_X_ITERS 5
#define GI_STAT_X_TRAV 6
#define GI_STAT_X_HANDLE 7
#define GI_STAT_X_HLANES 8
#define GI_STAT_X_HCLOSE 9
#define GI_STAT_X_HSHADOW 10
#define GI_STAT_X_CYC_TRAV 11
#define GI_STAT_X_CYC_HIT 12
#define GI_STAT_X_CYC_NEXT 13
#define GI_STAT_X_CYC_ALL 14
#define GI_STAT_X_RESOLVED 15
#define GI_STAT_X_IT_NODE 16
#define GI_STAT_X_LN_NODE 17
#define GI_STAT_X_IT_LEAF 18
#define GI_STAT_X_LN_LEAF 19
#define GI_STAT_X_IT_RS 20
#define GI_STAT_X_LN_RS 21
#define GI_STAT_X_IT_ST 22
#define GI_STAT_X_LN_ST 23
#define GI_STAT_R_PAIRS 24
#define GI_STAT_R_OVF_TILES 25
#define GI_STATS_N 26

#define GI_TILE 8

typedef struct gi_scene gi_scene;

typedef struct gi_scene_info {
    int32_t n_entities;
    int32_t n_nodes;
    int32_t n_leaves;
    int32_t max_depth;
    int32_t n_reachable;
    int32_t n_dropped;
    int32_t x_nodes;
    int32_t x_prims;
    int64_t device_bytes;
    int32_t x_node_bytes;
    int32_t x_lds_resident;
} gi_scene_info;

typedef struct gi_hit {
    int32_t entity;
    int32_t u, v;
    double point[3], normal[3];
} gi_hit;

typedef void (*gi_tile_cb)(void* user, int y0, int rows, const uint8_t* rgb8_rows, const double* rgb_rows);

int gi_abi_version(void);
const char* gi_last_error(void);
int gi_device_count(void);
int gi_device_list(int32_t* out, int cap);
const char* gi_build_id(void);

int gi_camera_init(const double pos[3], const double look_at[3], double focal, gi_camera* out);

int gi_scene_create(const gi_scene_desc* desc, gi_scene** out);
void gi_scene_destroy(gi_scene* scene);
int gi_scene_get_info(const gi_scene* scene, gi_scene_info* info);

int gi_render(gi_scene* scene, const gi_camera* cam, const double light[3], int w, int h,
              const gi_opts* opts, double* rgb, uint8_t* rgb8, const volatile int* cancel,
              gi_tile_cb cb, void* user);

int gi_render_device(gi_scene* scene, const gi_camera* cam, const double light[3], int w, int h,
                     const gi_opts* opts, double* d_rgb, uint8_t* d_rgb8, void* stream);

int64_t gi_shard_tiles(int w, int h, int shard_count);

int gi_unshard_device(int w, int h, int shard_count, const double* d_packed, const uint8_t* d_packed8,
                      double* d_rgb, uint8_t* d_rgb8, void* stream);

int gi_trace_ray(gi_scene* scene, const double origin[3], const double dir[3], const double light[3],
                 gi_hit* hit, double rgb[3]);

#define GI_RAY_DOUBLES 8
int gi_intersect_device(gi_scene* scene, int64_t n, const double* d_rays, double* d_t, int32_t* d_prim,
                        int32_t* d_entity, double* d_normal, void* stream);
int gi_occluded_device(gi_scene* scene, int64_t n, const double* d_rays, int32_t* d_occluded, void* stream);
int gi_intersect(gi_scene* scene, int64_t n, const double* rays, double* t, int32_t* prim, int32_t* entity,
                 double* normal);
int gi_occluded(gi_scene* scene, int64_t n, const double* rays, int32_t* occluded);

typedef struct gi_aov_frame { int32_t w, h, x0, y0, x1, y1; } gi_aov_frame;
typedef struct gi_aov { double* t; double* normal; double* albedo; int32_t* prim; int32_t* entity; int32_t* uv; } gi_aov;
int gi_render_aov_device(gi_scene* scene, const gi_camera* cam, const gi_aov_frame* frame, const gi_aov* d_out,
                         void* stream);
int gi_render_aov(gi_scene* scene, const gi_camera* cam, const gi_aov_frame* frame, const gi_aov* out);
int gi_camera_rays_device(const gi_camera* cam, const gi_aov_frame* frame, double* d_rays, void* stream);
int gi_camera_rays(const gi_camera* cam, const gi_aov_frame* frame, double* rays);

int gi_scene_kernel_ms(gi_scene* scene, float* avg_ms, int64_t* n);
int gi_scene_x_form(gi_scene* scene, const gi_opts* opts, int32_t* form);
int gi_scene_r_kernel(gi_scene* scene, const gi_opts* opts, int32_t* kernel);

typedef struct gi_octree gi_octree;
int gi_octree_create(const gi_scene_desc* desc, gi_octree** out);
void gi_octree_destroy(gi_octree* octree);
int gi_octree_intersect(const gi_octree* octree, const double origin[3], const double dir[3], int32_t* out,
                        int64_t cap, int64_t* n);

typedef struct gi_multi gi_multi;
int gi_multi_create(const gi_scene_desc* desc, int n_shards, const int* devices, gi_multi** out);
void gi_multi_destroy(gi_multi* multi);
int gi_multi_info(const gi_multi* multi, int* n_shards, int* n_devices, int* uses_rccl);
int gi_multi_render(gi_multi* multi, const gi_camera* cam, const double light[3], int w, int h, const gi_opts* opts,
                    double* rgb, uint8_t* rgb8, const volatile int* cancel, gi_tile_cb cb, void* user);

int gi_obj_parse(const char* text, int64_t len, const gi_entity_desc* tmpl, gi_entity_desc* out, int64_t cap,
                 int64_t* n);

int gi_kat_expbox(int n, const double* recs, int32_t* out);

int gi_kat_x_query(gi_scene* scene, int n, const double* recs, const double cam_pos[3], int flags, int32_t* prim1,
                   double* t1, int32_t* occl, int32_t* skip_s, int32_t* prim2, double* t2, int32_t* skip2,
                   double* skip_cos);
int gi_kat_x_variant(gi_scene* scene, int flags, int32_t out[6]);

#ifdef __cplusplus
}
#endif
#endif
```

Before: 32320.

## Add LDS ring for batched primary-ray refill in segmented path kernel

Adds a per-wave LDS ring to the segmented wavefront kernel. Batches of primary camera rays are generated ahead and the ones that miss are resolved immediately, so idle lanes refill from a compacted queue of surviving rays. The path bounce counter moves from an LDS slot into the upper bits of the splane register, which shrinks the per-thread slot from 9 to 8 doubles. In flat mode the kernel also stops staging the wide tree nodes into LDS. The ring is enabled only when occupancy does not drop, at the cost of extra LDS, wave barriers and more complex control flow.

Result: faster. 35490, median of 6 (+9.8%).

```diff
diff --git a/2019global_amd/__init__.py b/2019global_amd/__init__.py
--- a/2019global_amd/__init__.py
+++ b/2019global_amd/__init__.py
@@ -40,7 +40,7 @@
 STAT_R_PAIRS, STAT_R_OVF_TILES = 24, 25
 STATS_N = 26
 TILE = 8
-ABI_VERSION = 13
+ABI_VERSION = 14
 RAY_DOUBLES = 8
 AOV_OUTPUTS = ("t", "normal", "albedo", "prim", "entity", "uv")
 _AOV_KINDS = {"t": (np.float64, ()), "normal": (np.float64, (3,)), "albedo": (np.float64, (3,)),
@@ -101,7 +101,7 @@
 
 EXPORTS = ["gi_abi_version", "gi_last_error", "gi_camera_init", "gi_scene_create", "gi_scene_destroy",
            "gi_scene_get_info", "gi_render", "gi_render_device", "gi_shard_tiles", "gi_unshard_device",
-           "gi_trace_ray", "gi_kat_expbox", "gi_kat_x_query", "gi_kat_x_variant", "gi_scene_kernel_ms", "gi_scene_x_form", "gi_scene_r_kernel", "gi_octree_create", "gi_octree_destroy",
+           "gi_trace_ray", "gi_kat_expbox", "gi_kat_x_query", "gi_kat_x_variant", "gi_scene_kernel_ms", "gi_scene_x_form", "gi_scene_seg_ring", "gi_scene_r_kernel", "gi_octree_create", "gi_octree_destroy",
            "gi_octree_intersect", "gi_multi_create", "gi_multi_destroy", "gi_multi_info", "gi_multi_render", "gi_device_count",
            "gi_device_list", "gi_build_id", "gi_obj_parse", "gi_intersect", "gi_occluded", "gi_intersect_device",
            "gi_occluded_device", "gi_render_aov", "gi_render_aov_device", "gi_camera_rays", "gi_camera_rays_device"]
@@ -152,6 +152,7 @@
         L.gi_camera_rays_device.argtypes = [ctypes.POINTER(CameraDesc), ctypes.POINTER(AovFrame), vp, vp]
         L.gi_scene_kernel_ms.argtypes = [vp, ctypes.POINTER(ctypes.c_float), ctypes.POINTER(ctypes.c_int64)]
         L.gi_scene_x_form.argtypes = [vp, ctypes.POINTER(Opts), ctypes.POINTER(ctypes.c_int32)]
+        L.gi_scene_seg_ring.argtypes = [vp, ctypes.POINTER(Opts), ctypes.POINTER(ctypes.c_int32)]
         L.gi_scene_r_kernel.argtypes = [vp, ctypes.POINTER(Opts), ctypes.POINTER(ctypes.c_int32)]
         L.gi_octree_create.argtypes = [ctypes.POINTER(SceneDesc), ctypes.POINTER(vp)]
         L.gi_octree_destroy.argtypes = [vp]
@@ -491,6 +492,12 @@
         _check(lib().gi_scene_x_form(self._h, ctypes.byref(o), ctypes.byref(f)), "gi_scene_x_form")
         return X_FORMS[f.value]
 
+    def seg_ring(self, mode=MODE_X, spp=1, depth=1, flags=0) -> bool:
+        o = self.opts(mode, spp, depth, 0, flags=flags)
+        f = ctypes.c_int32()
+        _check(lib().gi_scene_seg_ring(self._h, ctypes.byref(o), ctypes.byref(f)), "gi_scene_seg_ring")
+        return bool(f.value)
+
     def r_kernel(self, flags=0) -> str:
         o = self.opts(MODE_R, 1, 1, 0, flags=flags)
         k = ctypes.c_int32()
diff --git a/2019global_amd/build.py b/2019global_amd/build.py
--- a/2019global_amd/build.py
+++ b/2019global_amd/build.py
@@ -17,7 +17,7 @@
 
 HOST_SRCS = ["gi_build.cpp", "gi_bvh.cpp", "gi_capi.cpp", "gi_multi.cpp", "gi_obj.cpp"]
 DEV_SRCS = ["gi_kernels.hip", "gi_wf.hip"]
-HEADERS = ["gi_math.h", "gi_scene.h", "gi_internal.h", "gi_dev.h"]
+HEADERS = ["gi_math.h", "gi_scene.h", "gi_internal.h", "gi_dev.h", "gi_seg_ring.h"]
 
 COMMON = ["-std=c++17", "-fPIC", "-ffp-contract=off", "-fno-fast-math", f"-I{INCLUDE}", f"-I{CSRC}"]
 
diff --git a/2019global_amd/csrc/gi_capi.cpp b/2019global_amd/csrc/gi_capi.cpp
--- a/2019global_amd/csrc/gi_capi.cpp
+++ b/2019global_amd/csrc/gi_capi.cpp
@@ -725,6 +725,15 @@
     });
 }
 
+int gi_scene_seg_ring(gi_scene* s, const gi_opts* o, int32_t* on) {
+    return guard([&]() -> int {
+        if (!s || !o || !on) return fail(GI_ERR_ARG, "null argument");
+        std::lock_guard<std::mutex> lk(s->mu);
+        *on = (x_form_choice(s->dev, s->xcfg, *o) == 2 && s->xcfg.seg_ring) ? 1 : 0;
+        return GI_OK;
+    });
+}
+
 int gi_scene_r_kernel(gi_scene* s, const gi_opts* o, int32_t* kernel) {
     return guard([&]() -> int {
         if (!s || !o || !kernel) return fail(GI_ERR_ARG, "null argument");
diff --git a/2019global_amd/csrc/gi_kernels.hip b/2019global_amd/csrc/gi_kernels.hip
--- a/2019global_amd/csrc/gi_kernels.hip
+++ b/2019global_amd/csrc/gi_kernels.hip
@@ -1812,7 +1812,7 @@
 long long shard_tiles(int w, int h, int shard_count) { return make_map(w, h, shard_count, 0).n_local; }
 
 struct XEnv {
-    int run_log2 = 0, help = 1, wf = -1, flat = 1;
+    int run_log2 = 0, help = 1, wf = -1, flat = 1, seg_ring = 1;
     int r_flat = -1;
     int rf_per_slot = 16;
     int rf_group = 0;
@@ -1823,6 +1823,7 @@
     std::call_once(once, [] {
         if (const char* v = std::getenv("GI_X_HELP")) env.help = std::atoi(v) != 0;
         if (const char* v = std::getenv("GI_X_FLAT")) env.flat = std::atoi(v) != 0;
+        if (const char* v = std::getenv("GI_SEG_RING")) env.seg_ring = std::atoi(v) != 0;
         if (const char* v = std::getenv("GI_R_FLAT")) env.r_flat = std::atoi(v);
         if (const char* v = std::getenv("GI_RF_PER_SLOT")) env.rf_per_slot = std::max(0, std::min(1024, std::atoi(v)));
         if (const char* v = std::getenv("GI_X_WF")) env.wf = std::atoi(v);
@@ -1842,7 +1843,8 @@
                      hipEvent_t ev_begin, hipEvent_t ev_end);
 hipError_t wf_occupancy(const DevScene& sc, XVariant var, bool flat, size_t lds_bytes, int form, int* per_cu);
 size_t wf_slot_bytes();
-size_t wf_scene_lds_bytes(const DevScene& sc);
+size_t wf_scene_lds_bytes(const DevScene& sc, bool flat);
+size_t wf_seg_ring_bytes();
 
 #ifndef GI_WF_MAX_DEPTH
 #define GI_WF_MAX_DEPTH 64
@@ -1889,14 +1891,20 @@
     });
     if (e != hipSuccess) return e;
     cfg.resident = std::max(1, cus) * std::max(1, per_cu);
-    cfg.wf_lds_bytes = (lds ? wf_scene_lds_bytes(sc) : 16 * 256 * sizeof(int)) + wf_slot_bytes();
     const bool flat = sc.x_flat && x_env().flat;
+    cfg.wf_lds_bytes = (lds ? wf_scene_lds_bytes(sc, flat) : 16 * 256 * sizeof(int)) + wf_slot_bytes();
+    cfg.wf_tree_lds_bytes = (lds ? wf_scene_lds_bytes(sc, false) : 16 * 256 * sizeof(int)) + wf_slot_bytes();
     e = wf_occupancy(sc, cfg.var, flat, cfg.wf_lds_bytes, 1, &per_cu);
     if (e != hipSuccess) return e;
     cfg.wf_resident = std::max(1, cus) * std::max(1, per_cu);
     e = wf_occupancy(sc, cfg.var, flat, cfg.wf_lds_bytes, 2, &per_cu);
     if (e != hipSuccess) return e;
     cfg.seg_resident = std::max(1, cus) * std::max(1, per_cu);
+    int per_cu_ring = 0;
+    e = wf_occupancy(sc, cfg.var, flat, cfg.wf_lds_bytes + wf_seg_ring_bytes(), 6, &per_cu_ring);
+    if (e != hipSuccess) return e;
+    cfg.seg_ring = x_env().seg_ring && per_cu_ring >= per_cu && per_cu >= 1;
+    cfg.seg_lds_bytes = cfg.wf_lds_bytes + (cfg.seg_ring ? wf_seg_ring_bytes() : 0);
     e = wf_occupancy(sc, cfg.var, flat, cfg.wf_lds_bytes, 3, &per_cu);
     if (e != hipSuccess) return e;
     cfg.cast_resident = std::max(1, cus) * std::max(1, per_cu);
@@ -1988,10 +1996,11 @@
         }, stats);
         const int h8 = sc.x_handle8;
         const int xf = sc.x_flags | (env.run_log2 << XF_RUN_SHIFT) | ((o.flags & GI_FLAG_X_NO_SHADOW) ? XF_NO_SHADOW : 0) |
-                       (env.help ? XF_HANDOFF : 0) | (help ? XF_SPREAD : 0) | XF_PIXEL_MAJOR | (env.flat ? 0 : XF_NO_FLAT);
+                       (env.help ? XF_HANDOFF : 0) | (help ? XF_SPREAD : 0) | XF_PIXEL_MAJOR | (env.flat ? 0 : XF_NO_FLAT) |
+                       (xc.seg_ring ? XF_SEG_RING : 0);
         if (form) {
             if (!xs.wcnt || (form == 1 && (!xs.wq[0] || !xs.wq[1] || xs.wcap <= 0))) return hipErrorInvalidValue;
-            e = launch_wf(sc, xc.var, xc.wf_lds_bytes, form == 2 ? xc.seg_resident : xc.wf_resident, form, cam, light, w, h, y0,
+            e = launch_wf(sc, xc.var, form == 2 ? xc.seg_lds_bytes : xc.wf_lds_bytes, form == 2 ? xc.seg_resident : xc.wf_resident, form, cam, light, w, h, y0,
                           o, rgb, rgb8, xs, sc.work + 1, stats ? st : nullptr, xf, stream, ev_begin, ev_end);
             if (e != hipSuccess) return e;
             if (o.spp > 1) hipLaunchKernelGGL(k_x_reduce, sgrid, dim3(256), 0, stream, m, wk, o.spp, rgb, rgb8);
@@ -2034,8 +2043,9 @@
 };
 XQueryCfg x_query_cfg(const XLaunchCfg& xc, int flags) {
     const bool hbm = (flags & 2) != 0 && xc.var.lds;
-    return XQueryCfg{hbm ? XVariant{} : xc.var, hbm ? 16 * 256 * sizeof(int) + wf_slot_bytes() : xc.wf_lds_bytes,
-                     x_env().flat && (flags & 1) == 0};
+    const bool flat = x_env().flat && (flags & 1) == 0;
+    return XQueryCfg{hbm ? XVariant{} : xc.var,
+                     hbm ? 16 * 256 * sizeof(int) + wf_slot_bytes() : flat ? xc.wf_lds_bytes : xc.wf_tree_lds_bytes, flat};
 }
 }
 hipError_t launch_x_query(const DevScene& sc, const XLaunchCfg& xc, V3 cam_pos, int flags, int n, const double* recs,
diff --git a/2019global_amd/csrc/gi_scene.h b/2019global_amd/csrc/gi_scene.h
--- a/2019global_amd/csrc/gi_scene.h
+++ b/2019global_amd/csrc/gi_scene.h
@@ -247,6 +247,7 @@
     XF_SPREAD = 1 << 4,
     XF_PIXEL_MAJOR = 1 << 5,
     XF_NO_FLAT = 1 << 6,
+    XF_SEG_RING = 1 << 7,
     XF_RUN_SHIFT = 8, XF_RUN_MASK = 7,
 };
 
@@ -273,8 +274,11 @@
     size_t lds_bytes = 0;
     int resident = 1;
     size_t wf_lds_bytes = 0;
+    size_t wf_tree_lds_bytes = 0;
     int wf_resident = 1;
     int seg_resident = 1;
+    bool seg_ring = false;
+    size_t seg_lds_bytes = 0;
     int cast_resident = 1;
     int occl_resident = 1;
     int aov_resident = 1;
diff --git a/2019global_amd/csrc/gi_seg_ring.h b/2019global_amd/csrc/gi_seg_ring.h
--- /dev/null
+++ b/2019global_amd/csrc/gi_seg_ring.h
@@ -0,0 +1,50 @@
+#ifndef GI_SEG_RING_H_
+#define GI_SEG_RING_H_
+
+#include "gi_math.h"
+
+namespace gi {
+
+constexpr unsigned kSegBatch = 64;
+
+struct SegUnits {
+    unsigned long long cur = 0, cur_end = 0;
+    bool exhausted = false;
+    unsigned head = 0, count = 0;
+
+    GI_HD bool units_left() const { return !(exhausted && cur >= cur_end); }
+    GI_HD bool done() const { return !units_left() && count == 0; }
+    GI_HD bool wants_batch(unsigned n_need) const { return n_need != 0 && count == 0 && units_left(); }
+    GI_HD bool wants_run() const { return cur >= cur_end && !exhausted; }
+    GI_HD void give_run(unsigned long long nb, unsigned long long run, unsigned long long total) {
+        if (nb >= total) {
+            exhausted = true;
+        } else {
+            cur = nb;
+            cur_end = nb + run < total ? nb + run : total;
+            if (cur_end == total) exhausted = true;
+        }
+    }
+    GI_HD unsigned take_batch(unsigned long long& first) {
+        const unsigned long long left = cur_end > cur ? cur_end - cur : 0ull;
+        const unsigned n = left < kSegBatch ? (unsigned)left : kSegBatch;
+        first = cur;
+        cur += n;
+        return n;
+    }
+    GI_HD void push(unsigned n_hit) {
+        head = 0;
+        count = n_hit;
+    }
+    GI_HD unsigned pop(unsigned n_need, unsigned& first) {
+        const unsigned k = n_need < count ? n_need : count;
+        first = head;
+        head += k;
+        count -= k;
+        return k;
+    }
+};
+
+}
+
+#endif
diff --git a/2019global_amd/csrc/gi_wf.hip b/2019global_amd/csrc/gi_wf.hip
--- a/2019global_amd/csrc/gi_wf.hip
+++ b/2019global_amd/csrc/gi_wf.hip
@@ -8,6 +8,7 @@
 #include "gi.h"
 #include "gi_dev.h"
 #include "gi_scene.h"
+#include "gi_seg_ring.h"
 
 namespace gi {
 namespace {
@@ -23,7 +24,10 @@
 #ifndef GI_WF_TAKE
 #define GI_WF_TAKE 16
 #endif
-constexpr size_t kWfSlotBytes = 9 * 256 * sizeof(double);
+constexpr size_t kWfSlotBytes = 8 * 256 * sizeof(double);
+constexpr int kSegRingPlanes = 5;
+constexpr size_t kSegRingBytes = 4 * kSegRingPlanes * kSegBatch * sizeof(uint64_t);
+constexpr int kSegPlaneBits = 8, kSegPlaneMask = (1 << kSegPlaneBits) - 1;
 
 struct PathId {
     uint64_t key;
@@ -312,7 +316,7 @@
     v.EN = sc.ents;
     v.FT = sc.xflat;
     if constexpr (LDS) {
-        const int nw = sc.n_xwnodes * (int)(sizeof(XWNode) / sizeof(int4));
+        const int nw = FLAT ? 0 : sc.n_xwnodes * (int)(sizeof(XWNode) / sizeof(int4));
         const int nh = sc.n_xhot * (int)(sizeof(XHot) / sizeof(int4));
         const int np = sc.n_xprims * (int)(sizeof(XPrim) / sizeof(int4));
         const int ne = sc.n_ents * (int)(sizeof(REnt) / sizeof(int4));
@@ -331,7 +335,7 @@
             v.FP = pkw;
         }
         __syncthreads();
-        v.LW = reinterpret_cast<const XWNode*>(lds);
+        if constexpr (!FLAT) v.LW = reinterpret_cast<const XWNode*>(lds);
         v.LH = reinterpret_cast<const XHot*>(lds + nw);
         v.XP = reinterpret_cast<const XPrim*>(lds + nw + nh);
         v.EN = reinterpret_cast<const REnt*>(lds + nw + nh + np);
@@ -419,7 +423,7 @@
     uint64_t c0 = STATS ? clock64() : 0;
     bool occl = false;
     double tbest = INFINITY;
-    const int skip_c = splane ? *splane : 254;
+    const int skip_c = splane ? (*splane & kSegPlaneMask) : 254;
     const int best = x_query<false, LDS, SH, TRI, CN, FLAT>(sc, v, far_r, o, d, INFINITY, act, tbest, nnode, nprim, st_steps, skip_c);
     if (act) ++nrays;
     if (STATS) {
@@ -495,7 +499,7 @@
         if (cont) {
             v.pl[0] = L.x; v.pl[256] = L.y; v.pl[512] = L.z;
             v.pl[768] = T.x; v.pl[1024] = T.y; v.pl[1280] = T.z;
-            if (splane) *splane = x_own_plane(h.pg, h.pn, d, skip_cos);
+            if (splane) *splane = (*splane & ~kSegPlaneMask) | x_own_plane(h.pg, h.pn, d, skip_cos);
         }
     }
     if (STATS) ws.cyc_sh += clock64() - c0;
@@ -613,7 +617,45 @@
 #ifndef GI_SEG_TAKE_TRI
 #define GI_SEG_TAKE_TRI 1
 #endif
-template <bool STATS, bool LDS, bool W4, bool SH, bool TRI, bool CN, bool FLAT>
+struct SegRay {
+    V3 d;
+    uint64_t key, is;
+};
+__device__ __forceinline__ bool seg_make_unit(const DevScene& sc, const CamDev& cam, const TileMap& m, const WFArgs& a, int spp,
+                                              uint64_t seed, double* rgb, uint8_t* rgb8, unsigned long long u, SegRay& r,
+                                              uint32_t& nrays, uint32_t& nres, uint32_t& npx) {
+    unsigned li, smp;
+    if (u < (1ull << 32)) {
+        li = (unsigned)u / a.ns;
+        smp = a.s0 + ((unsigned)u - li * a.ns);
+    } else {
+        li = (unsigned)(u / (unsigned long long)a.ns);
+        smp = a.s0 + (unsigned)(u - (unsigned long long)li * (unsigned long long)a.ns);
+    }
+    const unsigned ps = a.list[li];
+    long long idx = -1;
+    const V3 d0 = wf_primary(cam, m, ps, spp, seed, li, smp, idx, r.key);
+    if (smp == 0) ++npx;
+    if (wf_primary_misses(sc, cam, d0)) {
+        ++nrays;
+        ++nres;
+        wf_store(a.part, rgb, rgb8, spp, idx, smp, v3(0, 0, 0));
+        return false;
+    }
+    r.d = normalize(d0);
+    r.is = (uint64_t)(uint32_t)idx | ((uint64_t)smp << 32);
+    return true;
+}
+__device__ __forceinline__ unsigned seg_rank(unsigned long long mask) {
+    return __builtin_amdgcn_mbcnt_hi((unsigned)(mask >> 32), __builtin_amdgcn_mbcnt_lo((unsigned)mask, 0u));
+}
+__device__ __forceinline__ unsigned long long seg_uniform64(unsigned long long v) {
+    const unsigned lo = (unsigned)__builtin_amdgcn_readfirstlane((int)(unsigned)v);
+    const unsigned hi = (unsigned)__builtin_amdgcn_readfirstlane((int)(unsigned)(v >> 32));
+    return ((unsigned long long)hi << 32) | lo;
+}
+
+template <bool STATS, bool LDS, bool W4, bool SH, bool TRI, bool CN, bool FLAT, bool RING>
 __global__ __launch_bounds__(256, (LDS && W4) ? GI_WF_MIN_WAVES_LDS : GI_WF_MIN_WAVES) void k_seg(
     DevScene sc, CamDev cam, V3 light, TileMap m, int spp, int depth, uint64_t seed, double* rgb, uint8_t* rgb8,
     unsigned long long* stats, WFArgs a, int xflags) {
@@ -626,14 +668,24 @@
     const unsigned long long n_waves = (unsigned long long)gridDim.x * (blockDim.x >> 6);
     const unsigned long long run = 64ull * (unsigned long long)max(1ll, min(kTake, (long long)(total / (64ull * 8ull * n_waves))));
     uint32_t nnode = 0, nprim = 0, nrays = 0, nres = 0, npx = 0;
-    unsigned long long cur = 0, cur_end = 0;
-    bool exhausted = false;
+    SegUnits su;
     bool live = false;
-    unsigned li = 0, smp = 0;
-    long long idx = -1;
-    uint64_t key = 0;
     V3 o = cam.pos, d = v3(1, 0, 0), L = v3(0, 0, 0), T = v3(1, 1, 1);
     int splane = 254;
+    uint64_t* const rq = reinterpret_cast<uint64_t*>(v.pl - threadIdx.x + kWfSlotBytes / sizeof(double)) +
+                         (threadIdx.x >> 6) * (kSegRingPlanes * kSegBatch);
+    auto begin_path = [&](const V3& dir, uint64_t key, uint64_t is) {
+        live = true;
+        o = cam.pos;
+        d = dir;
+        splane = 254;
+        L = v3(0, 0, 0);
+        T = v3(1, 1, 1);
+        v.pl[0] = 0.0; v.pl[256] = 0.0; v.pl[512] = 0.0;
+        v.pl[768] = 1.0; v.pl[1024] = 1.0; v.pl[1280] = 1.0;
+        slot_put_u64(v.pl, 6, key);
+        slot_put_u64(v.pl, 7, is);
+    };
     const double skip_cos = x_skip_cos(sc, cam.pos);
     const float far_r = ray_far_r(sc, cam.pos);
     WFSegStats ws;
@@ -643,71 +695,80 @@
         const uint64_t t_ref = STATS ? clock64() : 0;
         for (int burst = 0; burst < GI_SEG_BURST; ++burst) {
             const unsigned long long m_need = __ballot(!live);
-            if (m_need == 0 || (exhausted && cur >= cur_end)) break;
-            const unsigned rank = (unsigned)__popcll(m_need & ((1ull << lane) - 1));
+            if (m_need == 0 || su.done()) break;
+            const unsigned rank = seg_rank(m_need);
             const unsigned n_need = (unsigned)__popcll(m_need);
+            if constexpr (RING) {
+                if (su.wants_batch(n_need)) {
+                    if (su.wants_run()) {
+                        unsigned long long nb = 0;
+                        if (lane == 0) nb = atomicAdd(reinterpret_cast<unsigned long long*>(a.take), run);
+                        su.give_run(seg_uniform64(nb), run, total);
+                    }
+                    unsigned long long first = 0;
+                    const unsigned n_batch = su.take_batch(first);
+                    if (n_batch != 0) {
+                        __builtin_amdgcn_fence(__ATOMIC_ACQ_REL, "wavefront");
+                        __builtin_amdgcn_wave_barrier();
+                        SegRay r{};
+                        bool hit = false;
+                        if ((unsigned)lane < n_batch) hit = seg_make_unit(sc, cam, m, a, spp, seed, rgb, rgb8, first + (unsigned)lane, r, nrays, nres, npx);
+                        const unsigned long long m_hit = __ballot(hit);
+                        if (hit) {
+                            uint64_t* e = rq + seg_rank(m_hit);
+                            e[0] = (uint64_t)__double_as_longlong(r.d.x);
+                            e[kSegBatch] = (uint64_t)__double_as_longlong(r.d.y);
+                            e[2 * kSegBatch] = (uint64_t)__double_as_longlong(r.d.z);
+                            e[3 * kSegBatch] = r.key;
+                            e[4 * kSegBatch] = r.is;
+                        }
+                        su.push((unsigned)__popcll(m_hit));
+                        __builtin_amdgcn_fence(__ATOMIC_ACQ_REL, "wavefront");
+                        __builtin_amdgcn_wave_barrier();
+                    }
+                }
+                unsigned first_e = 0;
+                const unsigned k = su.pop(n_need, first_e);
+                if (!live && rank < k) {
+                    const uint64_t* e = rq + (first_e + rank);
+                    begin_path(v3(__longlong_as_double((long long)e[0]), __longlong_as_double((long long)e[kSegBatch]),
+                                  __longlong_as_double((long long)e[2 * kSegBatch])),
+                               e[3 * kSegBatch], e[4 * kSegBatch]);
+                }
+                continue;
+            }
             unsigned long long u = ~0ull;
-            const unsigned long long avail = cur_end - cur;
-            if (n_need > avail && !exhausted) {
+            const unsigned long long avail = su.cur_end - su.cur;
+            if (n_need > avail && !su.exhausted) {
                 unsigned long long nb = 0;
                 if (lane == 0) nb = atomicAdd(reinterpret_cast<unsigned long long*>(a.take), run);
-                nb = __shfl(nb, 0);
+                nb = seg_uniform64(nb);
                 if (nb >= total) {
-                    exhausted = true;
-                    if (!live && rank < avail) u = cur + rank;
-                    cur = cur_end;
+                    su.exhausted = true;
+                    if (!live && rank < avail) u = su.cur + rank;
+                    su.cur = su.cur_end;
                 } else {
                     const unsigned long long ne = min(total, nb + run);
                     if (!live) {
-                        if (rank < avail) u = cur + rank;
+                        if (rank < avail) u = su.cur + rank;
                         else if (nb + (rank - avail) < ne) u = nb + (rank - avail);
                     }
-                    cur = min(ne, nb + (n_need - avail));
-                    cur_end = ne;
-                    if (ne == total) exhausted = true;
+                    su.cur = min(ne, nb + (n_need - avail));
+                    su.cur_end = ne;
+                    if (ne == total) su.exhausted = true;
                 }
             } else {
-                if (!live && rank < avail) u = cur + rank;
-                cur += min((unsigned long long)n_need, avail);
-            }
-            unsigned li_u = 0, smp_u = 0;
-            if (u != ~0ull) {
-                if (u < (1ull << 32)) {
-                    li_u = (unsigned)u / a.ns;
-                    smp_u = a.s0 + ((unsigned)u - li_u * a.ns);
-                } else {
-                    li_u = (unsigned)(u / (unsigned long long)a.ns);
-                    smp_u = a.s0 + (unsigned)(u - (unsigned long long)li_u * (unsigned long long)a.ns);
-                }
+                if (!live && rank < avail) u = su.cur + rank;
+                su.cur += min((unsigned long long)n_need, avail);
             }
             if (!live && u != ~0ull) {
-                li = li_u;
-                smp = smp_u;
-                const unsigned ps = a.list[li];
-                const V3 d0 = wf_primary(cam, m, ps, spp, seed, li, smp, idx, key);
-                if (smp == 0) ++npx;
-                if (wf_primary_misses(sc, cam, d0)) {
-                    ++nrays;
-                    ++nres;
-                    wf_store(a.part, rgb, rgb8, spp, idx, smp, v3(0, 0, 0));
-                } else {
-                    live = true;
-                    o = cam.pos;
-                    d = normalize(d0);
-                    splane = 254;
-                    L = v3(0, 0, 0);
-                    T = v3(1, 1, 1);
-                    v.pl[0] = 0.0; v.pl[256] = 0.0; v.pl[512] = 0.0;
-                    v.pl[768] = 1.0; v.pl[1024] = 1.0; v.pl[1280] = 1.0;
-                    slot_put_u64(v.pl, 6, key);
-                    slot_put_u64(v.pl, 7, (uint64_t)(uint32_t)idx | ((uint64_t)smp << 32));
-                    slot_put_u64(v.pl, 8, 0ull);
-                }
+                SegRay r{};
+                if (seg_make_unit(sc, cam, m, a, spp, seed, rgb, rgb8, u, r, nrays, nres, npx)) begin_path(r.d, r.key, r.is);
             }
         }
         if (STATS) ws.cyc_ref += clock64() - t_ref;
         if (__ballot(live) == 0) {
-            if (exhausted && cur >= cur_end) break;
+            if (su.done()) break;
             continue;
         }
         if (STATS) {
@@ -716,11 +777,11 @@
         }
         const bool cont = x_segment<STATS, LDS, SH, TRI, CN, FLAT>(
             sc, v, light, depth, no_shadow, live,
-            [&] { return PathId{slot_get_u64(v.pl, 6), (unsigned)(slot_get_u64(v.pl, 7) >> 32), (int)slot_get_u64(v.pl, 8)}; },
+            [&] { return PathId{slot_get_u64(v.pl, 6), (unsigned)(slot_get_u64(v.pl, 7) >> 32), splane >> kSegPlaneBits}; },
             o, d, L, T, nnode, nprim, nrays, ws, skip_cos, &splane, far_r);
         if (live) {
             if (cont) {
-                slot_put_u64(v.pl, 8, slot_get_u64(v.pl, 8) + 1);
+                splane += 1 << kSegPlaneBits;
             } else {
                 const uint64_t is = slot_get_u64(v.pl, 7);
                 wf_store(a.part, rgb, rgb8, spp, (long long)(uint32_t)is, (unsigned)(is >> 32), L);
@@ -942,7 +1003,11 @@
 }
 
 size_t wf_slot_bytes() { return kWfSlotBytes; }
-size_t wf_scene_lds_bytes(const DevScene& sc) { return (size_t)sc.x_lds_bytes + (sc.x_flat ? kFlatPkBytes : 0); }
+size_t wf_scene_lds_bytes(const DevScene& sc, bool flat) {
+    const size_t nodes = (flat && sc.x_flat) ? (size_t)sc.n_xwnodes * sizeof(XWNode) : 0;
+    return (size_t)sc.x_lds_bytes - nodes + (sc.x_flat ? kFlatPkBytes : 0);
+}
+size_t wf_seg_ring_bytes() { return kSegRingBytes; }
 
 template <typename F>
 void wf_dispatch(const DevScene& sc, XVariant var, bool flat, bool stats, F&& f) {
@@ -955,8 +1020,8 @@
         with_bools([&](auto S, auto T, auto C) { f(XTag<S.value, false, false, false, T.value, C.value, false>{}); },
                    stats, sc.x_tri_only != 0, sc.xcnodes != nullptr);
 }
-template <typename V>
-constexpr auto seg_kernel(V) { return &k_seg<V::stats, V::lds, V::w4, V::sh, V::tri, V::cn, V::flat>; }
+template <bool RING, typename V>
+constexpr auto seg_kernel(V) { return &k_seg<V::stats, V::lds, V::w4, V::sh, V::tri, V::cn, V::flat, RING>; }
 template <typename V>
 constexpr auto bounce_kernel(V) { return &k_wf_bounce<V::stats, V::lds, V::w4, V::sh, V::tri, V::cn, V::flat>; }
 
@@ -972,7 +1037,8 @@
         const void* f = form == 5   ? reinterpret_cast<const void*>(aov_kernel(V))
                         : form == 4 ? reinterpret_cast<const void*>(cast_kernel<true>(V))
                         : form == 3 ? reinterpret_cast<const void*>(cast_kernel<false>(V))
-                        : form == 2 ? reinterpret_cast<const void*>(seg_kernel(V))
+                        : form == 6 ? reinterpret_cast<const void*>(seg_kernel<true>(V))
+                        : form == 2 ? reinterpret_cast<const void*>(seg_kernel<false>(V))
                                     : reinterpret_cast<const void*>(bounce_kernel(V));
         e = hipOccupancyMaxActiveBlocksPerMultiprocessor(per_cu, f, 256, lds_bytes);
     });
@@ -999,7 +1065,10 @@
         a.ns = (unsigned)(s1 - s0);
         if (ev_begin) (void)hipEventRecord(ev_begin, stream);
         wf_dispatch(sc, var, flat, stats != nullptr, [&](auto V) {
-            hipLaunchKernelGGL(seg_kernel(V), grid, block, lds_bytes, stream, sc, cam, light, m, o.spp, depth, o.seed, rgb, rgb8, stats, a, xflags);
+            if (xflags & XF_SEG_RING)
+                hipLaunchKernelGGL(seg_kernel<true>(V), grid, block, lds_bytes, stream, sc, cam, light, m, o.spp, depth, o.seed, rgb, rgb8, stats, a, xflags);
+            else
+                hipLaunchKernelGGL(seg_kernel<false>(V), grid, block, lds_bytes, stream, sc, cam, light, m, o.spp, depth, o.seed, rgb, rgb8, stats, a, xflags);
         });
         if (ev_end) (void)hipEventRecord(ev_end, stream);
         return hipGetLastError();
diff --git a/include/gi.h b/include/gi.h
--- a/include/gi.h
+++ b/include/gi.h
@@ -8,7 +8,7 @@
 extern "C" {
 #endif
 
-#define GI_ABI_VERSION 13
+#define GI_ABI_VERSION 14
 
 typedef enum gi_status {
     GI_OK = 0,
@@ -182,6 +182,7 @@
 
 int gi_scene_kernel_ms(gi_scene* scene, float* avg_ms, int64_t* n);
 int gi_scene_x_form(gi_scene* scene, const gi_opts* opts, int32_t* form);
+int gi_scene_seg_ring(gi_scene* scene, const gi_opts* opts, int32_t* on);
 int gi_scene_r_kernel(gi_scene* scene, const gi_opts* opts, int32_t* kernel);
 
 typedef struct gi_octree gi_octree;
```
